# xiexh20/VisTracker

Hardware: AMD Instinct MI355X
Metric: frames/sec joint SMPL+object fit (higher is better)
Workload: dtype f32 (decoder GEMMs: 22-bit split-f16 operands x3 MFMA, fp32 accumulate)

## Files before the change

include/vistracker.h:

```cpp
#ifndef VISTRACKER_H
#define VISTRACKER_H

#ifdef __cplusplus
extern "C" {
#endif

#define VT_OK 0
#define VT_ERR_ARG -1
#define VT_ERR_HIP -2
#define VT_ERR_BUSY -3

#define VT_SMPL_V 6890
#define VT_SMPL_J 52
#define VT_SMPL_NB 10
#define VT_SMPL_NP 459
#define VT_FEAT 611
#define VT_HID 128

const char *vt_last_error(void);
int vt_version(void);

typedef struct vt_smplh vt_smplh;

int vt_smplh_create(vt_smplh **out, const float *v_template, const float *shapedirs, const float *posedirs,
                    const float *J_regressor, const float *weights, const int *parents, void *stream);
void vt_smplh_destroy(vt_smplh *h);

long vt_smplh_workspace_floats(int B);

int vt_smplh_forward(const vt_smplh *h, const float *pose, const float *betas, const float *trans, int B,
                     float *verts, float *jtr, float *v_posed, float *ws, void *stream);

long vt_smplh_bwd_scratch_floats(int B);
int vt_smplh_backward(const vt_smplh *h, const float *pose, const float *betas, int B, const float *dverts,
                      const float *djtr, const float *v_posed, const float *ws, float *scratch,
                      float *dpose, float *dbetas, float *dtrans, void *stream);

int vt_rodrigues_forward(const float *aa, int n, float *R, void *stream);
int vt_rodrigues_backward(const float *aa, int n, const float *dR, float *daa, void *stream);

typedef struct vt_landmarks vt_landmarks;
int vt_landmarks_create(vt_landmarks **out, const int *indptr, const int *indices, const float *data, int K, int V,
                        void *stream);
void vt_landmarks_destroy(vt_landmarks *h);
int vt_landmarks_forward(const vt_landmarks *h, const float *verts, int B, float *out, void *stream);
int vt_landmarks_backward(const vt_landmarks *h, const float *dout, int B, float *dverts, int accumulate, void *stream);

int vt_mahalanobis(const float *x, int B, int stride, int off, int n, const float *mean, const float *prec,
                   float *value, float *dx, float gscale, void *stream);

int vt_fill_f64(double *p, long n, double value, void *stream);
int vt_sum_to_term(const float *value, int n, float scale, double *term, void *stream);

typedef struct vt_sifnet vt_sifnet;
int vt_sifnet_create(vt_sifnet **out, const float *const *w, const float *const *b, const float *cam, void *stream);
void vt_sifnet_destroy(vt_sifnet *h);

int vt_nchw_to_nhwc(const float *src, int B, int C, int H, int W, float *dst, void *stream);

typedef struct {
    const float *maps[8];
    int res[8];
    const float *proj;
    int proj_cols;
    int act_level;
    int proj_level;
    int force_fp32;
} vt_maps;

int vt_query_forward(const vt_sifnet *h, const vt_maps *maps, const float *pts, const float *crop_center,
                     const float *body_center, int B, int N,
                     float *df, float *pca, float *parts, float *centers, float *vis, void *stream);
int vt_query_backward(const vt_sifnet *h, const vt_maps *maps, const float *pts, const float *crop_center,
                      const float *body_center, int B, int N,
                      const float *d_df, const float *d_pca, const float *d_parts, const float *d_centers,
                      const float *d_vis, float *dpts, void *stream);

long vt_query_projection_floats(const vt_maps *maps, int B);
int vt_query_build_projection(const vt_sifnet *h, const vt_maps *maps, int B, float *proj, void *stream);

int vt_query_human_loss(const vt_sifnet *h, const vt_maps *maps, const float *pts, const float *crop_center,
                        const float *body_center, int B, int N, const int *labels, const int *order, float w_dfh, float w_part,
                        float *dpts, double *terms, void *stream);
int vt_query_object_loss(const vt_sifnet *h, const vt_maps *maps, const float *pts, const float *crop_center,
                         const float *body_center, int B, int N, const float *occ, float w_obj,
                         float *dpts, double *terms, void *stream);

typedef struct vt_conv3x3 vt_conv3x3;
int vt_conv3x3_create(vt_conv3x3 **out, const float *weight, int cout, int cin, void *stream);
void vt_conv3x3_destroy(vt_conv3x3 *h);
int vt_conv3x3_forward(const vt_conv3x3 *h, const float *in, int B, int H, int W, float *out, int out_cstride, int out_coff, void *stream);
int vt_conv3x3_forward_gn(const vt_conv3x3 *h, const float *in, int in_cstride, int in_coff, const float *gn_stats, const float *gamma,
                          const float *beta, int groups, int B, int H, int W, float *out, int out_cstride, int out_coff, void *stream);
int vt_conv3x3_forward_gn_stats(const vt_conv3x3 *h, const float *in, int in_cstride, int in_coff, const float *gn_stats, const float *gamma,
                                const float *beta, int groups, int B, int H, int W, float *out, int out_cstride, int out_coff, double *stats_ws,
                                int stats_groups, void *stream);
int vt_conv3x3_forward_block(const vt_conv3x3 *h, const float *in, int in_cstride, int in_coff, const float *gn_stats, const float *gamma,
                             const float *beta, int groups, int B, int H, int W, float *out, int out_cstride, int out_coff,
                             const float *res, int res_cstride, int res_coff, float *fin, int fin_cstride, int fin_coff,
                             double *stats_ws, int stats_groups, void *stream);
int vt_conv3x3_tiles(int H, int W);
typedef struct vt_stem7x7 vt_stem7x7;
int vt_stem7x7_create(vt_stem7x7 **out, const float *weight, const float *bias, int cout, int cin, void *stream);
void vt_stem7x7_destroy(vt_stem7x7 *h);
int vt_stem7x7_forward(const vt_stem7x7 *h, const float *in, int in_cstride, int in_coff, int B, int H, int W, float *out, int out_cstride, int out_coff, void *stream);
typedef struct vt_conv1x1 vt_conv1x1;
int vt_conv1x1_create(vt_conv1x1 **out, const float *weight, const float *bias, int cout, int cin, void *stream);
void vt_conv1x1_destroy(vt_conv1x1 *h);
int vt_conv1x1_forward(const vt_conv1x1 *h, const float *in, int in_cstride, int in_coff, const float *gn_stats, const float *gamma, const float *beta, int groups,
                       int B, int H, int W, float *out, int out_cstride, int out_coff, const float *res, int res_cstride, int res_coff,
                       double *stats_ws, int stats_groups, void *stream);
int vt_groupnorm_finalize(double *ws, int nblk, int B, int HW, int C, int groups, float eps, void *stream);
int vt_conv3x3_forward_block_stats(const vt_conv3x3 *h, const float *in, int in_cstride, int in_coff, const float *gn_stats, const float *gamma,
                                   const float *beta, int groups, int B, int H, int W, float *out, int out_cstride, int out_coff,
                                   const float *res, int res_cstride, int res_coff, float *fin, int fin_cstride, int fin_coff,
                                   double *stats_ws, int stats_groups, double *fin_stats_ws, int fin_stats_groups, void *stream);
int vt_avgpool2x2_stats(const float *x, int B, int H, int W, int C, float *out, double *stats_ws, int stats_groups, void *stream);
int vt_sweep_blocks(int HW);
int vt_groupnorm_stats(const float *x, int cstride, int coff, int B, int HW, int C, int groups, float eps, double *ws, void *stream);

#define VT_PRECISION_SPLIT_F16 0
#define VT_PRECISION_FP32 1
int vt_sifnet_set_precision(vt_sifnet *h, int mode);
int vt_sifnet_get_precision(const vt_sifnet *h);

int vt_query_set_human_kernel(int threads);

int vt_query_project_step(const vt_sifnet *h, const vt_maps *maps, const float *pts, const float *crop_center,
                          const float *body_center, int B, int N, int df_idx, float threshold, float *pts_out,
                          float *df_target, void *stream);

int vt_kpts_step(const vt_landmarks *h, const float *verts, const float *kpts, const float *crop_center, int B, int mode, const float *cam, float net_size,
                 float gscale, double *term, float *J, float *dverts, int accumulate, void *stream);
int vt_query_human_step(const vt_sifnet *h, const vt_maps *maps, const float *pts, const float *crop_center, const float *body_center,
                        int B, int N, const int *labels, const int *order, float w_dfh, float w_part, int accumulate, float w_accel,
                        double *term_accel, float *dpts, double *terms, void *stream);
int vt_objstep_head(const float *M0, const float *noise, const float *t, const float *s, int B, const float *X0_points, int N, float *X_points,
                    const float *X0_verts, int NV, float *X_verts, float *R, double *terms, int nzero, float *svd_ws, void *stream);
int vt_temporal_loss2(const float *v, int B, int D, float gscale_accel, double *term_accel, float gscale_velocity, double *term_velocity, float *dv,
                      int init_zero, void *stream);
int vt_objstep_tail(const float *X0_verts, int NV, const float *dX_verts, const float *X0_points, int N, const float *dX_points, const float *s, int B,
                    const float *M0, const float *noise, const float *t, const float *t_init, float w_trans, double *term_trans,
                    float *dR, float *dt, float *dM,
                    float *pR, float *mR, float *vR, float lrR, float *pT, float *mT, float *vT, float lrT, int adam_step, float beta1, float beta2, float eps,
                    double *terms, const float *w, int nterms, float tol, int armed, float *state, int *stop_flag, float *history, int slot, int *ticket, int nzero,
                    float *svd_ws, void *stream);
int vt_objstep_tail_temporal(const float *X_points, float gscale_accel, double *term_accel, float gscale_velocity, double *term_velocity, int init_zero,
                             const float *X0_verts, int NV, const float *dX_verts, const float *X0_points, int N, const float *dX_points, const float *s, int B,
                             const float *M0, const float *noise, const float *t, const float *t_init, float w_trans, double *term_trans,
                             float *dR, float *dt, float *dM,
                             float *pR, float *mR, float *vR, float lrR, float *pT, float *mT, float *vT, float lrT, int adam_step, float beta1, float beta2, float eps,
                             double *terms, const float *w, int nterms, float tol, int armed, float *state, int *stop_flag, float *history, int slot, int *ticket, int nzero,
                             float *svd_ws, void *stream);
int vt_smplstep_tail(float *pose, const float *pose_init, float *dpose, int B, const float *prior_mean, const float *prior_prec, float gscale_prior,
                     double *term_prior, float w_pinit, double *term_pinit,
                     float *p0, int ps0, const float *g0, int gs0, float *m0, float *v0, int n0, float lr0,
                     float *p1, int ps1, const float *g1, int gs1, float *m1, float *v1, int n1, float lr1,
                     float *p2, int ps2, const float *g2, int gs2, float *m2, float *v2, int n2, float lr2,
                     int adam_step, float beta1, float beta2, float eps,
                     double *terms, const float *w, int nterms, float tol, int armed, float *state, int *stop_flag, float *history, int slot, int *ticket, int nzero,
                     void *stream);

int vt_so3_project_forward(const float *M0, const float *noise, int B, float *R, void *stream);
int vt_so3_project_backward(const float *M0, const float *noise, int B, const float *dR, float *dM, void *stream);

int vt_rigid_forward(const float *X0, int shared_x0, const float *R, const float *t, const float *s, int B, int N,
                     float *X, void *stream);
int vt_rigid_backward(const float *X0, int shared_x0, const float *s, int B, int N, const float *dX,
                      float *dR, float *dt, int accumulate, void *stream);

int vt_accel_loss(const float *v, int B, int D, const float *elem_w, float gscale, double *term, float *dv, void *stream);
int vt_accel_loss_strided(const float *v, int B, int D, int stride, const float *elem_w, float gscale, double *term,
                          float *dv, void *stream);
int vt_velocity_loss(const float *v, int B, int D, float gscale, double *term, float *dv, void *stream);

int vt_kpts_loss(const float *J, const float *kpts, const float *crop_center, int B, int K, int mode,
                 const float *cam, float net_size, float gscale, double *term, float *dJ, void *stream);

int vt_sqdiff_loss(const float *a, int a_stride, const float *b, int b_stride, int rows, int cols, float denom,
                   float gscale, double *term, float *da, void *stream);

long vt_collision_workspace_bytes(int B, int n_smpl_faces);
int vt_collision_loss(const float *smpl_verts, int n_smpl_verts, const int *smpl_faces, int n_smpl_faces, const float *obj_verts, int n_obj_verts,
                      const int *obj_faces, int n_obj_faces, int B, float sigma, int max_collisions, float gscale, double *term,
                      float *d_obj_t, int *pairs_per_frame, void *workspace, void *stream);

int vt_chamfer_ragged(const float *x, const int *offx, const float *y, const int *offy, int P, float gscale,
                      double *term, float *dx, float *dy, void *stream);
long vt_chamfer_ws_bytes(long total_x, long total_y, int P);
int vt_chamfer_ragged_ws(const float *x, const int *offx, long total_x, const float *y, const int *offy, long total_y, int P, float gscale,
                         double *term, float *dx, float *dy, void *ws, void *stream);

int vt_chamfer_ragged_idx(const float *x, const int *offx, long total_x, const float *y_base, const int *idx_y, const int *offy, long total_y, int P,
                          float gscale, double *term, float *dy_base, void *ws, int run_plan, void *stream);

int vt_nn_distance(const float *query, int nq, const float *search, int ns, int P, float *dist, void *stream);

long vt_sil_workspace_floats(int B, int NV, int NF, int size);
int vt_sil_forward(const float *verts, int B, int NV, const int *faces, int NF, const float *K, int size,
                   float *image, int *face_index, float *ws, void *stream);
int vt_sil_backward(const float *verts, int B, int NV, const int *faces, int NF, const float *K, int size,
                    const int *face_index, const float *d_image, float eps, float *ws, float *dverts, void *stream);
int vt_sil_setup(const float *mask_h, const float *mask_o, int B, int H, int W, const float *crop_centers, double expansion, int out, double crop_size,
                 double net_size, const double *cam_norm, double image_width, float *image_ref, float *keep_mask, float *K, double *boxes_ws, void *stream);

int vt_sil_mask_loss(const float *image, const float *keep, const float *ref, const float *occ, int B, int size,
                     float gscale, double *term, float *per_frame, float *d_image, void *stream);

int vt_sil_step(const float *verts, int B, int NV, const int *faces, int NF, const float *K, int size, const float *keep, const float *ref,
                const float *occ, float gscale, float eps, double *term, int *face_index, float *d_image, float *ws, float *dverts, void *stream);

int vt_triplane_render(const float *verts, const float *center, int B, int NV, const int *faces, int NF, int size,
                       float *masks, int *face_index, float *ws, void *stream);

int vt_upsample2x_bicubic_add(const float *low, const float *skip, int B, int h, int w, int C, float *out, void *stream);
int vt_upsample2x_bicubic_add_stats(const float *low, const float *skip, int B, int h, int w, int C, float *out, double *stats_ws, int stats_groups,
                                    void *stream);

long vt_groupnorm_workspace_doubles(int B, int HW, int C, int groups);
int vt_groupnorm_nhwc(const float *x, const float *gamma, const float *beta, int B, int HW, int C, int groups, float eps,
                      int relu, double *ws, float *y, void *stream);

int vt_adam_step(float *p, const float *g, float *m, float *v, long n, int step, float lr, float beta1, float beta2,
                 float eps, const int *stop_flag, void *stream);

int vt_adam_step_2d(float *p, long p_stride, const float *g, long g_stride, float *m, float *v, int rows, int cols,
                    int step, float lr, float beta1, float beta2, float eps, const int *stop_flag, void *stream);

int vt_loss_reduce_and_stop(const double *terms, const float *w, int nterms, float tol, int armed, float *state,
                            int *stop_flag, float *history, int slot, void *stream);

int vt_fill(float *p, long n, float value, void *stream);

int vt_stream_set_skip_flag(void *stream, const int *flag);

int vt_gen_round_compact(const float *surface, const float *df_target, const float *pre, const unsigned char *active, int B, int S, float filter_val,
                         float zmin, const long long *fill, int cap, int write, float *buf_points, int *order, float *kept_pre, long long *cnt,
                         long long *fill_out, void *stream);
int vt_gen_scatter_heads(const float *pred, int B, int C, int kmax, const long long *fill_old, const long long *cnt, int cap, float *buf, void *stream);
int vt_gen_resample(const float *samples, const int *order, const long long *cnt, const float *init, int B, int S, int S0, const float *u,
                    const float *pert, int M, float near_scale, float *out, void *stream);

long vt_render_workspace_bytes(int B, int NF, int size, int anti_aliasing, long list_entries);
int vt_render_static_create(void **layer, const float *verts, int NV, const int *faces, int NS, const float *face_colors, const float *K, float orig_size,
                            const float *light, int size, int anti_aliasing, void *stream);
void vt_render_static_destroy(void *layer);
int vt_render_rgb(const float *verts, int B, int NV, const int *faces, int NF, const float *face_colors, const float *K, int k_per_view, float orig_size,
                  const float *light, const float *background, const void *static_layer, int size, int anti_aliasing, float *rgb, float *alpha, float *depth,
                  int *face_index, void *ws, long ws_bytes, long *list_entries, void *stream);
int vt_render_panel_u8(const float *rgb, int B, int size, int row0, int nrows, int col0, int ncols, unsigned char *out, const long long *view_off,
                       long long out_row_stride, void *stream);
int vt_render_rgb_pv(const float *verts, int B, int NV, const int *faces, int NF, const float *face_colors, int colors_per_view, const float *K, int k_per_view,
                     float orig_size, const float *light, const float *background, const void *static_layer, int size, int anti_aliasing, float *rgb,
                     float *alpha, float *depth, int *face_index, void *ws, long ws_bytes, long *list_entries, void *stream);

int vt_contact_regions(const float *smpl_verts, const int *labels, const float *obj_verts, int B, int NVs, int NVo, int P, float thres, int *nn_idx,
                       float *nn_dist, int *part, int *count, float *centre, void *stream);
int vt_contact_spheres(const float *centre, const int *count, int B, int P, const float *unit_verts, int NSV, float radius, float *out, void *stream);
int vt_contact_face_colors(const int *part, int B, int NVo, const int *obj_faces, int NFo, int face_off, const float *base_colors, int NF, const float *palette,
                           int P, float *out, void *stream);

long vt_jpeg_workspace_bytes(int n, int H, int W, int subsampling, long long *max_out_bytes);
int vt_jpeg_encode(const unsigned char *rgb, int n, int H, int W, long long frame_stride, long long row_stride, int quality, int subsampling, void *ws,
                   long ws_bytes, unsigned char *out, long long out_cap, long long *offsets, void *stream);

int vt_mask_bbox(const unsigned char *pm, const unsigned char *om, int B, int H, int W, int thres, int *box, void *stream);
int vt_crop_resize_compose(const unsigned char *rgb, const unsigned char *pm, const unsigned char *om, int B, int H, int W, const int *corners, int crop_size,
                           int out_size, const float *table, float *out, long long frame_stride, void *stream);
int vt_resize_panel_u8(const unsigned char *src, long long src_bytes, const long long *frames, int n, int H, int size, int col0, int pw, unsigned char *out,
                       const long long *out_off, long long out_row_stride, void *stream);

int vt_overlay_panel_u8(const float *rgb, const float *alpha, int B, int size, int row0, int nrows, int col0, int ncols, unsigned char *out,
                        const long long *src_off, const long long *dst_off, long long out_row_stride, float opacity, void *stream);
int vt_mask_score(const int *fidx, int B, int is, int rows, int F, int nf_body, int nf_obj, const unsigned char *pm, long long pm_bytes, const unsigned char *om,
                  long long om_bytes, const long long *frames, int thres, int *count, void *stream);

long vt_point_mesh_workspace_bytes(int B, int n_faces);
int vt_point_mesh_distance(const float *points, int n_points, const float *verts, int n_verts, const int *faces, int n_faces, int B, float *dist, float *closest,
                           int *face_id, void *workspace, void *stream);
int vt_point_mesh_distance_ex(const float *points, int n_points, const float *verts, int n_verts, const int *faces, int n_faces, int B, float *dist,
                              float *closest, int *face_id, void *workspace, int flags, unsigned long long *n_tests, void *stream);
int vt_nearest_vertex(const float *points, int n_points, const float *verts, int n_verts, int B, int *vert_id, float *vert_dist, void *stream);

long vt_sifnet_loss_head_ws_bytes(int B, int n_points);
int vt_sifnet_loss_head(const float *df, const float *pca, const float *parts, const float *centers, const float *vis, int S, int B, int n_points,
                        const float *df_h, const float *df_o, const int *parts_gt, const float *pca_gt, const float *obj_center, const float *visibility,
                        int per_frame, float max_dist, const double *weights, int vis_loss, float gscale, double *terms, float *d_df, float *d_pca,
                        float *d_parts, float *d_centers, float *d_vis, void *workspace, void *stream);

long vt_decoder_param_floats(void);
long vt_decoder_param_offset(int head, int layer, int is_bias);
int vt_decoder_train_forward(const float *params, const float *cam, const vt_maps *maps, const float *pts, const float *crop_center, const float *body_center,
                             int B, int N, float *df, float *pca, float *parts, float *centers, float *vis, void *stream);
long vt_decoder_weight_grads_ws_bytes(int B, int N, int chunk_points);
int vt_decoder_weight_grads(const float *params, const float *cam, const vt_maps *maps, const float *pts, const float *crop_center, const float *body_center,
                            int B, int N, const float *d_df, const float *d_pca, const float *d_parts, const float *d_centers, const float *d_vis,
                            float *dparams, int accumulate, int chunk_points, void *workspace, void *stream);

long vt_decoder_grads_ws_bytes(int B, int N, int chunk_points, int want_maps);
int vt_decoder_grads(const float *params, const float *cam, const vt_maps *maps, const float *pts, const float *crop_center, const float *body_center,
                     int B, int N, const float *d_df, const float *d_pca, const float *d_parts, const float *d_centers, const float *d_vis,
                     float *dparams, int accumulate, const vt_maps *d_maps, int accumulate_maps, int chunk_points, void *workspace, void *stream);

long vt_conv_dgrad_workspace_bytes(int cout, int cin, int taps);
long vt_conv_wgrad_workspace_bytes(int B, int H, int W, int cout, int cin, int taps);
long vt_gn_relu_backward_workspace_bytes(int B, int HW, int C, int groups);
int vt_conv3x3_dgrad(const float *weight, int cout, int cin, const float *d_out, int do_cstride, int do_coff, int B, int H, int W,
                     float *d_in, int di_cstride, int di_coff, void *workspace, void *stream);
int vt_conv1x1_dgrad(const float *weight, int cout, int cin, const float *d_out, int do_cstride, int do_coff, int B, int H, int W,
                     float *d_in, int di_cstride, int di_coff, void *workspace, void *stream);
int vt_conv3x3_wgrad(const float *d_out, int do_cstride, int do_coff, const float *x_in, int xi_cstride, int xi_coff, const float *gn_stats, const float *gamma,
                     const float *beta, int groups, int B, int H, int W, int cin, int cout, float *dW, int accumulate, void *workspace, void *stream);
int vt_conv1x1_wgrad(const float *d_out, int do_cstride, int do_coff, const float *x_in, int xi_cstride, int xi_coff, const float *gn_stats, const float *gamma,
                     const float *beta, int groups, int B, int H, int W, int cin, int cout, float *dW, int accumulate, void *workspace, void *stream);
int vt_gn_relu_backward(const float *g, int g_cstride, int g_coff, const float *x_in, int x_cstride, int x_coff, const float *gn_stats, const float *gamma,
                        const float *beta, int groups, int B, int HW, int C, const float *base, int base_cstride, int base_coff,
                        float *d_x, int dx_cstride, int dx_coff, float *dgamma, float *dbeta, int accumulate, void *workspace, void *stream);
long vt_conv_block_backward_workspace(int B, int H, int W, int cin, int c1, int c2, int c3);
int vt_conv_block_backward(const float *dy, const float *x, const float *raw, const float *stats1, const float *stats2, const float *stats3,
                           const float *w1, const float *w2, const float *w3, const float *gamma1, const float *gamma2, const float *gamma3,
                           const float *beta1, const float *beta2, const float *beta3, const float *wproj, const float *gamma4, const float *beta4,
                           int B, int H, int W, int cin, int c1, int c2, int c3,
                           float *d_x, float *dW1, float *dW2, float *dW3, float *dgamma1, float *dbeta1, float *dgamma2, float *dbeta2, float *dgamma3, float *dbeta3,
                           float *dgamma4, float *dbeta4, float *dWproj, void *workspace, int accumulate, void *stream);

int vt_query_set_clock_probe(unsigned long long *counters);
long vt_calibrate_workspace_bytes(void);
int vt_calibrate(void *work, double *out, void *stream);

#ifdef __cplusplus
}
#endif
#endif
```

vistracker_amd/_lib.py:

```python
from __future__ import annotations

import ctypes as C
import os

_HERE = os.path.dirname(os.path.abspath(__file__))
LIB_PATH = os.environ.get("VT_LIB_PATH", os.path.join(_HERE, "libvistracker_hip.so"))

vp = C.c_void_p
fp = C.c_void_p
ci = C.c_int
cl = C.c_long
cf = C.c_float
cd = C.c_double


class VtMaps(C.Structure):
    _fields_ = [("maps", C.c_void_p * 8), ("res", C.c_int * 8), ("proj", C.c_void_p), ("proj_cols", C.c_int),
                ("act_level", C.c_int), ("proj_level", C.c_int), ("force_fp32", C.c_int)]


SIGNATURES = {
    "vt_last_error": (C.c_char_p, []),
    "vt_version": (ci, []),
    "vt_smplh_create": (ci, [C.POINTER(vp), vp, vp, vp, vp, vp, vp, vp]),
    "vt_smplh_destroy": (None, [vp]),
    "vt_smplh_workspace_floats": (cl, [ci]),
    "vt_smplh_bwd_scratch_floats": (cl, [ci]),
    "vt_smplh_forward": (ci, [vp, fp, fp, fp, ci, fp, fp, fp, fp, vp]),
    "vt_smplh_backward": (ci, [vp, fp, fp, ci, fp, fp, fp, fp, fp, fp, fp, fp, vp]),
    "vt_rodrigues_forward": (ci, [fp, ci, fp, vp]),
    "vt_rodrigues_backward": (ci, [fp, ci, fp, fp, vp]),
    "vt_landmarks_create": (ci, [C.POINTER(vp), vp, vp, vp, ci, ci, vp]),
    "vt_landmarks_destroy": (None, [vp]),
    "vt_landmarks_forward": (ci, [vp, fp, ci, fp, vp]),
    "vt_landmarks_backward": (ci, [vp, fp, ci, fp, ci, vp]),
    "vt_mahalanobis": (ci, [fp, ci, ci, ci, ci, fp, fp, fp, fp, cf, vp]),
    "vt_fill_f64": (ci, [fp, cl, cd, vp]),
    "vt_sum_to_term": (ci, [fp, ci, cf, fp, vp]),
    "vt_sifnet_create": (ci, [C.POINTER(vp), C.POINTER(vp), C.POINTER(vp), vp, vp]),
    "vt_sifnet_destroy": (None, [vp]),
    "vt_nchw_to_nhwc": (ci, [fp, ci, ci, ci, ci, fp, vp]),
    "vt_query_forward": (ci, [vp, C.POINTER(VtMaps), fp, fp, fp, ci, ci, fp, fp, fp, fp, fp, vp]),
    "vt_query_backward": (ci, [vp, C.POINTER(VtMaps), fp, fp, fp, ci, ci, fp, fp, fp, fp, fp, fp, vp]),
    "vt_query_human_loss": (ci, [vp, C.POINTER(VtMaps), fp, fp, fp, ci, ci, fp, fp, cf, cf, fp, fp, vp]),
    "vt_query_object_loss": (ci, [vp, C.POINTER(VtMaps), fp, fp, fp, ci, ci, fp, cf, fp, fp, vp]),
    "vt_query_set_human_kernel": (ci, [ci]),
    "vt_sifnet_set_precision": (ci, [vp, ci]),
    "vt_sifnet_get_precision": (ci, [vp]),
    "vt_groupnorm_nhwc": (ci, [fp, fp, fp, ci, ci, ci, ci, cf, ci, fp, fp, vp]),
    "vt_upsample2x_bicubic_add": (ci, [fp, fp, ci, ci, ci, ci, fp, vp]),
    "vt_conv3x3_create": (ci, [C.POINTER(vp), vp, ci, ci, vp]),
    "vt_conv3x3_destroy": (None, [vp]),
    "vt_conv3x3_forward": (ci, [vp, fp, ci, ci, ci, fp, ci, ci, vp]),
    "vt_conv3x3_forward_gn": (ci, [vp, fp, ci, ci, fp, fp, fp, ci, ci, ci, ci, fp, ci, ci, vp]),
    "vt_groupnorm_stats": (ci, [fp, ci, ci, ci, ci, ci, ci, cf, fp, vp]),
    "vt_groupnorm_workspace_doubles": (C.c_long, [ci, ci, ci, ci]),
    "vt_groupnorm_finalize": (ci, [fp, ci, ci, ci, ci, ci, cf, vp]),
    "vt_conv3x3_tiles": (ci, [ci, ci]),
    "vt_kpts_step": (ci, [vp, fp, fp, fp, ci, ci, vp, cf, cf, fp, fp, fp, ci, vp]),
    "vt_query_human_step": (ci, [vp, C.POINTER(VtMaps), fp, fp, fp, ci, ci, fp, fp, cf, cf, ci, cf, fp, fp, fp, vp]),
    "vt_objstep_head": (ci, [fp, fp, fp, fp, ci, fp, ci, fp, fp, ci, fp, fp, fp, ci, fp, vp]),
    "vt_temporal_loss2": (ci, [fp, ci, ci, cf, fp, cf, fp, fp, ci, vp]),
    "vt_objstep_tail": (ci, [fp, ci, fp, fp, ci, fp, fp, ci, fp, fp, fp, fp, cf, fp, fp, fp, fp,
                             fp, fp, fp, cf, fp, fp, fp, cf, ci, cf, cf, cf,
                             fp, vp, ci, cf, ci, fp, fp, fp, ci, fp, ci, fp, vp]),
    "vt_objstep_tail_temporal": (ci, [fp, cf, fp, cf, fp, ci,
                                      fp, ci, fp, fp, ci, fp, fp, ci, fp, fp, fp, fp, cf, fp, fp, fp, fp,
                                      fp, fp, fp, cf, fp, fp, fp, cf, ci, cf, cf, cf,
                                      fp, vp, ci, cf, ci, fp, fp, fp, ci, fp, ci, fp, vp]),
    "vt_smplstep_tail": (ci, [fp, fp, fp, ci, fp, fp, cf, fp, cf, fp,
                              fp, ci, fp, ci, fp, fp, ci, cf, fp, ci, fp, ci, fp, fp, ci, cf, fp, ci, fp, ci, fp, fp, ci, cf, ci, cf, cf, cf,
                              fp, vp, ci, cf, ci, fp, fp, fp, ci, fp, ci, vp]),
    "vt_stream_set_skip_flag": (ci, [vp, vp]),
    "vt_conv1x1_create": (ci, [C.POINTER(vp), vp, vp, ci, ci, vp]),
    "vt_stem7x7_create": (ci, [C.POINTER(vp), vp, vp, ci, ci, vp]),
    "vt_stem7x7_destroy": (None, [vp]),
    "vt_stem7x7_forward": (ci, [vp, fp, ci, ci, ci, ci, ci, fp, ci, ci, vp]),
    "vt_conv1x1_destroy": (None, [vp]),
    "vt_conv1x1_forward": (ci, [vp, fp, ci, ci, fp, fp, fp, ci, ci, ci, ci, fp, ci, ci, fp, ci, ci, fp, ci, vp]),
    "vt_conv3x3_forward_block": (ci, [vp, fp, ci, ci, fp, fp, fp, ci, ci, ci, ci, fp, ci, ci, fp, ci, ci, fp, ci, ci, fp, ci, vp]),
    "vt_conv3x3_forward_block_stats": (ci, [vp, fp, ci, ci, fp, fp, fp, ci, ci, ci, ci, fp, ci, ci, fp, ci, ci, fp, ci, ci, fp, ci, fp, ci, vp]),
    "vt_avgpool2x2_stats": (ci, [fp, ci, ci, ci, ci, fp, fp, ci, vp]),
    "vt_sweep_blocks": (ci, [ci]),
    "vt_upsample2x_bicubic_add_stats": (ci, [fp, fp, ci, ci, ci, ci, fp, fp, ci, vp]),
    "vt_conv3x3_forward_gn_stats": (ci, [vp, fp, ci, ci, fp, fp, fp, ci, ci, ci, ci, fp, ci, ci, fp, ci, vp]),
    "vt_triplane_render": (ci, [fp, fp, ci, ci, fp, ci, ci, fp, fp, fp, vp]),
    "vt_query_project_step": (ci, [vp, C.POINTER(VtMaps), fp, fp, fp, ci, ci, ci, cf, fp, fp, vp]),
    "vt_query_projection_floats": (C.c_long, [C.POINTER(VtMaps), ci]),
    "vt_query_build_projection": (ci, [vp, C.POINTER(VtMaps), ci, fp, vp]),
    "vt_so3_project_forward": (ci, [fp, fp, ci, fp, vp]),
    "vt_so3_project_backward": (ci, [fp, fp, ci, fp, fp, vp]),
    "vt_rigid_forward": (ci, [fp, ci, fp, fp, fp, ci, ci, fp, vp]),
    "vt_rigid_backward": (ci, [fp, ci, fp, ci, ci, fp, fp, fp, ci, vp]),
    "vt_accel_loss": (ci, [fp, ci, ci, fp, cf, fp, fp, vp]),
    "vt_accel_loss_strided": (ci, [fp, ci, ci, ci, fp, cf, fp, fp, vp]),
    "vt_velocity_loss": (ci, [fp, ci, ci, cf, fp, fp, vp]),
    "vt_kpts_loss": (ci, [fp, fp, fp, ci, ci, ci, vp, cf, cf, fp, fp, vp]),
    "vt_sqdiff_loss": (ci, [fp, ci, fp, ci, ci, ci, cf, cf, fp, fp, vp]),
    "vt_chamfer_ragged": (ci, [fp, fp, fp, fp, ci, cf, fp, fp, fp, vp]),
    "vt_chamfer_ws_bytes": (C.c_long, [C.c_long, C.c_long, ci]),
    "vt_chamfer_ragged_ws": (ci, [fp, fp, C.c_long, fp, fp, C.c_long, ci, cf, fp, fp, fp, fp, vp]),
    "vt_chamfer_ragged_idx": (ci, [fp, fp, C.c_long, fp, fp, fp, C.c_long, ci, cf, fp, fp, fp, ci, vp]),
    "vt_collision_workspace_bytes": (cl, [ci, ci]),
    "vt_collision_loss": (ci, [fp, ci, fp, ci, fp, ci, fp, ci, ci, cf, ci, cf, fp, fp, fp, fp, vp]),
    "vt_nn_distance": (ci, [fp, ci, fp, ci, ci, fp, vp]),
    "vt_sil_workspace_floats": (cl, [ci, ci, ci, ci]),
    "vt_sil_forward": (ci, [fp, ci, ci, fp, ci, fp, ci, fp, fp, fp, vp]),
    "vt_sil_backward": (ci, [fp, ci, ci, fp, ci, fp, ci, fp, fp, cf, fp, fp, vp]),
    "vt_sil_mask_loss": (ci, [fp, fp, fp, fp, ci, ci, cf, fp, fp, fp, vp]),
    "vt_sil_step": (ci, [fp, ci, ci, fp, ci, fp, ci, fp, fp, fp, cf, cf, fp, fp, fp, fp, fp, vp]),
    "vt_gen_round_compact": (ci, [fp, fp, fp, vp, ci, ci, cf, cf, vp, ci, ci, fp, vp, fp, vp, vp, vp]),
    "vt_gen_scatter_heads": (ci, [fp, ci, ci, ci, vp, vp, ci, fp, vp]),
    "vt_gen_resample": (ci, [fp, vp, vp, fp, ci, ci, ci, fp, fp, ci, cf, fp, vp]),
    "vt_sil_setup": (ci, [fp, fp, ci, ci, ci, fp, C.c_double, ci, C.c_double, C.c_double, C.POINTER(C.c_double), C.c_double, fp, fp, fp, fp, vp]),
    "vt_adam_step": (ci, [fp, fp, fp, fp, cl, ci, cf, cf, cf, cf, fp, vp]),
    "vt_adam_step_2d": (ci, [fp, cl, fp, cl, fp, fp, ci, ci, ci, cf, cf, cf, cf, fp, vp]),
    "vt_loss_reduce_and_stop": (ci, [fp, vp, ci, cf, ci, fp, fp, fp, ci, vp]),
    "vt_fill": (ci, [fp, cl, cf, vp]),
    "vt_selftest_mfma": (ci, [fp, fp, fp, vp]),
    "vt_query_set_clock_probe": (ci, [vp]),
    "vt_render_workspace_bytes": (cl, [ci, ci, ci, ci, cl]),
    "vt_render_static_create": (ci, [C.POINTER(vp), fp, ci, fp, ci, fp, fp, cf, C.POINTER(cf), ci, ci, vp]),
    "vt_render_static_destroy": (None, [vp]),
    "vt_render_rgb": (ci, [fp, ci, ci, fp, ci, fp, fp, ci, cf, C.POINTER(cf), C.POINTER(cf), vp, ci, ci, fp, fp, fp, fp, fp, cl,
                           C.POINTER(cl), vp]),
    "vt_render_panel_u8": (ci, [fp, ci, ci, ci, ci, ci, ci, fp, fp, C.c_longlong, vp]),
    "vt_render_rgb_pv": (ci, [fp, ci, ci, fp, ci, fp, ci, fp, ci, cf, C.POINTER(cf), C.POINTER(cf), vp, ci, ci, fp, fp, fp, fp, fp, cl,
                              C.POINTER(cl), vp]),
    "vt_contact_regions": (ci, [fp, fp, fp, ci, ci, ci, ci, cf, fp, fp, fp, fp, fp, vp]),
    "vt_contact_spheres": (ci, [fp, fp, ci, ci, fp, ci, cf, fp, vp]),
    "vt_contact_face_colors": (ci, [fp, ci, ci, fp, ci, ci, fp, ci, fp, ci, fp, vp]),
    "vt_jpeg_workspace_bytes": (cl, [ci, ci, ci, ci, C.POINTER(C.c_longlong)]),
    "vt_jpeg_encode": (ci, [fp, ci, ci, ci, C.c_longlong, C.c_longlong, ci, ci, vp, cl, vp, C.c_longlong,
                            C.POINTER(C.c_longlong), vp]),
    "vt_mask_bbox": (ci, [fp, fp, ci, ci, ci, ci, fp, vp]),
    "vt_crop_resize_compose": (ci, [fp, fp, fp, ci, ci, ci, fp, ci, ci, fp, fp, C.c_longlong, vp]),
    "vt_resize_panel_u8": (ci, [fp, C.c_longlong, vp, ci, ci, ci, ci, ci, fp, fp, C.c_longlong, vp]),
    "vt_overlay_panel_u8": (ci, [fp, fp, ci, ci, ci, ci, ci, ci, fp, fp, fp, C.c_longlong, cf, vp]),
    "vt_mask_score": (ci, [fp, ci, ci, ci, ci, ci, ci, fp, C.c_longlong, fp, C.c_longlong, vp, ci, fp, vp]),
    "vt_point_mesh_workspace_bytes": (cl, [ci, ci]),
    "vt_point_mesh_distance": (ci, [fp, ci, fp, ci, fp, ci, ci, fp, fp, fp, vp, vp]),
    "vt_point_mesh_distance_ex": (ci, [fp, ci, fp, ci, fp, ci, ci, fp, fp, fp, vp, ci, fp, vp]),
    "vt_nearest_vertex": (ci, [fp, ci, fp, ci, ci, fp, fp, vp]),
    "vt_sifnet_loss_head_ws_bytes": (cl, [ci, ci]),
    "vt_sifnet_loss_head": (ci, [fp, fp, fp, fp, fp, ci, ci, ci, fp, fp, fp, fp, fp, fp, ci, cf, C.POINTER(cd), ci, cf, fp, fp, fp, fp, fp, fp, vp, vp]),
    "vt_decoder_param_floats": (cl, []),
    "vt_decoder_param_offset": (cl, [ci, ci, ci]),
    "vt_decoder_train_forward": (ci, [fp, vp, C.POINTER(VtMaps), fp, fp, fp, ci, ci, fp, fp, fp, fp, fp, vp]),
    "vt_decoder_weight_grads_ws_bytes": (cl, [ci, ci, ci]),
    "vt_decoder_weight_grads": (ci, [fp, vp, C.POINTER(VtMaps), fp, fp, fp, ci, ci, fp, fp, fp, fp, fp, fp, ci, ci, vp, vp]),
    "vt_decoder_grads_ws_bytes": (cl, [ci, ci, ci, ci]),
    "vt_decoder_grads": (ci, [fp, vp, C.POINTER(VtMaps), fp, fp, fp, ci, ci, fp, fp, fp, fp, fp, fp, ci, C.POINTER(VtMaps), ci, ci, vp, vp]),
    "vt_conv_dgrad_workspace_bytes": (cl, [ci, ci, ci]),
    "vt_conv_wgrad_workspace_bytes": (cl, [ci, ci, ci, ci, ci, ci]),
    "vt_gn_relu_backward_workspace_bytes": (cl, [ci, ci, ci, ci]),
    "vt_conv3x3_dgrad": (ci, [fp, ci, ci, fp, ci, ci, ci, ci, ci, fp, ci, ci, vp, vp]),
    "vt_conv1x1_dgrad": (ci, [fp, ci, ci, fp, ci, ci, ci, ci, ci, fp, ci, ci, vp, vp]),
    "vt_conv3x3_wgrad": (ci, [fp, ci, ci, fp, ci, ci, fp, fp, fp, ci, ci, ci, ci, ci, ci, fp, ci, vp, vp]),
    "vt_conv1x1_wgrad": (ci, [fp, ci, ci, fp, ci, ci, fp, fp, fp, ci, ci, ci, ci, ci, ci, fp, ci, vp, vp]),
    "vt_gn_relu_backward": (ci, [fp, ci, ci, fp, ci, ci, fp, fp, fp, ci, ci, ci, ci, fp, ci, ci, fp, ci, ci, fp, fp, ci, vp, vp]),
    "vt_conv_block_backward_workspace": (cl, [ci, ci, ci, ci, ci, ci, ci]),
    "vt_conv_block_backward": (ci, [fp] * 6 + [fp] * 9 + [fp] * 3 + [ci] * 7 + [fp] * 13 + [vp, ci, vp]),
    "vt_calibrate_workspace_bytes": (cl, []),
    "vt_calibrate": (ci, [vp, C.POINTER(C.c_double), vp]),
}

_lib = None


class VtError(RuntimeError):
    pass


def lib():
    global _lib
    if _lib is None:
        if not os.path.exists(LIB_PATH):
            raise VtError(f"{LIB_PATH} is missing: build it with `make -C vistracker_amd/csrc` "
                          f"(or `python -c 'import __graft_entry__ as g; g.build()'`); there is no CPU fallback")
        import torch
        l = C.CDLL(LIB_PATH)
        for name, (res, args) in SIGNATURES.items():
            fn = getattr(l, name)
            fn.restype = res
            fn.argtypes = args
        _lib = l
        _host_tuning()
    return _lib


def _host_tuning():
    if os.environ.get("VT_HOST_THP", "keep") != "off":
        return
    try:
        C.CDLL(None, use_errno=True).prctl(41, 1, 0, 0, 0)
    except Exception:
        pass


VT_OK, VT_ERR_ARG, VT_ERR_HIP, VT_ERR_BUSY = 0, -1, -2, -3


def check(rc: int):
    if rc != 0:
        raise VtError(f"libvistracker_hip error {rc}: {lib().vt_last_error().decode()}")


def stream_ptr():
    import torch
    return torch.cuda.current_stream().cuda_stream


def dptr(t):
    if t is None:
        return None
    if not t.is_cuda:
        raise VtError("libvistracker_hip ops need CUDA (HIP) tensors; there is no CPU fallback in the product path")
    if not t.is_contiguous():
        raise VtError("libvistracker_hip ops need contiguous tensors")
    import torch
    if t.device.index != torch.cuda.current_device():
        raise VtError(f"tensor on cuda:{t.device.index} but the current device is cuda:{torch.cuda.current_device()}: "
                      "wrap the call in `with torch.cuda.device(tensor.device):`")
    return t.data_ptr()
```

vistracker_amd/csrc/smplh.hip:

```cpp
#include "common.h"
#include <cstring>

#define V_ VT_SMPL_V
#define J_ VT_SMPL_J
#define NB_ VT_SMPL_NB
#define NP_ VT_SMPL_NP
#define VP_ 6912
#define NVT_ 27
#define KQ_ 472
#define NQ_ 480
typedef float f32x4 __attribute__((ext_vector_type(4)));
#define MFMA16(a, b, c) __builtin_amdgcn_mfma_f32_16x16x4f32((a), (b), (c), 0, 0, 0)

#define WS_R 0
#define WS_J (52 * 9)
#define WS_G (WS_J + 52 * 3)
#define WS_A (WS_G + 52 * 12)
#define WS_FRAME (WS_A + 52 * 12)
#define PT_DA 0
#define PT_DTR 624
#define PT_N 627
#define KTOT_ (VP_ * 3)
#define KG_SLAB 24
#define NKS_ (KTOT_ / 16 / KG_SLAB)

#define SCHED_STEPS 32
#define SCHED_WIDTH 10
struct SmplParents { int p[J_]; int nsteps; short sched[SCHED_STEPS][SCHED_WIDTH]; };

#define SP_K 8
struct vt_smplh {
    float *Q_kcv, *Q_t, *W_jv, *W_v64, *J_t, *J_s;
    float *W_sp;
    int nnz;
    SmplParents par;
};

struct RodCtx { float n, ax, ay, az, c, s, qn, w, x, y, z; };

__device__ __forceinline__ void rodrigues_fwd(const float *t, float *R, RodCtx *k)
{
    const float xe = t[0] + 1e-8f, ye = t[1] + 1e-8f, ze = t[2] + 1e-8f;
    const float n = sqrtf(xe * xe + ye * ye + ze * ze);
    const float ax = t[0] / n, ay = t[1] / n, az = t[2] / n;
    const float h = n * 0.5f;
    const float c = cosf(h), s = sinf(h);
    const float q0 = c, q1 = s * ax, q2 = s * ay, q3 = s * az;
    const float qn = sqrtf(q0 * q0 + q1 * q1 + q2 * q2 + q3 * q3);
    const float w = q0 / qn, x = q1 / qn, y = q2 / qn, z = q3 / qn;
    const float w2 = w * w, x2 = x * x, y2 = y * y, z2 = z * z;
    const float wx = w * x, wy = w * y, wz = w * z, xy = x * y, xz = x * z, yz = y * z;
    R[0] = w2 + x2 - y2 - z2; R[1] = 2 * xy - 2 * wz;   R[2] = 2 * wy + 2 * xz;
    R[3] = 2 * wz + 2 * xy;   R[4] = w2 - x2 + y2 - z2; R[5] = 2 * yz - 2 * wx;
    R[6] = 2 * xz - 2 * wy;   R[7] = 2 * wx + 2 * yz;   R[8] = w2 - x2 - y2 + z2;
    if (k) { k->n = n; k->ax = ax; k->ay = ay; k->az = az; k->c = c; k->s = s; k->qn = qn; k->w = w; k->x = x; k->y = y; k->z = z; }
}

__device__ __forceinline__ void rodrigues_bwd(const float *t, const float *dR, float *dt)
{
    float R[9]; RodCtx k; rodrigues_fwd(t, R, &k);
    const float w = k.w, x = k.x, y = k.y, z = k.z;
    const float dw = 2 * w * (dR[0] + dR[4] + dR[8]) + 2 * (-z * dR[1] + y * dR[2] + z * dR[3] - x * dR[5] - y * dR[6] + x * dR[7]);
    const float dx = 2 * x * (dR[0] - dR[4] - dR[8]) + 2 * (y * dR[1] + z * dR[2] + y * dR[3] - w * dR[5] + z * dR[6] + w * dR[7]);
    const float dy = 2 * y * (-dR[0] + dR[4] - dR[8]) + 2 * (x * dR[1] + w * dR[2] + x * dR[3] + z * dR[5] - w * dR[6] + z * dR[7]);
    const float dz = 2 * z * (-dR[0] - dR[4] + dR[8]) + 2 * (-w * dR[1] + x * dR[2] + w * dR[3] + y * dR[5] + x * dR[6] + y * dR[7]);
    const float dot = w * dw + x * dx + y * dy + z * dz;
    const float dq0 = (dw - w * dot) / k.qn, dq1 = (dx - x * dot) / k.qn, dq2 = (dy - y * dot) / k.qn, dq3 = (dz - z * dot) / k.qn;
    const float dh = -k.s * dq0 + k.c * (k.ax * dq1 + k.ay * dq2 + k.az * dq3);
    const float dax = k.s * dq1, day = k.s * dq2, daz = k.s * dq3;
    const float dn = 0.5f * dh - (t[0] * dax + t[1] * day + t[2] * daz) / (k.n * k.n);
    dt[0] = dax / k.n + dn * (t[0] + 1e-8f) / k.n;
    dt[1] = day / k.n + dn * (t[1] + 1e-8f) / k.n;
    dt[2] = daz / k.n + dn * (t[2] + 1e-8f) / k.n;
}

__global__ void rodrigues_fwd_kernel(const float *aa, int n, float *R)
{
    const int i = blockIdx.x * blockDim.x + threadIdx.x;
    if (i >= n) return;
    float t[3] = {aa[3 * i], aa[3 * i + 1], aa[3 * i + 2]}, r[9];
    rodrigues_fwd(t, r, nullptr);
#pragma unroll
    for (int e = 0; e < 9; e++) R[9 * i + e] = r[e];
}

__global__ void rodrigues_bwd_kernel(const float *aa, int n, const float *dR, float *daa)
{
    const int i = blockIdx.x * blockDim.x + threadIdx.x;
    if (i >= n) return;
    float t[3] = {aa[3 * i], aa[3 * i + 1], aa[3 * i + 2]}, g[9], d[3];
#pragma unroll
    for (int e = 0; e < 9; e++) g[e] = dR[9 * i + e];
    rodrigues_bwd(t, g, d);
    daa[3 * i] = d[0]; daa[3 * i + 1] = d[1]; daa[3 * i + 2] = d[2];
}

__global__ __launch_bounds__(64) void smplh_pose_kernel(const float *__restrict__ pose, const float *__restrict__ betas,
                                                        const float *__restrict__ trans, const float *__restrict__ J_t,
                                                        const float *__restrict__ J_s, SmplParents par,
                                                        float *__restrict__ ws, float *__restrict__ jtr, const int *skip)
{
    VT_SKIP_RETURN(skip);
    __shared__ float sR[J_ * 9], sJ[J_ * 3], sG[J_ * 12];
    const int b = blockIdx.x, j = threadIdx.x;
    float *w = ws + (size_t)b * WS_FRAME;
    if (j < J_) {
        float t[3] = {pose[(b * J_ + j) * 3], pose[(b * J_ + j) * 3 + 1], pose[(b * J_ + j) * 3 + 2]}, R[9];
        rodrigues_fwd(t, R, nullptr);
#pragma unroll
        for (int e = 0; e < 9; e++) { sR[j * 9 + e] = R[e]; w[WS_R + j * 9 + e] = R[e]; }
#pragma unroll
        for (int c = 0; c < 3; c++) {
            float a = J_t[j * 3 + c];
#pragma unroll
            for (int l = 0; l < NB_; l++) a += J_s[(j * 3 + c) * NB_ + l] * betas[b * NB_ + l];
            sJ[j * 3 + c] = a; w[WS_J + j * 3 + c] = a;
        }
    }
    __shared__ int sPar[J_];
    if (j < J_) sPar[j] = par.p[j];
    __syncthreads();
    int lvl = 0, maxl = 0;
    if (j < J_) { for (int q = j; q != 0; q = sPar[q]) lvl++; }
    maxl = lvl;
    for (int o = 32; o > 0; o >>= 1) maxl = max(maxl, __shfl_xor(maxl, o, 64));
    maxl = __builtin_amdgcn_readfirstlane(maxl);
    if (j == 0) { for (int r = 0; r < 3; r++) { for (int c = 0; c < 3; c++) sG[r * 4 + c] = sR[r * 3 + c]; sG[r * 4 + 3] = sJ[r]; } }
    __syncthreads();
    for (int l = 1; l <= maxl; l++) {
        if (j < J_ && lvl == l) {
            const int i = j, p = sPar[i];
            const float *Gp = sG + 12 * p, *Ri = sR + 9 * i;
            const float d0 = sJ[3 * i] - sJ[3 * p], d1 = sJ[3 * i + 1] - sJ[3 * p + 1], d2 = sJ[3 * i + 2] - sJ[3 * p + 2];
            float *Gi = sG + 12 * i;
            for (int r = 0; r < 3; r++) {
                const float g0 = Gp[r * 4], g1 = Gp[r * 4 + 1], g2 = Gp[r * 4 + 2];
                Gi[r * 4 + 0] = g0 * Ri[0] + g1 * Ri[3] + g2 * Ri[6];
                Gi[r * 4 + 1] = g0 * Ri[1] + g1 * Ri[4] + g2 * Ri[7];
                Gi[r * 4 + 2] = g0 * Ri[2] + g1 * Ri[5] + g2 * Ri[8];
                Gi[r * 4 + 3] = g0 * d0 + g1 * d1 + g2 * d2 + Gp[r * 4 + 3];
            }
        }
        __syncthreads();
    }
    if (j < J_) {
        const float *G = sG + 12 * j;
#pragma unroll
        for (int r = 0; r < 3; r++) {
            const float gt = G[r * 4 + 3];
            w[WS_G + j * 12 + r * 4 + 0] = G[r * 4]; w[WS_G + j * 12 + r * 4 + 1] = G[r * 4 + 1];
            w[WS_G + j * 12 + r * 4 + 2] = G[r * 4 + 2]; w[WS_G + j * 12 + r * 4 + 3] = gt;
            w[WS_A + j * 12 + r * 4 + 0] = G[r * 4]; w[WS_A + j * 12 + r * 4 + 1] = G[r * 4 + 1]; w[WS_A + j * 12 + r * 4 + 2] = G[r * 4 + 2];
            w[WS_A + j * 12 + r * 4 + 3] = gt - (G[r * 4] * sJ[3 * j] + G[r * 4 + 1] * sJ[3 * j + 1] + G[r * 4 + 2] * sJ[3 * j + 2]);
            if (jtr) jtr[(b * J_ + j) * 3 + r] = gt + trans[3 * b + r];
        }
    }
}

#define FWD_FB 16
#ifndef FWD_PF
#define FWD_PF 6
#endif
#define AXS 516
#define SAS 628
#define FWD_R0 (FWD_FB * AXS > 8 * SAS ? FWD_FB * AXS : 8 * SAS)
__global__ __launch_bounds__(256) void smplh_verts_kernel(const float *__restrict__ Q_kcv, const float *__restrict__ W_jv,
                                                          const float *__restrict__ betas, const float *__restrict__ trans,
                                                          const float *__restrict__ ws, int B,
                                                          float *__restrict__ verts, float *__restrict__ v_posed, const float *__restrict__ W_sp, int nnz, const int *skip)
{
    VT_SKIP_RETURN(skip);
    extern __shared__ __attribute__((aligned(16))) float lds[];
    float *sAx = lds;
    float *sA = lds;
    float *sVp = lds + FWD_R0;
    float *sW = sVp + FWD_FB * 64 * 3;
    float *sTr = sW + (nnz > 0 ? 2 * SP_K * 64 : J_ * 64);
    const int tid = threadIdx.x, wave = tid >> 6, lane = tid & 63, q = lane >> 4, j = lane & 15;
    const int b0 = blockIdx.y * FWD_FB, v = blockIdx.x * 64 + wave * 16 + j;
    for (int k = tid; k < KQ_; k += 256) {
        const int e9 = k % 9;
        const float sub = (k < NP_ && (e9 == 0 || e9 == 4 || e9 == 8)) ? 1.f : 0.f;
        float val[FWD_FB];
#pragma unroll
        for (int f = 0; f < FWD_FB; f++) {
            const int b = min(b0 + f, B - 1);
            if (k < NP_) val[f] = ws[(size_t)b * WS_FRAME + WS_R + 9 + k];
            else if (k < NP_ + NB_) val[f] = betas[b * NB_ + (k - NP_)];
            else val[f] = (k == NP_ + NB_) ? 1.f : 0.f;
        }
#pragma unroll
        for (int f = 0; f < FWD_FB; f++) sAx[f * AXS + k] = val[f] - sub;
    }
    if (nnz > 0) {
        for (int i = tid; i < nnz * 64; i += 256) {
            sW[i] = W_sp[(size_t)(i >> 6) * VP_ + blockIdx.x * 64 + (i & 63)];
            sW[SP_K * 64 + i] = W_sp[(size_t)(SP_K + (i >> 6)) * VP_ + blockIdx.x * 64 + (i & 63)];
        }
    } else
        for (int i = tid; i < J_ * 64; i += 256) sW[i] = W_jv[(i >> 6) * VP_ + blockIdx.x * 64 + (i & 63)];
    if (tid < FWD_FB * 3) { const int f = tid / 3, b = min(b0 + f, B - 1); sTr[tid] = trans[b * 3 + tid % 3]; }
    __syncthreads();

    f32x4 acc[3];
#pragma unroll
    for (int c = 0; c < 3; c++) acc[c] = (f32x4){0.f, 0.f, 0.f, 0.f};
    constexpr int NS = KQ_ / 8;
    float bq[FWD_PF][2][3];
#define FWD_LOADQ(slot_, s_)                                                                     \
    {                                                                                            \
        const float *qk = Q_kcv + (size_t)(8 * (s_) + 2 * q) * 3 * VP_ + v;                      \
        _Pragma("unroll") for (int e = 0; e < 2; e++)                                            \
            _Pragma("unroll") for (int c = 0; c < 3; c++) bq[slot_][e][c] = qk[(size_t)(e * 3 + c) * VP_]; \
    }
#pragma unroll
    for (int s = 0; s < FWD_PF; s++) FWD_LOADQ(s, s)
#pragma unroll
    for (int s = 0; s < NS; s++) {
        const float2 av = *reinterpret_cast<const float2 *>(sAx + j * AXS + 8 * s + 2 * q);
#pragma unroll
        for (int c = 0; c < 3; c++) acc[c] = MFMA16(av.x, bq[s % FWD_PF][0][c], acc[c]);
#pragma unroll
        for (int c = 0; c < 3; c++) acc[c] = MFMA16(av.y, bq[s % FWD_PF][1][c], acc[c]);
        if (s + FWD_PF < NS) FWD_LOADQ(s % FWD_PF, s + FWD_PF)
        __builtin_amdgcn_sched_barrier(0);
    }
#undef FWD_LOADQ
    __syncthreads();
#pragma unroll
    for (int r = 0; r < 4; r++)
#pragma unroll
        for (int c = 0; c < 3; c++) sVp[((4 * q + r) * 64 + wave * 16 + j) * 3 + c] = acc[c][r];
    const int vv = tid & 63, vg = blockIdx.x * 64 + vv;
#pragma unroll 1
    for (int r = 0; r < 4; r++) {
        if ((r & 1) == 0) {
            if (r) __syncthreads();
            for (int i = tid; i < 8 * 624; i += 256) {
                const int sl = i / 624, f = 4 * (sl >> 1) + r + (sl & 1), b = min(b0 + f, B - 1);
                sA[sl * SAS + (i % 624)] = ws[(size_t)b * WS_FRAME + WS_A + (i % 624)];
            }
            __syncthreads();
        }
        const int f = 4 * wave + r, b = b0 + f;
        float T[12];
#pragma unroll
        for (int e = 0; e < 12; e++) T[e] = 0.f;
        const float4 *Af = reinterpret_cast<const float4 *>(sA + (2 * wave + (r & 1)) * SAS);
        if (nnz > 0) {
            for (int k = 0; k < nnz; k++) {
                const int jj = __float_as_int(sW[k * 64 + vv]);
                const float wj = sW[(SP_K + k) * 64 + vv];
                const float4 a0 = Af[jj * 3], a1 = Af[jj * 3 + 1], a2 = Af[jj * 3 + 2];
                T[0] += wj * a0.x; T[1] += wj * a0.y; T[2] += wj * a0.z; T[3] += wj * a0.w;
                T[4] += wj * a1.x; T[5] += wj * a1.y; T[6] += wj * a1.z; T[7] += wj * a1.w;
                T[8] += wj * a2.x; T[9] += wj * a2.y; T[10] += wj * a2.z; T[11] += wj * a2.w;
            }
        } else {
#pragma unroll 4
            for (int jj = 0; jj < J_; jj++) {
                const float wj = sW[jj * 64 + vv];
                const float4 a0 = Af[jj * 3], a1 = Af[jj * 3 + 1], a2 = Af[jj * 3 + 2];
                T[0] += wj * a0.x; T[1] += wj * a0.y; T[2] += wj * a0.z; T[3] += wj * a0.w;
                T[4] += wj * a1.x; T[5] += wj * a1.y; T[6] += wj * a1.z; T[7] += wj * a1.w;
                T[8] += wj * a2.x; T[9] += wj * a2.y; T[10] += wj * a2.z; T[11] += wj * a2.w;
            }
        }
        if (b < B && vg < V_) {
            const float p0 = sVp[(f * 64 + vv) * 3], p1 = sVp[(f * 64 + vv) * 3 + 1], p2 = sVp[(f * 64 + vv) * 3 + 2];
            const size_t o = ((size_t)b * V_ + vg) * 3;
#pragma unroll
            for (int rr = 0; rr < 3; rr++) verts[o + rr] = T[rr * 4] * p0 + T[rr * 4 + 1] * p1 + T[rr * 4 + 2] * p2 + T[rr * 4 + 3] + sTr[f * 3 + rr];
            v_posed[o] = p0; v_posed[o + 1] = p1; v_posed[o + 2] = p2;
        }
    }
}

template <int FB>
__global__ __launch_bounds__(256) void smplh_bwd_tile_kernel(const float *__restrict__ W_v64, const float *__restrict__ ws,
                                                             const float *__restrict__ v_posed, const float *__restrict__ dverts,
                                                             int B, float *__restrict__ part, float *__restrict__ dvp_g, const int *skip)
{
    VT_SKIP_RETURN(skip);
    extern __shared__ __attribute__((aligned(16))) float lds[];
    float *sdT = lds;
    float *sA = sdT + 256 * 13;
    const int tid = threadIdx.x, tile = blockIdx.x, b0 = blockIdx.y * FB, v0 = tile * 256, v = v0 + tid;
    const int wave = tid >> 6, lane = tid & 63, q = lane >> 4, j = lane & 15;
    for (int i = tid; i < FB * 624; i += 256) { const int f = i / 624, b = min(b0 + f, B - 1); sA[i] = ws[(size_t)b * WS_FRAME + WS_A + (i % 624)]; }
    float w1[4][13], w2[64];
#pragma unroll
    for (int mt = 0; mt < 4; mt++)
#pragma unroll
        for (int ks = 0; ks < 13; ks++) w1[mt][ks] = W_v64[(size_t)(v0 + 64 * wave + 16 * mt + j) * 64 + 4 * ks + q];
#pragma unroll
    for (int ks = 0; ks < 64; ks++) w2[ks] = W_v64[(size_t)(v0 + 4 * ks + q) * 64 + wave * 16 + j];
    __syncthreads();
    float dvn[3] = {0.f, 0.f, 0.f}, vpn[3] = {0.f, 0.f, 0.f};
    auto fetch = [&](int b) {
#pragma unroll
        for (int r = 0; r < 3; r++) { dvn[r] = 0.f; vpn[r] = 0.f; }
        if (b < B && v < V_) {
            const size_t o = ((size_t)b * V_ + v) * 3;
            dvn[0] = dverts[o]; dvn[1] = dverts[o + 1]; dvn[2] = dverts[o + 2];
            vpn[0] = v_posed[o]; vpn[1] = v_posed[o + 1]; vpn[2] = v_posed[o + 2];
        }
    };
    fetch(b0);
#pragma unroll 1
    for (int f = 0; f < FB; f++) {
        const int b = b0 + f;
        const float dv[3] = {dvn[0], dvn[1], dvn[2]}, vp[3] = {vpn[0], vpn[1], vpn[2]};
        if (f + 1 < FB) fetch(b + 1);
#pragma unroll
        for (int r = 0; r < 3; r++) {
            sdT[tid * 13 + r * 4 + 0] = dv[r] * vp[0]; sdT[tid * 13 + r * 4 + 1] = dv[r] * vp[1];
            sdT[tid * 13 + r * 4 + 2] = dv[r] * vp[2]; sdT[tid * 13 + r * 4 + 3] = dv[r];
        }
        __syncthreads();
        {
            f32x4 t[4];
#pragma unroll
            for (int mt = 0; mt < 4; mt++) t[mt] = (f32x4){0.f, 0.f, 0.f, 0.f};
#pragma unroll
            for (int ks = 0; ks < 13; ks++) {
                const float bv = j < 12 ? sA[f * 624 + (4 * ks + q) * 12 + j] : 0.f;
#pragma unroll
                for (int mt = 0; mt < 4; mt++) t[mt] = MFMA16(w1[mt][ks], bv, t[mt]);
            }
            const int r4 = (j < 12 ? (j >> 2) : 0) * 4 + 3;
#pragma unroll
            for (int mt = 0; mt < 4; mt++) {
#pragma unroll
                for (int r = 0; r < 4; r++) {
                    const int vl = 64 * wave + 16 * mt + 4 * q + r;
                    float x = t[mt][r] * sdT[vl * 13 + r4];
                    x += __shfl_down(x, 4, 16) + __shfl_down(x, 8, 16);
                    if (j < 3 && b < B) dvp_g[(size_t)b * KTOT_ + (size_t)(v0 + vl) * 3 + j] = x;
                }
            }
        }
        {
            f32x4 acc = (f32x4){0.f, 0.f, 0.f, 0.f}, acc2 = (f32x4){0.f, 0.f, 0.f, 0.f};
#pragma unroll
            for (int ks = 0; ks < 64; ks += 2) {
                const int va = 4 * ks + q, vb = va + 4;
                const float a0 = j < 12 ? sdT[va * 13 + j] : 0.f, a1 = j < 12 ? sdT[vb * 13 + j] : 0.f;
                acc = MFMA16(a0, w2[ks], acc);
                acc2 = MFMA16(a1, w2[ks + 1], acc2);
            }
            acc += acc2;
            if (b < B) {
                float *dst = part + ((size_t)tile * B + b) * PT_N;
                const int jn = wave * 16 + j;
#pragma unroll
                for (int r = 0; r < 4; r++) {
                    const int e = 4 * q + r;
                    if (e < 12) {
                        if (jn < J_) dst[PT_DA + jn * 12 + e] = acc[r];
                        else if (jn == J_ && (e & 3) == 3) dst[PT_DTR + (e >> 2)] = acc[r];
                    }
                }
            }
        }
        __syncthreads();
    }
}

#define BL_M 96
#ifndef BL_NW
#define BL_NW 1
#endif
#define BL_AS 132
__global__ __launch_bounds__(256) void smplh_bwd_blend_kernel(const float *__restrict__ Q_p, const float *__restrict__ dvp_g, int B,
                                                              float *__restrict__ part3, const int *skip)
{
    VT_SKIP_RETURN(skip);
    __shared__ __attribute__((aligned(16))) float sA[BL_M * BL_AS];
    const int tid = threadIdx.x, wave = tid >> 6, lane = tid & 63, q = lane >> 4, j = lane & 15;
    const int ks = blockIdx.x, m0 = blockIdx.z * BL_M, nt0 = blockIdx.y * (4 * BL_NW) + wave * BL_NW;
    f32x4 acc[6][BL_NW];
#pragma unroll
    for (int mt = 0; mt < 6; mt++)
#pragma unroll
        for (int n = 0; n < BL_NW; n++) acc[mt][n] = (f32x4){0.f, 0.f, 0.f, 0.f};
    const float4 *Q4 = reinterpret_cast<const float4 *>(Q_p);
#pragma unroll 1
    for (int c = 0; c < KG_SLAB / 8; c++) {
        __syncthreads();
        for (int i = tid; i < BL_M * 32; i += 256) {
            const int row = i >> 5, c4 = i & 31, b = m0 + row;
            float4 v = make_float4(0.f, 0.f, 0.f, 0.f);
            if (b < B) v = *reinterpret_cast<const float4 *>(dvp_g + (size_t)b * KTOT_ + (size_t)(ks * KG_SLAB + c * 8) * 16 + c4 * 4);
            *reinterpret_cast<float4 *>(sA + row * BL_AS + c4 * 4) = v;
        }
        __syncthreads();
#pragma unroll
        for (int g = 0; g < 8; g++) {
            const size_t kg = (size_t)ks * KG_SLAB + c * 8 + g;
            float bq[BL_NW][4];
#pragma unroll
            for (int n = 0; n < BL_NW; n++) {
                const float4 fq = Q4[(kg * (NQ_ / 16) + min(nt0 + n, NQ_ / 16 - 1)) * 64 + lane];
                bq[n][0] = fq.x; bq[n][1] = fq.y; bq[n][2] = fq.z; bq[n][3] = fq.w;
            }
#pragma unroll
            for (int mt = 0; mt < 6; mt++) {
                const float4 a4 = *reinterpret_cast<const float4 *>(sA + (mt * 16 + j) * BL_AS + g * 16 + q * 4);
                const float av[4] = {a4.x, a4.y, a4.z, a4.w};
#pragma unroll
                for (int s = 0; s < 4; s++)
#pragma unroll
                    for (int n = 0; n < BL_NW; n++) acc[mt][n] = MFMA16(av[s], bq[n][s], acc[mt][n]);
            }
        }
    }
#pragma unroll
    for (int mt = 0; mt < 6; mt++) {
#pragma unroll
        for (int r = 0; r < 4; r++) {
            const int b = m0 + mt * 16 + 4 * q + r;
            if (b < B) {
                float *dst = part3 + ((size_t)ks * B + b) * NQ_;
#pragma unroll
                for (int n = 0; n < BL_NW; n++)
                    if (nt0 + n < NQ_ / 16) dst[(nt0 + n) * 16 + j] = acc[mt][n][r];
            }
        }
    }
}

__global__ __launch_bounds__(256) void smplh_bwd_frame_kernel(const float *__restrict__ pose, const float *__restrict__ J_s,
                                                              SmplParents par, const float *__restrict__ ws,
                                                              const float *__restrict__ part, const float *__restrict__ part3,
                                                              const float *__restrict__ djtr, int B, float *__restrict__ dpose, float *__restrict__ dbetas,
                                                              float *__restrict__ dtrans, const int *skip)
{
    VT_SKIP_RETURN(skip);
    __shared__ float red[PT_N], red3[NQ_];
    __shared__ float sdG[J_ * 12], sdJ[J_ * 3], sdR[J_ * 9];
    __shared__ float sG[J_ * 12], sRm[J_ * 9], sJr[J_ * 3];
    const int b = blockIdx.x, tid = threadIdx.x;
    const float *w = ws + (size_t)b * WS_FRAME;
    for (int i = tid; i < J_ * 12; i += 256) sG[i] = w[WS_G + i];
    for (int i = tid; i < J_ * 9; i += 256) sRm[i] = w[WS_R + i];
    for (int i = tid; i < J_ * 3; i += 256) sJr[i] = w[WS_J + i];
    for (int i = tid; i < PT_N; i += 256) {
        float s = 0.f;
#pragma unroll 9
        for (int t = 0; t < NVT_; t++) s += part[((size_t)t * B + b) * PT_N + i];
        red[i] = s;
    }
    for (int i = tid; i < NQ_; i += 256) {
        float s = 0.f;
#pragma unroll 9
        for (int t = 0; t < NKS_; t++) s += part3[((size_t)t * B + b) * NQ_ + i];
        red3[i] = s;
    }
    __syncthreads();
    if (tid < J_) {
        const int j = tid;
        const float *G = sG + 12 * j; const float *Jr = sJr;
        float dj[3] = {0.f, 0.f, 0.f};
#pragma unroll
        for (int r = 0; r < 3; r++) {
            const float dat = red[PT_DA + 12 * j + r * 4 + 3];
#pragma unroll
            for (int c = 0; c < 3; c++) { sdG[12 * j + r * 4 + c] = red[PT_DA + 12 * j + r * 4 + c] - dat * Jr[3 * j + c]; dj[c] -= G[r * 4 + c] * dat; }
            sdG[12 * j + r * 4 + 3] = dat + (djtr ? djtr[(b * J_ + j) * 3 + r] : 0.f);
        }
        sdJ[3 * j] = dj[0]; sdJ[3 * j + 1] = dj[1]; sdJ[3 * j + 2] = dj[2];
#pragma unroll
        for (int e = 0; e < 9; e++) sdR[9 * j + e] = 0.f;
    }
    __syncthreads();
    const int jloc = tid / 24, el = tid - 24 * jloc;
    const int nsteps = par.nsteps > 0 ? par.nsteps : J_ - 1;
    for (int step = 0; step < nsteps; step++) {
        const int j = par.nsteps > 0 ? (jloc < SCHED_WIDTH ? (int)par.sched[step][jloc < SCHED_WIDTH ? jloc : 0] : -1) : (jloc == 0 ? J_ - 1 - step : -1);
        if (j >= 1) {
            const int p = par.p[j];
            const float *Gp = sG + 12 * p, *Rj = sRm + 9 * j, *dGj = sdG + 12 * j;
            float upd = 0.f; float *dst = nullptr; float upd2 = 0.f; float *dst2 = nullptr;
            if (el < 12) {
                const int r = el >> 2, c = el & 3;
                dst = sdG + 12 * p + el;
                if (c < 3) upd = dGj[r * 4] * Rj[3 * c] + dGj[r * 4 + 1] * Rj[3 * c + 1] + dGj[r * 4 + 2] * Rj[3 * c + 2] + dGj[r * 4 + 3] * (sJr[3 * j + c] - sJr[3 * p + c]);
                else upd = dGj[r * 4 + 3];
            } else if (el < 21) {
                const int e = el - 12, r = e / 3, c = e - 3 * r;
                dst = sdR + 9 * j + e;
                upd = Gp[r] * dGj[c] + Gp[4 + r] * dGj[4 + c] + Gp[8 + r] * dGj[8 + c];
            } else {
                const int c = el - 21;
                upd = Gp[c] * dGj[3] + Gp[4 + c] * dGj[7] + Gp[8 + c] * dGj[11];
                dst = sdJ + 3 * j + c; dst2 = sdJ + 3 * p + c; upd2 = -upd;
            }
            if (dst) *dst += upd;
            if (dst2) *dst2 += upd2;
        }
        __syncthreads();
    }
    if (tid < 3) { for (int c = 0; c < 3; c++) sdR[3 * tid + c] += sdG[tid * 4 + c]; sdJ[tid] += sdG[tid * 4 + 3]; }
    __syncthreads();
    if (tid < J_) {
        const int j = tid;
        float g[9], t[3] = {pose[(b * J_ + j) * 3], pose[(b * J_ + j) * 3 + 1], pose[(b * J_ + j) * 3 + 2]}, d[3];
#pragma unroll
        for (int e = 0; e < 9; e++) g[e] = sdR[9 * j + e] + (j >= 1 ? red3[(j - 1) * 9 + e] : 0.f);
        rodrigues_bwd(t, g, d);
        dpose[(b * J_ + j) * 3] = d[0]; dpose[(b * J_ + j) * 3 + 1] = d[1]; dpose[(b * J_ + j) * 3 + 2] = d[2];
    } else if (tid >= 64 && tid < 64 + NB_) {
        const int l = tid - 64;
        float s = red3[NP_ + l];
        for (int i = 0; i < J_ * 3; i++) s += J_s[i * NB_ + l] * sdJ[i];
        dbetas[b * NB_ + l] = s;
    } else if (tid >= 128 && tid < 131) {
        const int c = tid - 128;
        float s = red[PT_DTR + c];
        if (djtr) for (int j = 0; j < J_; j++) s += djtr[(b * J_ + j) * 3 + c];
        dtrans[b * 3 + c] = s;
    }
}

extern "C" int vt_smplh_create(vt_smplh **out, const float *v_template, const float *shapedirs, const float *posedirs,
                               const float *J_regressor, const float *weights, const int *parents, void *stream)
{
    VT_REQUIRE(out && v_template && shapedirs && posedirs && J_regressor && weights && parents, "vt_smplh_create: null argument");
    hipStream_t st = vt_stream(stream);
    vt_smplh *h = new vt_smplh();
    for (int j = 0; j < J_; j++) h->par.p[j] = (j == 0) ? 0 : parents[j];
    for (int j = 1; j < J_; j++) VT_REQUIRE(h->par.p[j] >= 0 && h->par.p[j] < j, "vt_smplh_create: parents[%d]=%d must be in [0,%d)", j, parents[j], j);
    {
        int lvl[J_], rank[J_], maxl = 0;
        lvl[0] = 0; rank[0] = 0;
        for (int j = 1; j < J_; j++) { lvl[j] = lvl[h->par.p[j]] + 1; maxl = std::max(maxl, lvl[j]); rank[j] = 0; for (int k = j + 1; k < J_; k++) rank[j] += (h->par.p[k] == h->par.p[j]); }
        int n = 0; bool ok = true;
        for (int t = 0; t < SCHED_STEPS; t++) for (int i = 0; i < SCHED_WIDTH; i++) h->par.sched[t][i] = -1;
        for (int l = maxl; l >= 1 && ok; l--)
            for (int r = 0; r < J_ && ok; r++) {
                int cnt = 0;
                for (int j = J_ - 1; j >= 1; j--) if (lvl[j] == l && rank[j] == r) { if (n >= SCHED_STEPS || cnt >= SCHED_WIDTH) { ok = false; break; } h->par.sched[n][cnt++] = (short)j; }
                if (cnt) n++;
            }
        h->par.nsteps = ok ? n : 0;
    }
    float *Q_kcv = new float[(size_t)KQ_ * 3 * VP_](), *Q_t = new float[(size_t)VP_ * 3 * NQ_](), *W_jv = new float[(size_t)J_ * VP_](),
          *J_t = new float[J_ * 3], *J_s = new float[J_ * 3 * NB_];
    for (int v = 0; v < V_; v++) for (int c = 0; c < 3; c++) {
        for (int k = 0; k < NP_ + NB_ + 1; k++) {
            const float val = k < NP_ ? posedirs[((size_t)v * 3 + c) * NP_ + k]
                            : (k < NP_ + NB_ ? shapedirs[((size_t)v * 3 + c) * NB_ + (k - NP_)] : v_template[v * 3 + c]);
            Q_kcv[(size_t)(k * 3 + c) * VP_ + v] = val;
            {
                const size_t kr = (size_t)v * 3 + c, g = kr >> 4, qq = (kr & 15) >> 2, ss = kr & 3;
                Q_t[((g * (NQ_ / 16) + (k >> 4)) * 64 + qq * 16 + (k & 15)) * 4 + ss] = val;
            }
        }
    }
    float *W_v64 = new float[(size_t)VP_ * 64]();
    for (int v = 0; v < V_; v++) { for (int j = 0; j < J_; j++) { W_jv[(size_t)j * VP_ + v] = weights[(size_t)v * J_ + j]; W_v64[(size_t)v * 64 + j] = weights[(size_t)v * J_ + j]; } W_v64[(size_t)v * 64 + J_] = 1.0f; }
    float *W_sp = new float[(size_t)2 * SP_K * VP_]();
    int nnz = 0;
    for (int v = 0; v < V_; v++) {
        int k = 0;
        for (int j = 0; j < J_; j++) {
            const float w = weights[(size_t)v * J_ + j];
            if (w == 0.0f) continue;
            if (k < SP_K) { const int jj = j; memcpy(&W_sp[(size_t)k * VP_ + v], &jj, 4); W_sp[(size_t)(SP_K + k) * VP_ + v] = w; }
            k++;
        }
        nnz = k > nnz ? k : nnz;
    }
    h->nnz = nnz <= SP_K ? (nnz > 0 ? nnz : 1) : 0;
    for (int j = 0; j < J_; j++) for (int c = 0; c < 3; c++) {
        double a = 0; double sb[NB_] = {0};
        for (int v = 0; v < V_; v++) {
            const double r = J_regressor[(size_t)j * V_ + v];
            if (r == 0.0) continue;
            a += r * v_template[v * 3 + c];
            for (int l = 0; l < NB_; l++) sb[l] += r * shapedirs[((size_t)v * 3 + c) * NB_ + l];
        }
        J_t[j * 3 + c] = (float)a;
        for (int l = 0; l < NB_; l++) J_s[(j * 3 + c) * NB_ + l] = (float)sb[l];
    }
    int rc = VT_OK;
    if ((rc = vt_upload(&h->Q_kcv, Q_kcv, (size_t)KQ_ * 3 * VP_, st)) || (rc = vt_upload(&h->Q_t, Q_t, (size_t)VP_ * 3 * NQ_, st)) ||
        (rc = vt_upload(&h->W_jv, W_jv, (size_t)J_ * VP_, st)) || (rc = vt_upload(&h->W_v64, W_v64, (size_t)VP_ * 64, st)) ||
        (rc = vt_upload(&h->J_t, J_t, (size_t)J_ * 3, st)) || (rc = vt_upload(&h->J_s, J_s, (size_t)J_ * 3 * NB_, st)) ||
        (rc = vt_upload(&h->W_sp, W_sp, (size_t)2 * SP_K * VP_, st))) {
        return rc;
    }
    VT_HIP(hipStreamSynchronize(st));
    delete[] Q_kcv; delete[] Q_t; delete[] W_jv; delete[] W_v64; delete[] J_t; delete[] J_s; delete[] W_sp;
    *out = h;
    return VT_OK;
}

extern "C" void vt_smplh_destroy(vt_smplh *h)
{
    if (!h) return;
    hipFree(h->Q_kcv); hipFree(h->Q_t); hipFree(h->W_jv); hipFree(h->W_v64); hipFree(h->J_t); hipFree(h->J_s); hipFree(h->W_sp);
    delete h;
}

extern "C" long vt_smplh_workspace_floats(int B) { return (long)B * WS_FRAME; }
extern "C" long vt_smplh_bwd_scratch_floats(int B) { return (long)NVT_ * B * PT_N + (long)B * KTOT_ + (long)NKS_ * B * NQ_; }

#define BWD_FB 6

extern "C" int vt_smplh_forward(const vt_smplh *h, const float *pose, const float *betas, const float *trans, int B,
                                float *verts, float *jtr, float *v_posed, float *ws, void *stream)
{
    VT_REQUIRE(h && pose && betas && trans && verts && v_posed && ws && B > 0, "vt_smplh_forward: null argument or B <= 0");
    hipStream_t st = vt_stream(stream); const int *skip = vt_skip_flag_of(st);
    hipLaunchKernelGGL(smplh_pose_kernel, dim3(B), dim3(64), 0, st, pose, betas, trans, h->J_t, h->J_s, h->par, ws, jtr, skip);
    VT_LAUNCH_CHECK();
    const size_t lds_f = sizeof(float) * (FWD_R0 + FWD_FB * 64 * 3 + (h->nnz > 0 ? 2 * SP_K * 64 : J_ * 64) + FWD_FB * 3);
    VT_LDS_LIMIT(smplh_verts_kernel, sizeof(float) * (FWD_R0 + FWD_FB * 64 * 3 + J_ * 64 + FWD_FB * 3));
    hipLaunchKernelGGL(smplh_verts_kernel, dim3(VP_ / 64, (B + FWD_FB - 1) / FWD_FB), dim3(256), lds_f, st, h->Q_kcv, h->W_jv, betas, trans, ws, B,
                       verts, v_posed, h->W_sp, h->nnz, skip);
    VT_LAUNCH_CHECK();
    return VT_OK;
}

extern "C" int vt_smplh_backward(const vt_smplh *h, const float *pose, const float *betas, int B, const float *dverts,
                                 const float *djtr, const float *v_posed, const float *ws, float *scratch,
                                 float *dpose, float *dbetas, float *dtrans, void *stream)
{
    (void)betas;
    VT_REQUIRE(h && pose && dverts && v_posed && ws && scratch && dpose && dbetas && dtrans && B > 0, "vt_smplh_backward: null argument or B <= 0");
    hipStream_t st = vt_stream(stream); const int *skip = vt_skip_flag_of(st);
    const size_t lds = sizeof(float) * (256 * 13 + BWD_FB * 624);
    float *dvp_g = scratch + (size_t)NVT_ * B * PT_N, *part3 = dvp_g + (size_t)B * KTOT_;
    VT_LDS_LIMIT(smplh_bwd_tile_kernel<BWD_FB>, lds);
    hipLaunchKernelGGL(smplh_bwd_tile_kernel<BWD_FB>, dim3(NVT_, (B + BWD_FB - 1) / BWD_FB), dim3(256), lds, st, h->W_v64, ws, v_posed, dverts, B, scratch, dvp_g, skip);
    VT_LAUNCH_CHECK();
    hipLaunchKernelGGL(smplh_bwd_blend_kernel, dim3(NKS_, (NQ_ / 16 + 4 * BL_NW - 1) / (4 * BL_NW), (B + BL_M - 1) / BL_M), dim3(256), 0, st, h->Q_t, dvp_g, B, part3, skip);
    VT_LAUNCH_CHECK();
    hipLaunchKernelGGL(smplh_bwd_frame_kernel, dim3(B), dim3(256), 0, st, pose, h->J_s, h->par, ws, scratch, part3, djtr, B, dpose, dbetas, dtrans, skip);
    VT_LAUNCH_CHECK();
    return VT_OK;
}

extern "C" int vt_rodrigues_forward(const float *aa, int n, float *R, void *stream)
{
    VT_REQUIRE(aa && R && n > 0, "vt_rodrigues_forward: bad argument");
    hipLaunchKernelGGL(rodrigues_fwd_kernel, dim3((n + 255) / 256), dim3(256), 0, vt_stream(stream), aa, n, R);
    VT_LAUNCH_CHECK();
    return VT_OK;
}

extern "C" int vt_rodrigues_backward(const float *aa, int n, const float *dR, float *daa, void *stream)
{
    VT_REQUIRE(aa && dR && daa && n > 0, "vt_rodrigues_backward: bad argument");
    hipLaunchKernelGGL(rodrigues_bwd_kernel, dim3((n + 255) / 256), dim3(256), 0, vt_stream(stream), aa, n, dR, daa);
    VT_LAUNCH_CHECK();
    return VT_OK;
}
```

vistracker_amd/fitting.py:

```python
from __future__ import annotations

import contextlib
import ctypes as C
import functools
import os
import threading
import time
from dataclasses import dataclass, field

import numpy as np
import torch

from . import _lib as L
from . import ops

FIT_WEIGHTS = {"pose": 1e-5, "hand": 1e-5, "j2d": 0.09, "object": 900.0, "part": 0.0025, "contact": 900.0, "scale": 100.0,
               "df_h": 100.0, "mask": 0.0009, "ocent": 0.0, "pinit": 25.0, "rot": 100.0, "trans": 100.0,
               "stemp": 10000.0, "otemp": 225.0, "ovtemp": 2500.0, "collide": 9.0}
SMPLT_WEIGHTS = {"pose": 1e-5, "hand": 1e-5, "kpts": 0.09, "temp": 900.0, "ptemp": 25.0, "pinit": 900.0}
JOINT_WEIGHTS_66 = np.repeat(np.array([1, 10, 10, 10, 5, 5, 10, 1, 1, 10, 1, 1, 5, 5, 5, 5, 5, 5, 1, 1, 1, 1], np.float32), 3)
JOINT_WEIGHTS_66[37:39] = 10.0


def _lib():
    return L.lib()


def _chk(rc):
    L.check(rc)


def _ev_begin(prof):
    if prof is None:
        return None
    e = torch.cuda.Event(enable_timing=True); e.record()
    return e


def _flush_events(prof, local, executed):
    if prof is None:
        return
    for k, v in local.items():
        prof[k].extend((a, b, n) for a, b, n, step in v if executed is None or step < executed)


def _ev_end(prof, key, e0, frames, step):
    if prof is None:
        return
    e1 = torch.cuda.Event(enable_timing=True); e1.record()
    prof[key].append((e0, e1, frames, step))


class Terms:

    def __init__(self, names, device):
        self.names = list(names)
        self.buf = torch.zeros(len(self.names), dtype=torch.float64, device=device)
        self.idx = {n: i for i, n in enumerate(self.names)}

    def ptr(self, name):
        return self.buf.data_ptr() + 8 * self.idx[name]

    def zero(self, first=0, count=None):
        count = len(self.names) - first if count is None else count
        _chk(_lib().vt_fill_f64(self.buf.data_ptr() + 8 * first, count, 0.0, L.stream_ptr()))

    def weights(self, table, decay, extra=None):
        w = np.zeros(16, np.float32)
        for n, i in self.idx.items():
            w[i] = table[n] / (1.0 + decay) * (1.0 if extra is None else extra.get(n, 1.0))
        return w


class AdamState:

    def __init__(self, slices, stop_flag):
        self.slices = slices
        self.m = [torch.zeros(p.shape[0], n, device=p.device) for p, n, g, lr in slices]
        self.v = [torch.zeros(p.shape[0], n, device=p.device) for p, n, g, lr in slices]
        self.t = 0
        self.stop_flag = stop_flag

    def tick(self):
        self.t += 1
        return self.t

    def step(self):
        t = self.tick()
        for (p, n, g, lr), m, v in zip(self.slices, self.m, self.v):
            _chk(_lib().vt_adam_step_2d(p.data_ptr(), p.shape[1], g.data_ptr(), g.shape[1], m.data_ptr(), v.data_ptr(), p.shape[0], n,
                                        t, lr, 0.9, 0.999, 1e-8, self.stop_flag.data_ptr(), L.stream_ptr()))

    @functools.cached_property
    def smpl_tail_groups(self):
        out = ()
        for (p, n, g, lr), m, v in zip(self.slices, self.m, self.v):
            out += (p.data_ptr(), p.shape[1], g.data_ptr(), g.shape[1], m.data_ptr(), v.data_ptr(), n, lr)
        return out + (None, 0, None, 0, None, None, 0, 0.0) * (3 - len(self.slices))

    @functools.cached_property
    def object_tail_groups(self):
        rot = trans = (None, None, None, 0.0)
        for (p, n, g, lr), m, v in zip(self.slices, self.m, self.v):
            if n == 9:
                rot = (p.data_ptr(), m.data_ptr(), v.data_ptr(), lr)
            else:
                trans = (p.data_ptr(), m.data_ptr(), v.data_ptr(), lr)
        return rot + trans


def _check_finite(res, what):
    executed = res.losses[:res.steps]
    if executed.size and not np.isfinite(executed).all():
        bad = int(np.flatnonzero(~np.isfinite(executed))[0])
        raise FloatingPointError(f"{what}: non-finite loss at Adam step {bad} (non-finite input or decoder activation out of range)")


def _as_input(t, dev):
    if t is None:
        return None
    return torch.as_tensor(t).to(device=dev, dtype=torch.float32).contiguous()


def _require_params(*ts):
    for t in ts:
        if not (torch.is_tensor(t) and t.is_cuda and t.dtype == torch.float32 and t.is_contiguous()):
            raise L.VtError("fit loops update their parameters in place: pass contiguous float32 CUDA tensors "
                            f"(got {type(t).__name__} {getattr(t, 'dtype', None)} on {getattr(t, 'device', None)})")
        if t.device != ts[0].device:
            raise L.VtError("fit loops: all parameters must live on the same device")


@dataclass
class FitResult:
    steps: int = 0
    outer_iters: int = 0
    stopped_early: bool = False
    losses: np.ndarray = field(default_factory=lambda: np.zeros(0, np.float32))


def morton_order(points) -> np.ndarray:
    p = np.asarray(points, np.float64)
    q = ((p - p.min(0)) / (p.max(0) - p.min(0) + 1e-12) * 1023).astype(np.int64)

    def part(x):
        x = (x | (x << 16)) & 0x030000FF; x = (x | (x << 8)) & 0x0300F00F; x = (x | (x << 4)) & 0x030C30C3
        return (x | (x << 2)) & 0x09249249
    return np.argsort(part(q[:, 0]) | (part(q[:, 1]) << 1) | (part(q[:, 2]) << 2), kind="stable")


def morton_order_device(p: torch.Tensor) -> torch.Tensor:
    p = p.double()
    lo = p.min(0).values; hi = p.max(0).values
    q = ((p - lo) / (hi - lo + 1e-12) * 1023).long()

    def part(x):
        x = (x | (x << 16)) & 0x030000FF; x = (x | (x << 8)) & 0x0300F00F; x = (x | (x << 4)) & 0x030C30C3
        return (x | (x << 2)) & 0x09249249
    key = part(q[:, 0]) | (part(q[:, 1]) << 1)
    if p.shape[1] > 2:
        key = key | (part(q[:, 2]) << 2)
    return torch.argsort(key, stable=True).to(torch.int32)


class _StopWatch:
    _tls = threading.local()

    def __init__(self, ctx, stop, lookahead):
        self.ctx, self.stop, self.look = ctx, stop, lookahead
        self.pending = None; self.n = 0
        if lookahead:
            pool = getattr(self._tls, "pool", None)
            if pool is None or pool[0] != stop.device:
                pool = (stop.device, torch.zeros(2, dtype=torch.int32).pin_memory(), [torch.cuda.Event(), torch.cuda.Event()])
                self._tls.pool = pool
            _, self.host, self.ev = pool

    def _wait(self, k):
        t0 = time.perf_counter()
        self.ev[k].synchronize()
        with self.ctx._counter_lock:
            self.ctx.host_wait_s += time.perf_counter() - t0
        return bool(int(self.host[k]))

    def check(self):
        if not self.look:
            return bool(self.ctx._read_stop(self.stop))
        k = self.n & 1; self.n += 1
        self.host[k:k + 1].copy_(self.stop, non_blocking=True); self.ev[k].record()
        prev, self.pending = self.pending, k
        return prev is not None and self._wait(prev)

    def final(self):
        if not self.look or self.pending is None:
            return False
        k, self.pending = self.pending, None
        return self._wait(k)


class _Fit:

    def __init__(self, dev, names, nsteps, prev_loss, prof):
        self.terms = Terms(names, dev)
        self.stop = torch.zeros(1, dtype=torch.int32, device=dev)
        self.loss_state = torch.full((2,), prev_loss, device=dev)
        self.ticket = torch.zeros(1, dtype=torch.int32, device=dev)
        self.hist = torch.full((nsteps,), float("nan"), device=dev)
        self.lp = {"human": [], "object": []} if prof is not None else None
        self.adam = None


class _SmplFit(_Fit):

    def __init__(self, pose, betas, trans, names, nsteps, prev_loss, prof=None):
        dev = pose.device; B = self.B = pose.shape[0]
        super().__init__(dev, names, nsteps, prev_loss, prof)
        self.pose, self.betas, self.trans = pose, betas, trans
        self.verts = torch.empty(B, 6890, 3, device=dev); self.jtr = torch.empty(B, 52, 3, device=dev); self.vposed = torch.empty_like(self.verts)
        self.ws = torch.empty(_lib().vt_smplh_workspace_floats(B), device=dev); self.scratch = torch.empty(_lib().vt_smplh_bwd_scratch_floats(B), device=dev)
        self.dverts = torch.empty_like(self.verts); self.J = torch.empty(B, 25, 3, device=dev); self.dJ = torch.empty_like(self.J)
        self.dpose = torch.empty(B, 156, device=dev); self.dbetas = torch.empty(B, 10, device=dev); self.dtrans = torch.empty(B, 3, device=dev)
        self.vb = torch.empty(B, device=dev)
        self.pose_init = pose.clone()

    @property
    def vert_order_ptr(self):
        return self.vert_order.data_ptr() if self.vert_order is not None else None


class _ObjectFit(_Fit):

    def __init__(self, ctx, obj_R, obj_t, sil, nsteps, prof):
        dev = obj_R.device; B = self.B = obj_R.shape[0]; N = self.N = ctx.obj_points.shape[0]; NV = self.NV = ctx.obj_verts.shape[0]
        super().__init__(dev, ["object", "otemp", "ovtemp", "mask", "trans", "contact", "collide", "scale"], nsteps, 300.0, prof)
        self.obj_R, self.obj_t, self.sil = obj_R, obj_t, sil
        self.R = torch.empty(B, 3, 3, device=dev); self.X = torch.empty(B, N, 3, device=dev); self.dX = torch.empty_like(self.X)
        self.svd_ws = torch.empty(B, 22, device=dev)
        self.dR = torch.empty(B, 3, 3, device=dev); self.dM = torch.empty(B, 3, 3, device=dev); self.dt = torch.empty(B, 3, device=dev)
        if sil is not None:
            self.Vt = torch.empty(B, NV, 3, device=dev); self.dVt = torch.empty_like(self.Vt)
            self.fidx = torch.empty(B, sil.size, sil.size, dtype=torch.int32, device=dev); self.dimg = torch.empty(B, sil.size, sil.size, device=dev)
            self.sws = torch.empty(_lib().vt_sil_workspace_floats(B, NV, ctx.obj_faces.shape[0], sil.size), device=dev)
            if not ctx.fused_steps:
                self.img = torch.empty_like(self.dimg); self.per = torch.empty(B, device=dev)
        self.trans_init = None
        self.Vc = self.cws = None
        self.contact = None


class FitContext:
    use_projection = True
    sort_object_points = True
    sort_query_points = True
    collision_loss = False
    fused_steps = os.environ.get("VT_FUSED_STEPS", "1") != "0"
    fused_smpl_query = os.environ.get("VT_FUSED_SMPL_QUERY", "0") != "0"
    device_skip = os.environ.get("VT_DEVICE_SKIP", "1") != "0"

    def __init__(self, smpl_model, regressors, priors, decoders=None, part_labels=None, obj_verts=None, obj_faces=None, obj_points=None,
                 cam=ops.DEFAULT_CAM, device="cuda:0"):
        self.device = torch.device(device)
        dev = self.device
        self.smpl = ops.SmplhHandle(smpl_model, dev)
        self.b25 = ops.LandmarkHandle(regressors["body25"], dev)
        self.net = ops.SifNetHandle(decoders, cam, dev) if decoders is not None else None
        self.cam = np.ascontiguousarray(cam, np.float32)
        t = lambda a, dt=torch.float32: None if a is None else torch.as_tensor(np.ascontiguousarray(a), dtype=dt, device=dev)
        self.pri = {k: t(v) for k, v in priors.items()}
        self.labels = t(part_labels, torch.int32)
        self.vert_order = t(morton_order(np.asarray(smpl_model["v_template"])), torch.int32) if self.sort_query_points else None
        if obj_points is not None and self.sort_object_points:
            obj_points = np.asarray(obj_points, np.float32)[morton_order(obj_points)]
        self.obj_verts = t(obj_verts); self.obj_faces = t(obj_faces, torch.int32); self.obj_points = t(obj_points)
        self.smpl_faces = t(np.asarray(smpl_model["f"]).astype(np.int32), torch.int32) if "f" in smpl_model else None
        self.jw66 = t(JOINT_WEIGHTS_66)

    range_retries = 0
    fp32_fallbacks = 0
    _counter_lock = threading.Lock()
    host_wait_s = 0.0

    def _with_range_fallback(self, maps, params, run):
        if self.net is None or maps is None or maps.force_fp32 or self.net.precision == "fp32":
            return run()
        saved = [p.clone() for p in params]
        while True:
            try:
                return run()
            except FloatingPointError as e:
                import warnings
                for p, s0 in zip(params, saved):
                    p.copy_(s0)
                if maps.act_level + 1 < maps.ACT_LEVELS:
                    maps.set_act_level(maps.act_level + 1)
                    warnings.warn(f"{e}; repeating the fit at operand-range level {maps.act_level} of the split-f16 decoders", RuntimeWarning)
                    with self._counter_lock:
                        self.range_retries += 1
                    continue
                if maps.force_fp32:
                    raise
                warnings.warn(f"{e}; repeating the fit on the strict-fp32 decoder kernels (5x slower)", RuntimeWarning)
                maps.set_force_fp32(True)
                with self._counter_lock:
                    self.fp32_fallbacks += 1
                return run()

    def smpl_forward(self, pose, betas, trans, verts, jtr, vposed, ws):
        _chk(_lib().vt_smplh_forward(self.smpl.h, pose.data_ptr(), betas.data_ptr(), trans.data_ptr(), pose.shape[0], verts.data_ptr(),
                                     jtr.data_ptr(), vposed.data_ptr(), ws.data_ptr(), L.stream_ptr()))

    def smpl_backward(self, pose, betas, dverts, vposed, ws, scratch, dpose, dbetas, dtrans):
        _chk(_lib().vt_smplh_backward(self.smpl.h, pose.data_ptr(), betas.data_ptr(), pose.shape[0], dverts.data_ptr(), None, vposed.data_ptr(),
                                      ws.data_ptr(), scratch.data_ptr(), dpose.data_ptr(), dbetas.data_ptr(), dtrans.data_ptr(), L.stream_ptr()))

    def hand_prior_value(self, pose, terms, name, scratch_b):
        B = pose.shape[0]
        for off, m, p in ((66, "lhand_mean", "lhand_prec"), (111, "rhand_mean", "rhand_prec")):
            _chk(_lib().vt_mahalanobis(pose.data_ptr(), B, 156, off, 45, self.pri[m].data_ptr(), self.pri[p].data_ptr(), scratch_b.data_ptr(), None, 0.0, L.stream_ptr()))
            _chk(_lib().vt_sum_to_term(scratch_b.data_ptr(), B, 1.0 / 45.0, terms.ptr(name), L.stream_ptr()))

    def body_prior(self, pose, dpose, w, terms, name, scratch_b):
        B = pose.shape[0]
        _chk(_lib().vt_mahalanobis(pose.data_ptr(), B, 156, 3, 63, self.pri["body_mean"].data_ptr(), self.pri["body_prec"].data_ptr(),
                                   scratch_b.data_ptr(), dpose.data_ptr(), w / B, L.stream_ptr()))
        _chk(_lib().vt_sum_to_term(scratch_b.data_ptr(), B, 1.0 / B, terms.ptr(name), L.stream_ptr()))

    def _run_fit(self, f, start, end, check_every, outer, prof=None):
        res = FitResult()
        with self._skip_after_stop(f.stop) as skipping:
            watch = _StopWatch(self, f.stop, skipping)
            for it in range(start, end):
                step, phase, w, armed = outer(it)
                for i in range(10):
                    step(f, phase, (it - start) * 10 + i, w, armed)
                res.steps += 10
                res.outer_iters += 1
                if (it - start) % check_every == check_every - 1 and watch.check():
                    res.stopped_early = True
                    break
            res.stopped_early = res.stopped_early or watch.final()
        res.losses = f.hist.cpu().numpy()
        if res.stopped_early:
            res.steps = int(np.isfinite(res.losses).sum())
            res.outer_iters = -(-res.steps // 10)
        _flush_events(prof, f.lp, res.steps if (res.stopped_early and self.device_skip) else None)
        _check_finite(res, "fit")
        return res

    def fit_smplt(self, pose, betas, trans, kpts, max_iter=100, iter_for_global=8, temporal=True, pinit_w=900.0,
                  lr_global=0.01, lr_all=0.001, it_range=None, check_every=1, weights=None, early_stop=True):
        with torch.cuda.device(pose.device):
            return self._fit_smplt(pose, betas, trans, kpts, max_iter, iter_for_global, temporal, pinit_w, lr_global, lr_all, it_range, check_every, weights, early_stop)

    def _fit_smplt(self, pose, betas, trans, kpts, max_iter, iter_for_global, temporal, pinit_w, lr_global, lr_all, it_range, check_every, weights, early_stop=True):
        _require_params(pose, betas, trans)
        table = dict(SMPLT_WEIGHTS); table["pinit"] = pinit_w
        if weights is not None:
            table.update({k: float(v) for k, v in weights.items() if k in table})
        start, end = it_range if it_range is not None else (0, max_iter)
        f = _SmplFit(pose, betas, trans, ["kpts", "temp", "ptemp", "pose", "pinit", "hand"], (end - start) * 10, 0.0)
        f.kpts = _as_input(kpts, pose.device)
        f.temporal = temporal and f.B >= 3
        self.hand_prior_value(pose, f.terms, "hand", f.vb)

        def outer(it):
            if f.adam is None or it == iter_for_global:
                if it < iter_for_global:
                    f.adam = AdamState([(trans, 3, f.dtrans, lr_global), (pose, 3, f.dpose, lr_global), (betas, 2, f.dbetas, lr_global)], f.stop)
                else:
                    f.adam = AdamState([(trans, 3, f.dtrans, lr_all), (pose, 66, f.dpose, lr_all), (betas, 10, f.dbetas, lr_all)], f.stop)
            return self._smplt_step, None, f.terms.weights(table, it // 3), int(early_stop and it > 0.3 * max_iter)
        return self._run_fit(f, start, end, check_every, outer)

    def optimize_smpl(self, maps, pose, betas, trans, crop_center, body_center, body_kpts, max_iter=100, iter_for_betas=1,
                      iter_for_pose=1, iter_for_kpts=1, it_range=None, net_size=512.0, check_every=1, prof=None, early_stop=True):
        with torch.cuda.device(pose.device):
            return self._with_range_fallback(maps, (pose, betas, trans), lambda: self._optimize_smpl(
                maps, pose, betas, trans, crop_center, body_center, body_kpts, max_iter, iter_for_betas, iter_for_pose, iter_for_kpts, it_range, net_size,
                check_every, prof, early_stop))

    def _optimize_smpl(self, maps, pose, betas, trans, crop_center, body_center, body_kpts, max_iter, iter_for_betas, iter_for_pose, iter_for_kpts,
                       it_range, net_size, check_every, prof, early_stop=True):
        dev = pose.device
        _require_params(pose, betas, trans)
        split_route = self.net.precision != "fp32" and not maps.force_fp32
        if self.use_projection and split_route:
            maps.build_projection(self.net)
        total = iter_for_betas + iter_for_kpts + iter_for_pose + max_iter
        start, end = it_range if it_range is not None else (0, total)
        f = _SmplFit(pose, betas, trans, ["df_h", "part", "pose", "pinit", "j2d", "stemp", "hand"], (end - start) * 10, 300.0, prof)
        f.maps, f.net_size = maps, net_size
        f.crop_center, f.body_center, f.body_kpts = _as_input(crop_center, dev), _as_input(body_center, dev), _as_input(body_kpts, dev)
        f.vert_order = self.vert_order
        if self.sort_query_points:
            self.smpl_forward(pose, betas, trans, f.verts, f.jtr, f.vposed, f.ws)
            v0 = f.verts[f.B // 2]
            f.vert_order = morton_order_device(torch.stack([v0[:, 0] / v0[:, 2], v0[:, 1] / v0[:, 2]], 1))
        self.hand_prior_value(pose, f.terms, "hand", f.vb)
        if not self.fused_steps:
            step = self._smpl_step
        elif split_route and self.fused_smpl_query:
            step = self._smpl_step_fused_query
        else:
            step = self._smpl_step_fused
        arm_after = 0.25 * max_iter + iter_for_betas + iter_for_pose

        def outer(it):
            if it < iter_for_betas:
                phase = "global"
                if f.adam is None:
                    f.adam = AdamState([(betas, 2, f.dbetas, 0.02), (trans, 3, f.dtrans, 0.02)], f.stop)
            else:
                phase = "kpts" if it >= iter_for_betas + iter_for_pose else "smpl all pose"
                if f.adam is None or it == iter_for_betas:
                    f.adam = AdamState([(trans, 3, f.dtrans, 0.006), (pose, 66, f.dpose, 0.006), (betas, 10, f.dbetas, 0.006)], f.stop)
            return step, phase, f.terms.weights(FIT_WEIGHTS, 1 if phase != "kpts" else it / 3), int(early_stop and it > arm_after)
        return self._run_fit(f, start, end, check_every, outer, prof)

    def optimize_smpl_object(self, maps, smpl_verts, obj_R, obj_t, obj_s, crop_center, body_center, occ, sil=None, noise=None,
                             iter_for_obj=15, iter_for_sil=30, joint_iter=10, max_iter=100, it_range=None, seed=0, check_every=1, prof=None, early_stop=True):
        with torch.cuda.device(obj_R.device):
            return self._with_range_fallback(maps, (obj_R, obj_t), lambda: self._optimize_smpl_object(
                maps, smpl_verts, obj_R, obj_t, obj_s, crop_center, body_center, occ, sil, noise, iter_for_obj, iter_for_sil, joint_iter, max_iter, it_range,
                seed, check_every, prof, early_stop))

    def _optimize_smpl_object(self, maps, smpl_verts, obj_R, obj_t, obj_s, crop_center, body_center, occ, sil, noise, iter_for_obj, iter_for_sil,
                              joint_iter, max_iter, it_range, seed, check_every, prof, early_stop=True):
        dev = obj_R.device; B = obj_R.shape[0]
        _require_params(obj_R, obj_t)
        if self.use_projection and self.net.precision != "fp32" and not maps.force_fp32:
            maps.build_projection(self.net)
        total = joint_iter + iter_for_obj + max_iter + iter_for_sil
        start, end = it_range if it_range is not None else (0, total)
        f = _ObjectFit(self, obj_R, obj_t, sil, (end - start) * 10, prof)
        f.maps = maps
        f.smpl_verts, f.obj_s, f.crop_center, f.body_center, f.occ = (_as_input(x, dev) for x in (smpl_verts, obj_s, crop_center, body_center, occ))
        f.obj_s = f.obj_s.reshape(-1)
        if noise is not None:
            f.noise = _as_input(noise, dev)
        else:
            gen = torch.Generator(device=dev); gen.manual_seed(seed)
            f.noise = torch.rand((end - start) * 10, B, 3, 3, device=dev, generator=gen)
        ones = torch.ones_like(f.obj_s)
        _chk(_lib().vt_sqdiff_loss(f.obj_s.data_ptr(), 1, ones.data_ptr(), 1, B, 1, float(B), 0.0, f.terms.ptr("scale"), None, L.stream_ptr()))
        Rv, dMv = obj_R.view(B, 9), f.dM.view(B, 9)

        def outer(it):
            if it < iter_for_obj:
                phase = "object only"
                if f.adam is None:
                    f.adam = AdamState([(Rv, 9, dMv, 0.002), (obj_t, 3, f.dt, 0.006)], f.stop)
            elif it < iter_for_obj + iter_for_sil:
                phase = "sil"
                if sil is None:
                    raise L.VtError("phase 'sil' needs a SilSetup")
                if f.adam is None or it == iter_for_obj:
                    f.adam = AdamState([(Rv, 9, dMv, 0.006), (obj_t, 3, f.dt, 0.006)], f.stop)
                    f.trans_init = obj_t.clone()
            else:
                phase = "joint"
                if f.adam is None or it == iter_for_obj + iter_for_sil:
                    f.adam = AdamState([(obj_t, 3, f.dt, 0.002)], f.stop)
            decay = 1 if phase == "object only" else (it - iter_for_obj + 1 if phase == "sil" else (it - iter_for_obj + 1) / 3)
            tw = 10.0 if phase == "joint" else 1.0
            w = f.terms.weights(FIT_WEIGHTS, decay, {"otemp": tw, "ovtemp": tw})
            fused = self.fused_steps and not (phase == "joint" and self.collision_loss)
            return (self._object_step_fused if fused else self._object_step), phase, w, int(early_stop and phase == "joint" and it > 0.25 * max_iter)
        return self._run_fit(f, start, end, check_every, outer, prof)

    def _read_stop(self, stop):
        t0 = time.perf_counter()
        v = int(stop.item())
        with self._counter_lock:
            self.host_wait_s += time.perf_counter() - t0
        return v

    @contextlib.contextmanager
    def _skip_after_stop(self, stop):
        if not self.device_skip:
            yield False
            return
        sp = L.stream_ptr()
        rc = _lib().vt_stream_set_skip_flag(sp, stop.data_ptr())
        if rc == L.VT_ERR_BUSY:
            yield False
            return
        L.check(rc)
        try:
            yield True
        finally:
            _lib().vt_stream_set_skip_flag(sp, None)

    def _smplt_step(self, f, phase, k, w, armed):
        lib = _lib(); st = L.stream_ptr(); B = f.B; pose = f.pose
        f.terms.zero(0, 5)
        self.smpl_forward(pose, f.betas, f.trans, f.verts, f.jtr, f.vposed, f.ws)
        _chk(lib.vt_landmarks_forward(self.b25.h, f.verts.data_ptr(), B, f.J.data_ptr(), st))
        _chk(lib.vt_kpts_loss(f.J.data_ptr(), f.kpts.data_ptr(), None, B, 25, 0, self.cam.ctypes.data, 0.0, float(w[0]), f.terms.ptr("kpts"), f.dJ.data_ptr(), st))
        _chk(lib.vt_landmarks_backward(self.b25.h, f.dJ.data_ptr(), B, f.dverts.data_ptr(), 0, st))
        if f.temporal:
            _chk(lib.vt_accel_loss(f.verts.data_ptr(), B, 6890 * 3, None, float(w[1]), f.terms.ptr("temp"), f.dverts.data_ptr(), st))
        self.smpl_backward(pose, f.betas, f.dverts, f.vposed, f.ws, f.scratch, f.dpose, f.dbetas, f.dtrans)
        if f.temporal:
            _chk(lib.vt_accel_loss_strided(pose.data_ptr(), B, 66, 156, self.jw66.data_ptr(), float(w[2]), f.terms.ptr("ptemp"), f.dpose.data_ptr(), st))
        self.body_prior(pose, f.dpose, float(w[3]), f.terms, "pose", f.vb)
        _chk(lib.vt_sqdiff_loss(pose.data_ptr() + 12, 156, f.pose_init.data_ptr() + 12, 156, B, 63, float(B * 63), float(w[4]),
                                f.terms.ptr("pinit"), f.dpose.data_ptr() + 12, st))
        f.adam.step()
        _chk(lib.vt_loss_reduce_and_stop(f.terms.buf.data_ptr(), w.ctypes.data, len(f.terms.names), 1e-3, armed, f.loss_state.data_ptr(),
                                         f.stop.data_ptr(), f.hist.data_ptr(), k, st))

    def _human_query(self, f, k, w):
        ev = _ev_begin(f.lp)
        _chk(_lib().vt_query_human_loss(self.net.h, C.byref(f.maps.c), f.verts.data_ptr(), f.crop_center.data_ptr(), f.body_center.data_ptr(), f.B, 6890,
                                        self.labels.data_ptr(), f.vert_order_ptr, float(w[0]), float(w[1]), f.dverts.data_ptr(), f.terms.ptr("df_h"),
                                        L.stream_ptr()))
        _ev_end(f.lp, "human", ev, f.B, k)

    def _smpl_step(self, f, phase, k, w, armed):
        lib = _lib(); st = L.stream_ptr(); B = f.B; pose = f.pose
        f.terms.zero(0, 6)
        self.smpl_forward(pose, f.betas, f.trans, f.verts, f.jtr, f.vposed, f.ws)
        self._human_query(f, k, w)
        if phase == "kpts":
            _chk(lib.vt_landmarks_forward(self.b25.h, f.verts.data_ptr(), B, f.J.data_ptr(), st))
            _chk(lib.vt_kpts_loss(f.J.data_ptr(), f.body_kpts.data_ptr(), f.crop_center.data_ptr(), B, 25, 1, self.cam.ctypes.data, f.net_size,
                                  float(w[4]), f.terms.ptr("j2d"), f.dJ.data_ptr(), st))
            _chk(lib.vt_landmarks_backward(self.b25.h, f.dJ.data_ptr(), B, f.dverts.data_ptr(), 1, st))
        if B >= 4:
            _chk(lib.vt_accel_loss(f.verts.data_ptr(), B, 6890 * 3, None, float(w[5]), f.terms.ptr("stemp"), f.dverts.data_ptr(), st))
        self.smpl_backward(pose, f.betas, f.dverts, f.vposed, f.ws, f.scratch, f.dpose, f.dbetas, f.dtrans)
        self.body_prior(pose, f.dpose, float(w[2]), f.terms, "pose", f.vb)
        _chk(lib.vt_sqdiff_loss(pose.data_ptr() + 12, 156, f.pose_init.data_ptr() + 12, 156, B, 69, float(B), float(w[3]),
                                f.terms.ptr("pinit"), f.dpose.data_ptr() + 12, st))
        f.adam.step()
        _chk(lib.vt_loss_reduce_and_stop(f.terms.buf.data_ptr(), w.ctypes.data, len(f.terms.names), 1e-3, armed, f.loss_state.data_ptr(),
                                         f.stop.data_ptr(), f.hist.data_ptr(), k, st))

    def _smpl_step_fused(self, f, phase, k, w, armed):
        lib = _lib(); st = L.stream_ptr(); B = f.B
        self.smpl_forward(f.pose, f.betas, f.trans, f.verts, f.jtr, f.vposed, f.ws)
        self._human_query(f, k, w)
        if phase == "kpts":
            _chk(lib.vt_kpts_step(self.b25.h, f.verts.data_ptr(), f.body_kpts.data_ptr(), f.crop_center.data_ptr(), B, 1, self.cam.ctypes.data, f.net_size,
                                  float(w[4]), f.terms.ptr("j2d"), f.J.data_ptr(), f.dverts.data_ptr(), 1, st))
        if B >= 4:
            _chk(lib.vt_accel_loss(f.verts.data_ptr(), B, 6890 * 3, None, float(w[5]), f.terms.ptr("stemp"), f.dverts.data_ptr(), st))
        self.smpl_backward(f.pose, f.betas, f.dverts, f.vposed, f.ws, f.scratch, f.dpose, f.dbetas, f.dtrans)
        self._smpl_tail(f, k, w, armed)

    def _smpl_step_fused_query(self, f, phase, k, w, armed):
        lib = _lib(); st = L.stream_ptr(); B = f.B
        self.smpl_forward(f.pose, f.betas, f.trans, f.verts, f.jtr, f.vposed, f.ws)
        if phase == "kpts":
            _chk(lib.vt_kpts_step(self.b25.h, f.verts.data_ptr(), f.body_kpts.data_ptr(), f.crop_center.data_ptr(), B, 1, self.cam.ctypes.data, f.net_size,
                                  float(w[4]), f.terms.ptr("j2d"), f.J.data_ptr(), f.dverts.data_ptr(), 0, st))
        ev = _ev_begin(f.lp)
        _chk(lib.vt_query_human_step(self.net.h, C.byref(f.maps.c), f.verts.data_ptr(), f.crop_center.data_ptr(), f.body_center.data_ptr(), B, 6890,
                                     self.labels.data_ptr(), f.vert_order_ptr, float(w[0]), float(w[1]), int(phase == "kpts"), float(w[5]),
                                     f.terms.ptr("stemp") if B >= 4 else None, f.dverts.data_ptr(), f.terms.ptr("df_h"), st))
        _ev_end(f.lp, "human", ev, B, k)
        self.smpl_backward(f.pose, f.betas, f.dverts, f.vposed, f.ws, f.scratch, f.dpose, f.dbetas, f.dtrans)
        self._smpl_tail(f, k, w, armed)

    def _smpl_tail(self, f, k, w, armed):
        _chk(_lib().vt_smplstep_tail(f.pose.data_ptr(), f.pose_init.data_ptr(), f.dpose.data_ptr(), f.B, self.pri["body_mean"].data_ptr(),
                                     self.pri["body_prec"].data_ptr(), float(w[2]) / f.B, f.terms.ptr("pose"), float(w[3]), f.terms.ptr("pinit"),
                                     *f.adam.smpl_tail_groups, f.adam.tick(), 0.9, 0.999, 1e-8,
                                     f.terms.buf.data_ptr(), w.ctypes.data, len(f.terms.names), 1e-3, armed, f.loss_state.data_ptr(), f.stop.data_ptr(),
                                     f.hist.data_ptr(), k, f.ticket.data_ptr(), 6, L.stream_ptr()))

    def _object_query(self, f, k, w):
        ev = _ev_begin(f.lp)
        _chk(_lib().vt_query_object_loss(self.net.h, C.byref(f.maps.c), f.X.data_ptr(), f.crop_center.data_ptr(), f.body_center.data_ptr(), f.B, f.N,
                                         f.occ.data_ptr(), float(w[0]), f.dX.data_ptr(), f.terms.ptr("object"), L.stream_ptr()))
        _ev_end(f.lp, "object", ev, f.B, k)

    def _contacts(self, f, w):
        if f.contact is None:
            f.contact = self._contacts_once(f.maps, f.smpl_verts, f.X, f.crop_center, f.body_center)
        if f.contact["P"] > 0:
            self._contact_term(f.contact, f.X, f.dX, float(w[5]), f.terms)

    def _object_step(self, f, phase, k, w, armed):
        lib = _lib(); st = L.stream_ptr(); B, N, NV, nz = f.B, f.N, f.NV, f.noise[k]
        obj_R, obj_t, obj_s, X, dX, R, dR, dt = f.obj_R, f.obj_t, f.obj_s, f.X, f.dX, f.R, f.dR, f.dt
        nf = self.obj_faces.shape[0]
        f.terms.zero(0, 7)
        _chk(lib.vt_so3_project_forward(obj_R.data_ptr(), nz.data_ptr(), B, R.data_ptr(), st))
        _chk(lib.vt_rigid_forward(self.obj_points.data_ptr(), 1, R.data_ptr(), obj_t.data_ptr(), obj_s.data_ptr(), B, N, X.data_ptr(), st))
        if phase == "sil":
            _chk(lib.vt_fill(dX.data_ptr(), dX.numel(), 0.0, st))
        else:
            self._object_query(f, k, w)
        if B >= 4:
            _chk(lib.vt_accel_loss(X.data_ptr(), B, N * 3, None, float(w[1]), f.terms.ptr("otemp"), dX.data_ptr(), st))
            _chk(lib.vt_velocity_loss(X.data_ptr(), B, N * 3, float(w[2]), f.terms.ptr("ovtemp"), dX.data_ptr(), st))
        acc = 0
        if phase == "sil":
            sil = f.sil
            _chk(lib.vt_rigid_forward(self.obj_verts.data_ptr(), 1, R.data_ptr(), obj_t.data_ptr(), obj_s.data_ptr(), B, NV, f.Vt.data_ptr(), st))
            _chk(lib.vt_sil_forward(f.Vt.data_ptr(), B, NV, self.obj_faces.data_ptr(), nf, sil.K.data_ptr(), sil.size, f.img.data_ptr(), f.fidx.data_ptr(),
                                    f.sws.data_ptr(), st))
            _chk(lib.vt_sil_mask_loss(f.img.data_ptr(), sil.keep.data_ptr(), sil.ref.data_ptr(), f.occ.data_ptr(), B, sil.size, float(w[3]),
                                      f.terms.ptr("mask"), f.per.data_ptr(), f.dimg.data_ptr(), st))
            _chk(lib.vt_sil_backward(f.Vt.data_ptr(), B, NV, self.obj_faces.data_ptr(), nf, sil.K.data_ptr(), sil.size, f.fidx.data_ptr(), f.dimg.data_ptr(),
                                     1e-4, f.sws.data_ptr(), f.dVt.data_ptr(), st))
            _chk(lib.vt_rigid_backward(self.obj_verts.data_ptr(), 1, obj_s.data_ptr(), B, NV, f.dVt.data_ptr(), dR.data_ptr(), dt.data_ptr(), 0, st))
            _chk(lib.vt_sqdiff_loss(obj_t.data_ptr(), 3, f.trans_init.data_ptr(), 3, B, 3, float(B * 3), float(w[4]), f.terms.ptr("trans"), dt.data_ptr(), st))
            acc = 1
        if phase == "joint":
            self._contacts(f, w)
        _chk(lib.vt_rigid_backward(self.obj_points.data_ptr(), 1, obj_s.data_ptr(), B, N, dX.data_ptr(), dR.data_ptr(), dt.data_ptr(), acc, st))
        if phase == "joint" and self.collision_loss:
            if f.cws is None:
                f.Vc = torch.empty(B, NV, 3, device=X.device)
                f.cws = torch.empty((lib.vt_collision_workspace_bytes(B, self.smpl_faces.shape[0]) + 7) // 8, dtype=torch.int64, device=X.device)
            _chk(lib.vt_rigid_forward(self.obj_verts.data_ptr(), 1, R.data_ptr(), obj_t.data_ptr(), obj_s.data_ptr(), B, NV, f.Vc.data_ptr(), st))
            _chk(lib.vt_collision_loss(f.smpl_verts.data_ptr(), f.smpl_verts.shape[1], self.smpl_faces.data_ptr(), self.smpl_faces.shape[0], f.Vc.data_ptr(), NV,
                                       self.obj_faces.data_ptr(), nf, B, 0.5, 8, float(w[6]), f.terms.ptr("collide"), dt.data_ptr(), None, f.cws.data_ptr(), st))
        _chk(lib.vt_so3_project_backward(obj_R.data_ptr(), nz.data_ptr(), B, dR.data_ptr(), f.dM.data_ptr(), st))
        f.adam.step()
        _chk(lib.vt_loss_reduce_and_stop(f.terms.buf.data_ptr(), w.ctypes.data, len(f.terms.names), 1e-4, armed, f.loss_state.data_ptr(), f.stop.data_ptr(),
                                         f.hist.data_ptr(), k, st))

    def _object_step_fused(self, f, phase, k, w, armed):
        lib = _lib(); st = L.stream_ptr(); B, N, NV, nz = f.B, f.N, f.NV, f.noise[k]
        is_sil = phase == "sil"
        X, dX = f.X.data_ptr(), f.dX.data_ptr()
        obj_verts, Vt, dVt = (self.obj_verts.data_ptr(), f.Vt.data_ptr(), f.dVt.data_ptr()) if is_sil else (None, None, None)
        _chk(lib.vt_objstep_head(f.obj_R.data_ptr(), nz.data_ptr(), f.obj_t.data_ptr(), f.obj_s.data_ptr(), B, self.obj_points.data_ptr(), N, X,
                                 obj_verts, NV, Vt, f.R.data_ptr(), f.terms.buf.data_ptr(), 7, f.svd_ws.data_ptr(), st))
        if not is_sil:
            self._object_query(f, k, w)
        tail_temporal = B >= 4 and phase != "joint"
        if B >= 4 and phase == "joint":
            _chk(lib.vt_temporal_loss2(X, B, N * 3, float(w[1]), f.terms.ptr("otemp"), float(w[2]), f.terms.ptr("ovtemp"), dX, 0, st))
        elif is_sil and B < 4:
            _chk(lib.vt_fill(dX, f.dX.numel(), 0.0, st))
        if is_sil:
            sil = f.sil
            _chk(lib.vt_sil_step(Vt, B, NV, self.obj_faces.data_ptr(), self.obj_faces.shape[0], sil.K.data_ptr(), sil.size, sil.keep.data_ptr(),
                                 sil.ref.data_ptr(), f.occ.data_ptr(), float(w[3]), 1e-4, f.terms.ptr("mask"), f.fidx.data_ptr(), f.dimg.data_ptr(),
                                 f.sws.data_ptr(), dVt, st))
        if phase == "joint":
            self._contacts(f, w)
        tail, pre = lib.vt_objstep_tail, ()
        if tail_temporal:
            tail, pre = lib.vt_objstep_tail_temporal, (X, float(w[1]), f.terms.ptr("otemp"), float(w[2]), f.terms.ptr("ovtemp"), int(is_sil))
        _chk(tail(*pre, obj_verts, NV, dVt, self.obj_points.data_ptr(), N, dX, f.obj_s.data_ptr(), B, f.obj_R.data_ptr(), nz.data_ptr(), f.obj_t.data_ptr(),
                  f.trans_init.data_ptr() if is_sil else None, float(w[4]), f.terms.ptr("trans"), f.dR.data_ptr(), f.dt.data_ptr(), f.dM.data_ptr(),
                  *f.adam.object_tail_groups, f.adam.tick(), 0.9, 0.999, 1e-8, f.terms.buf.data_ptr(), w.ctypes.data, len(f.terms.names), 1e-4, armed,
                  f.loss_state.data_ptr(), f.stop.data_ptr(), f.hist.data_ptr(), k, f.ticket.data_ptr(), 0, f.svd_ws.data_ptr(), st))

    def _contact_term(self, contact, X, dX, w, terms):
        _chk(_lib().vt_chamfer_ragged_idx(contact["x"].data_ptr(), contact["offx"].data_ptr(), contact["x"].shape[0], X.data_ptr(), contact["idx_o32"].data_ptr(),
                                          contact["offy"].data_ptr(), contact["idx_o32"].shape[0], contact["P"], w, terms.ptr("contact"), dX.data_ptr(),
                                          contact["ws"].data_ptr(), int(not contact["planned"]), L.stream_ptr()))
        contact["planned"] = True

    def _contacts_once(self, maps, smpl_verts, X, crop_center, body_center, thres=0.08):
        B, N = X.shape[:2]; V = smpl_verts.shape[1]; dev = X.device
        df_o, _, parts_o, _, _ = ops.sifnet_query(self.net, maps, X, crop_center, body_center, head_mask=0b00101)
        df_h, _, _, _, _ = ops.sifnet_query(self.net, maps, smpl_verts, crop_center, body_center, head_mask=0b00001)
        mask_o = df_o[:, 0] < thres
        mask_h = df_h[:, 1] < thres
        lab_o = parts_o.argmax(1)
        lab_h = self.labels.long().unsqueeze(0).expand(B, V)
        oh = torch.zeros(B, 14, device=dev, dtype=torch.long); oo = torch.zeros_like(oh)
        oh.scatter_add_(1, lab_h, mask_h.long()); oo.scatter_add_(1, lab_o, mask_o.long())
        pair = (oh > 0) & (oo > 0)
        P = int(pair.sum().item())
        if P == 0:
            return {"P": 0}
        sel_h = mask_h & pair.gather(1, lab_h); sel_o = mask_o & pair.gather(1, lab_o)
        bh, vh = sel_h.nonzero(as_tuple=True); bo, no = sel_o.nonzero(as_tuple=True)
        cnt_h = (oh * pair).reshape(-1); cnt_o = (oo * pair).reshape(-1)
        keep = pair.reshape(-1)
        ch, co = cnt_h[keep], cnt_o[keep]
        perm = torch.argsort(ch * co, descending=True, stable=True)
        rank_of_key = torch.zeros(B * 14, dtype=torch.long, device=dev)
        rank_of_key[keep.nonzero(as_tuple=True)[0][perm]] = torch.arange(P, device=dev)
        kh = rank_of_key[bh * 14 + lab_h[bh, vh]]; ko = rank_of_key[bo * 14 + lab_o[bo, no]]
        oh_s = torch.sort(kh, stable=True); oo_s = torch.sort(ko, stable=True)
        idx_h = (bh * V + vh)[oh_s.indices]; idx_o = (bo * N + no)[oo_s.indices]
        offx = torch.zeros(P + 1, dtype=torch.int32, device=dev); offy = torch.zeros(P + 1, dtype=torch.int32, device=dev)
        offx[1:] = torch.cumsum(ch[perm], 0).int(); offy[1:] = torch.cumsum(co[perm], 0).int()
        x = smpl_verts.reshape(-1, 3).index_select(0, idx_h).contiguous()
        ws = torch.empty(int(_lib().vt_chamfer_ws_bytes(x.shape[0], idx_o.shape[0], P)), dtype=torch.uint8, device=dev)
        return {"P": P, "x": x, "offx": offx, "offy": offy, "idx_o": idx_o, "idx_o32": idx_o.int().contiguous(), "ws": ws, "planned": False}


class SilSetup:

    def __init__(self, K, keep, ref, size=256):
        self.K, self.keep, self.ref, self.size = K.contiguous(), keep.contiguous(), ref.contiguous(), size
```

vistracker_amd/ops.py:

```python
from __future__ import annotations

import ctypes as C

import numpy as np
import torch

from . import _lib as L


def _f32(t):
    return t.detach().contiguous().float()


def _np32(a):
    return np.ascontiguousarray(np.asarray(a), dtype=np.float32)


class SmplhHandle:

    def __init__(self, model: dict, device="cuda:0"):
        self.device = torch.device(device)
        par = np.asarray(model["parents"]).astype(np.int64).copy()
        par[0] = 0
        par = np.ascontiguousarray(par, dtype=np.int32)
        arrs = [_np32(model[k]) for k in ("v_template", "shapedirs", "posedirs", "J_regressor", "weights")]
        assert arrs[0].shape == (6890, 3) and arrs[1].shape == (6890, 3, 10) and arrs[2].shape == (6890, 3, 459)
        assert arrs[3].shape == (52, 6890) and arrs[4].shape == (6890, 52)
        h = C.c_void_p()
        with torch.cuda.device(self.device):
            L.check(L.lib().vt_smplh_create(C.byref(h), *[a.ctypes.data for a in arrs], par.ctypes.data, L.stream_ptr()))
        self.h = h
        self.faces = np.asarray(model["f"]).astype(np.int64) if "f" in model else None

    def __del__(self):
        try:
            if getattr(self, "h", None):
                L.lib().vt_smplh_destroy(self.h)
        except Exception:
            pass


class _SmplhFn(torch.autograd.Function):
    @staticmethod
    def forward(ctx, handle: SmplhHandle, pose, betas, trans):
        pose, betas, trans = _f32(pose), _f32(betas), _f32(trans)
        B = pose.shape[0]
        dev = pose.device
        verts = torch.empty(B, 6890, 3, device=dev); jtr = torch.empty(B, 52, 3, device=dev)
        vposed = torch.empty(B, 6890, 3, device=dev)
        ws = torch.empty(L.lib().vt_smplh_workspace_floats(B), device=dev)
        L.check(L.lib().vt_smplh_forward(handle.h, L.dptr(pose), L.dptr(betas), L.dptr(trans), B, L.dptr(verts), L.dptr(jtr),
                                         L.dptr(vposed), L.dptr(ws), L.stream_ptr()))
        ctx.handle = handle
        ctx.save_for_backward(pose, betas, vposed, ws)
        ctx.mark_non_differentiable(vposed)
        return verts, jtr, vposed

    @staticmethod
    def backward(ctx, dverts, djtr, _dvp):
        pose, betas, vposed, ws = ctx.saved_tensors
        B = pose.shape[0]
        dev = pose.device
        dverts = torch.zeros(B, 6890, 3, device=dev) if dverts is None else _f32(dverts)
        djtr = None if djtr is None else _f32(djtr)
        scratch = torch.empty(L.lib().vt_smplh_bwd_scratch_floats(B), device=dev)
        dpose = torch.empty(B, 156, device=dev); dbetas = torch.empty(B, 10, device=dev); dtrans = torch.empty(B, 3, device=dev)
        L.check(L.lib().vt_smplh_backward(ctx.handle.h, L.dptr(pose), L.dptr(betas), B, L.dptr(dverts), L.dptr(djtr), L.dptr(vposed),
                                          L.dptr(ws), L.dptr(scratch), L.dptr(dpose), L.dptr(dbetas), L.dptr(dtrans), L.stream_ptr()))
        return None, dpose, dbetas, dtrans


def smplh_forward(handle: SmplhHandle, pose, betas, trans):
    return _SmplhFn.apply(handle, pose, betas, trans)


def rodrigues(aa):
    aa = _f32(aa).reshape(-1, 3)
    R = torch.empty(aa.shape[0], 9, device=aa.device)
    L.check(L.lib().vt_rodrigues_forward(L.dptr(aa), aa.shape[0], L.dptr(R), L.stream_ptr()))
    return R


def rodrigues_bwd(aa, dR):
    aa = _f32(aa).reshape(-1, 3); dR = _f32(dR).reshape(-1, 9)
    d = torch.empty_like(aa)
    L.check(L.lib().vt_rodrigues_backward(L.dptr(aa), aa.shape[0], L.dptr(dR), L.dptr(d), L.stream_ptr()))
    return d


class LandmarkHandle:
    def __init__(self, csr: dict, device="cuda:0"):
        self.K, self.V = csr["shape"]
        ip = np.ascontiguousarray(csr["indptr"], np.int32); ix = np.ascontiguousarray(csr["indices"], np.int32)
        da = _np32(csr["data"])
        h = C.c_void_p()
        with torch.cuda.device(torch.device(device)):
            L.check(L.lib().vt_landmarks_create(C.byref(h), ip.ctypes.data, ix.ctypes.data, da.ctypes.data, self.K, self.V, L.stream_ptr()))
        self.h = h

    def __del__(self):
        try:
            if getattr(self, "h", None):
                L.lib().vt_landmarks_destroy(self.h)
        except Exception:
            pass


class _LandmarkFn(torch.autograd.Function):
    @staticmethod
    def forward(ctx, handle, verts):
        verts = _f32(verts); B = verts.shape[0]
        out = torch.empty(B, handle.K, 3, device=verts.device)
        L.check(L.lib().vt_landmarks_forward(handle.h, L.dptr(verts), B, L.dptr(out), L.stream_ptr()))
        ctx.handle = handle; ctx.B = B
        return out

    @staticmethod
    def backward(ctx, dout):
        dout = _f32(dout)
        dverts = torch.empty(ctx.B, ctx.handle.V, 3, device=dout.device)
        L.check(L.lib().vt_landmarks_backward(ctx.handle.h, L.dptr(dout), ctx.B, L.dptr(dverts), 0, L.stream_ptr()))
        return None, dverts


def landmarks(handle: LandmarkHandle, verts):
    return _LandmarkFn.apply(handle, verts)


class _MahalanobisFn(torch.autograd.Function):
    @staticmethod
    def forward(ctx, x, off, mean, prec):
        x = _f32(x); B, stride = x.shape; n = mean.shape[0]
        val = torch.empty(B, device=x.device)
        L.check(L.lib().vt_mahalanobis(L.dptr(x), B, stride, off, n, L.dptr(mean), L.dptr(prec), L.dptr(val), None, 0.0, L.stream_ptr()))
        ctx.save_for_backward(x, mean, prec); ctx.off = off
        return val

    @staticmethod
    def backward(ctx, dval):
        x, mean, prec = ctx.saved_tensors
        B, stride = x.shape; n = mean.shape[0]
        dx = torch.zeros_like(x); val = torch.empty(B, device=x.device)
        L.check(L.lib().vt_mahalanobis(L.dptr(x), B, stride, ctx.off, n, L.dptr(mean), L.dptr(prec), L.dptr(val), L.dptr(dx), 1.0, L.stream_ptr()))
        return dx * dval.reshape(B, 1), None, None, None


def mahalanobis(x, off, mean, prec):
    return _MahalanobisFn.apply(x, off, mean, prec)


HEADS = ("df", "pca", "parts", "centers", "vis")
HEAD_DIMS = (2, 9, 14, 3, 1)
MAP_ORDER = ("im_feat", "tmpx", "tri_tmpx0", "tri_tmpx1", "tri_tmpx2", "tri_feat0", "tri_feat1", "tri_feat2")
MAP_CHANNELS = (256, 64, 32, 32, 32, 64, 64, 64)
DEFAULT_CAM = (979.7844, 979.840, 1018.952, 779.486, 1200.0)


class SifNetHandle:

    def __init__(self, decoders: dict, cam=DEFAULT_CAM, device="cuda:0"):
        ws, bs = [], []
        for name, k in zip(HEADS, HEAD_DIMS):
            layers = decoders[name]
            assert len(layers) == 4 and tuple(layers[0][0].shape) == (128, 611) and tuple(layers[3][0].shape) == (k, 128)
            for (w, b) in layers:
                ws.append(_np32(w)); bs.append(_np32(b))
        wp = (C.c_void_p * 20)(*[w.ctypes.data for w in ws]); bp = (C.c_void_p * 20)(*[b.ctypes.data for b in bs])
        cam = _np32(cam)
        h = C.c_void_p()
        with torch.cuda.device(torch.device(device)):
            L.check(L.lib().vt_sifnet_create(C.byref(h), wp, bp, cam.ctypes.data, L.stream_ptr()))
        self.h = h; self.cam = cam

    PRECISIONS = {"split-f16": 0, "fp32": 1}

    def set_precision(self, mode: str):
        L.check(L.lib().vt_sifnet_set_precision(self.h, self.PRECISIONS[mode]))
        return self

    @property
    def precision(self) -> str:
        return {v: k for k, v in self.PRECISIONS.items()}[L.lib().vt_sifnet_get_precision(self.h)]

    def __del__(self):
        try:
            if getattr(self, "h", None):
                L.lib().vt_sifnet_destroy(self.h)
        except Exception:
            pass


class FeatureMaps:

    def __init__(self, nhwc: dict):
        self.t = [nhwc[k] for k in MAP_ORDER]
        for t, c in zip(self.t, MAP_CHANNELS):
            assert t.is_cuda and t.is_contiguous() and t.dtype == torch.float32 and t.shape[-1] == c and t.shape[1] == t.shape[2]
        self.B = self.t[0].shape[0]
        self.proj = None
        self.c = L.VtMaps()
        for i, t in enumerate(self.t):
            self.c.maps[i] = t.data_ptr(); self.c.res[i] = t.shape[1]

    ACT_LEVELS = 3

    @property
    def act_level(self) -> int:
        return int(self.c.act_level)

    def set_act_level(self, level: int):
        assert 0 <= level < self.ACT_LEVELS
        self.c.act_level = level
        return self

    @property
    def force_fp32(self) -> bool:
        return bool(self.c.force_fp32)

    def set_force_fp32(self, on: bool = True):
        self.c.force_fp32 = 1 if on else 0
        return self

    def slice(self, start, end):
        fm = FeatureMaps({k: t[start:end] for k, t in zip(MAP_ORDER, self.t)})
        fm.c.act_level = self.c.act_level; fm.c.force_fp32 = self.c.force_fp32
        return fm

    def select(self, idx):
        fm = FeatureMaps({k: t.index_select(0, idx).contiguous() for k, t in zip(MAP_ORDER, self.t)})
        fm.c.act_level = self.c.act_level; fm.c.force_fp32 = self.c.force_fp32
        if self.proj is not None:
            fm.proj = self.proj.view(self.B, -1).index_select(0, idx).reshape(-1).contiguous()
            fm.c.proj = fm.proj.data_ptr(); fm.c.proj_cols = self.c.proj_cols; fm.c.proj_level = self.c.proj_level
        return fm

    def build_projection(self, net):
        h = net.h if hasattr(net, "h") else net.handle.h
        n = L.lib().vt_query_projection_floats(C.byref(self.c), self.B)
        self.proj = torch.empty(n, device=self.t[0].device)
        self.c.proj = None; self.c.proj_cols = 0
        L.check(L.lib().vt_query_build_projection(h, C.byref(self.c), self.B, self.proj.data_ptr(), L.stream_ptr()))
        self.c.proj = self.proj.data_ptr(); self.c.proj_cols = n // (self.B * self.t[0].shape[1] * self.t[0].shape[2])
        self.c.proj_level = self.c.act_level
        return self

    def drop_projection(self):
        self.proj = None; self.c.proj = None; self.c.proj_cols = 0
        return self

    @staticmethod
    def from_nchw(maps: dict, device="cuda:0"):
        out = {}
        for k in MAP_ORDER:
            src = maps[k]
            src = torch.as_tensor(src, dtype=torch.float32).to(device).contiguous()
            B, Cc, H, W = src.shape
            dst = torch.empty(B, H, W, Cc, device=src.device)
            L.check(L.lib().vt_nchw_to_nhwc(L.dptr(src), B, Cc, H, W, L.dptr(dst), L.stream_ptr()))
            out[k] = dst
        return FeatureMaps(out)


class _QueryFn(torch.autograd.Function):
    @staticmethod
    def forward(ctx, net: SifNetHandle, maps: FeatureMaps, pts, cc, bc, head_mask):
        pts, cc, bc = _f32(pts), _f32(cc), _f32(bc)
        B, N = pts.shape[:2]
        outs = [torch.empty(B, k, N, device=pts.device) if (head_mask >> i) & 1 else None for i, k in enumerate(HEAD_DIMS)]
        L.check(L.lib().vt_query_forward(net.h, C.byref(maps.c), L.dptr(pts), L.dptr(cc), L.dptr(bc), B, N,
                                         *[L.dptr(o) for o in outs], L.stream_ptr()))
        ctx.net, ctx.maps, ctx.mask = net, maps, head_mask
        ctx.save_for_backward(pts, cc, bc)
        return tuple(o if o is not None else pts.new_zeros(0) for o in outs)

    @staticmethod
    def backward(ctx, *gs):
        pts, cc, bc = ctx.saved_tensors
        B, N = pts.shape[:2]
        live = [(i, _f32(g)) for i, g in enumerate(gs) if g is not None and (ctx.mask >> i) & 1 and g.numel() > 0]
        total = None
        for s in range(0, len(live), 2):
            args = [None] * 5
            for i, g in live[s:s + 2]:
                args[i] = g
            dpts = torch.empty(B, N, 3, device=pts.device)
            L.check(L.lib().vt_query_backward(ctx.net.h, C.byref(ctx.maps.c), L.dptr(pts), L.dptr(cc), L.dptr(bc), B, N,
                                              *[L.dptr(a) for a in args], L.dptr(dpts), L.stream_ptr()))
            total = dpts if total is None else total + dpts
        if total is None:
            total = torch.zeros(B, N, 3, device=pts.device)
        return None, None, total, None, None, None


def sifnet_query(net, maps, pts, crop_center, body_center, head_mask=31):
    return _QueryFn.apply(net, maps, pts, crop_center, body_center, head_mask)


def sifnet_project_step(net, maps, pts, crop_center, body_center, df_idx, threshold=1.0, out=None, want_target=True):
    pts = _f32(pts.detach()); B, N = pts.shape[:2]
    cc = _f32(crop_center); bc = _f32(body_center)
    out = torch.empty_like(pts) if out is None else out
    dft = torch.empty(B, N, device=pts.device) if want_target else None
    L.check(L.lib().vt_query_project_step(net.h, C.byref(maps.c), L.dptr(pts), L.dptr(cc), L.dptr(bc), B, N, int(df_idx), float(threshold),
                                          L.dptr(out), L.dptr(dft), L.stream_ptr()))
    return out, dft


class _So3Fn(torch.autograd.Function):
    @staticmethod
    def forward(ctx, M, noise):
        M = _f32(M); B = M.shape[0]
        noise = None if noise is None else _f32(noise)
        R = torch.empty(B, 3, 3, device=M.device)
        L.check(L.lib().vt_so3_project_forward(L.dptr(M), L.dptr(noise), B, L.dptr(R), L.stream_ptr()))
        ctx.save_for_backward(M, noise if noise is not None else M.new_zeros(0)); ctx.has_noise = noise is not None
        return R

    @staticmethod
    def backward(ctx, dR):
        M, noise = ctx.saved_tensors
        dR = _f32(dR); dM = torch.empty_like(M)
        L.check(L.lib().vt_so3_project_backward(L.dptr(M), L.dptr(noise) if ctx.has_noise else None, M.shape[0], L.dptr(dR), L.dptr(dM), L.stream_ptr()))
        return dM, None


def so3_project(M, noise=None):
    return _So3Fn.apply(M, noise)


class _RigidFn(torch.autograd.Function):
    @staticmethod
    def forward(ctx, X0, R, t, s):
        X0, R, t, s = _f32(X0), _f32(R), _f32(t), _f32(s)
        B = R.shape[0]; shared = int(X0.dim() == 2); N = X0.shape[-2]
        X = torch.empty(B, N, 3, device=R.device)
        L.check(L.lib().vt_rigid_forward(L.dptr(X0), shared, L.dptr(R), L.dptr(t), L.dptr(s), B, N, L.dptr(X), L.stream_ptr()))
        ctx.save_for_backward(X0, s); ctx.shared = shared
        return X

    @staticmethod
    def backward(ctx, dX):
        X0, s = ctx.saved_tensors
        dX = _f32(dX); B, N = dX.shape[:2]
        dR = torch.empty(B, 3, 3, device=dX.device); dt = torch.empty(B, 3, device=dX.device)
        L.check(L.lib().vt_rigid_backward(L.dptr(X0), ctx.shared, L.dptr(s), B, N, L.dptr(dX), L.dptr(dR), L.dptr(dt), 0, L.stream_ptr()))
        return None, dR, dt, None


def rigid_transform(X0, R, t, s):
    return _RigidFn.apply(X0, R, t, s)


class _StencilFn(torch.autograd.Function):
    @staticmethod
    def forward(ctx, v, kind, elem_w):
        v2 = _f32(v).reshape(v.shape[0], -1)
        B, D = v2.shape
        term = torch.zeros(1, dtype=torch.float64, device=v.device)
        if kind == "accel":
            L.check(L.lib().vt_accel_loss(L.dptr(v2), B, D, L.dptr(elem_w), 0.0, L.dptr(term), None, L.stream_ptr()))
        else:
            L.check(L.lib().vt_velocity_loss(L.dptr(v2), B, D, 0.0, L.dptr(term), None, L.stream_ptr()))
        ctx.save_for_backward(v2, elem_w if elem_w is not None else v2.new_zeros(0))
        ctx.kind, ctx.shape, ctx.has_w = kind, v.shape, elem_w is not None
        return term.float().reshape(())

    @staticmethod
    def backward(ctx, g):
        v2, w = ctx.saved_tensors
        B, D = v2.shape
        dv = torch.zeros_like(v2)
        if ctx.kind == "accel":
            L.check(L.lib().vt_accel_loss(L.dptr(v2), B, D, L.dptr(w) if ctx.has_w else None, 1.0, None, L.dptr(dv), L.stream_ptr()))
        else:
            L.check(L.lib().vt_velocity_loss(L.dptr(v2), B, D, 1.0, None, L.dptr(dv), L.stream_ptr()))
        return (dv * g).reshape(ctx.shape), None, None


def accel_loss(v, elem_w=None):
    return _StencilFn.apply(v, "accel", elem_w)


def velocity_loss(v):
    return _StencilFn.apply(v, "velocity", None)


class _ChamferFn(torch.autograd.Function):
    @staticmethod
    def forward(ctx, x, y, offx, offy):
        x, y = _f32(x), _f32(y); P = offx.numel() - 1
        term = torch.zeros(1, dtype=torch.float64, device=x.device)
        L.check(L.lib().vt_chamfer_ragged(L.dptr(x), L.dptr(offx), L.dptr(y), L.dptr(offy), P, 0.0, L.dptr(term), None, None, L.stream_ptr()))
        ctx.save_for_backward(x, y, offx, offy)
        return term.float().reshape(())

    @staticmethod
    def backward(ctx, g):
        x, y, offx, offy = ctx.saved_tensors
        dx = torch.zeros_like(x); dy = torch.zeros_like(y)
        L.check(L.lib().vt_chamfer_ragged(L.dptr(x), L.dptr(offx), L.dptr(y), L.dptr(offy), offx.numel() - 1, 1.0, None, L.dptr(dx), L.dptr(dy), L.stream_ptr()))
        return dx * g, dy * g, None, None


def chamfer_ragged(x, y, offx, offy):
    return _ChamferFn.apply(x, y, offx, offy)


def collision_loss(smpl_verts, smpl_faces, obj_verts, obj_faces, sigma=0.5, max_collisions=8, gscale=0.0, want_pairs=False):
    sv, ov = _f32(smpl_verts), _f32(obj_verts)
    sf = smpl_faces.to(torch.int32).contiguous(); of = obj_faces.to(torch.int32).contiguous()
    B = sv.shape[0]; dev = sv.device
    ws = torch.empty((L.lib().vt_collision_workspace_bytes(B, sf.shape[0]) + 7) // 8, dtype=torch.int64, device=dev)
    term = torch.zeros(1, dtype=torch.float64, device=dev); dt = torch.zeros(B, 3, device=dev)
    npairs = torch.zeros(B, dtype=torch.int32, device=dev) if want_pairs else None
    L.check(L.lib().vt_collision_loss(L.dptr(sv), sv.shape[1], L.dptr(sf), sf.shape[0], L.dptr(ov), ov.shape[1], L.dptr(of), of.shape[0], B, float(sigma),
                                      int(max_collisions), float(gscale), L.dptr(term), L.dptr(dt), L.dptr(npairs), L.dptr(ws), L.stream_ptr()))
    return (term.float().reshape(()), dt, npairs) if want_pairs else (term.float().reshape(()), dt)


def _frames(t, name):
    if not torch.is_tensor(t) or not t.is_cuda:
        raise L.VtError(f"{name}: a device tensor expected; there is no CPU path")
    t = _f32(t)
    single = t.dim() == 2
    if single:
        t = t[None]
    if t.dim() != 3 or t.shape[-1] != 3 or t.shape[1] == 0:
        raise L.VtError(f"{name}: (B,K,3) or (K,3) with K > 0 expected, got {tuple(t.shape)}")
    return t.contiguous(), single


def check_faces(faces, n_verts):
    f = torch.as_tensor(faces)
    if f.dim() != 2 or f.shape[1] != 3 or f.shape[0] == 0 or f.dtype.is_floating_point:
        raise L.VtError(f"faces: (NF,3) integers with NF > 0 expected, got {tuple(f.shape)} {f.dtype}")
    lo, hi = int(f.min()), int(f.max())
    if lo < 0 or hi >= n_verts:
        raise L.VtError(f"faces: vertex indices span [{lo}, {hi}] but the mesh has {n_verts} vertices")
    return f.to(torch.int32).contiguous()


def point_mesh_distance(points, verts, faces, want_closest=True, want_face=True, validate=True, culling=True, n_tests=None):
    p, single = _frames(points, "points")
    v, vsingle = _frames(verts, "verts")
    if single != vsingle or p.shape[0] != v.shape[0] or p.device != v.device:
        raise L.VtError(f"point_mesh_distance: points {tuple(p.shape)} and verts {tuple(v.shape)} must share the frame axis and the device")
    B, N = p.shape[:2]; NV = v.shape[1]
    f = check_faces(faces, NV) if validate else faces
    if f.dtype != torch.int32 or f.device != p.device:
        f = f.to(device=p.device, dtype=torch.int32)
    f = f.contiguous(); NF = f.shape[0]
    dev = p.device
    with torch.cuda.device(dev):
        ws = torch.empty((L.lib().vt_point_mesh_workspace_bytes(B, NF) + 15) // 16, 2, dtype=torch.int64, device=dev)
        dist = torch.empty(B, N, device=dev)
        closest = torch.empty(B, N, 3, device=dev) if want_closest else None
        face_id = torch.empty(B, N, dtype=torch.int32, device=dev) if want_face else None
        if culling and n_tests is None:
            L.check(L.lib().vt_point_mesh_distance(L.dptr(p), N, L.dptr(v), NV, L.dptr(f), NF, B, L.dptr(dist), L.dptr(closest), L.dptr(face_id), L.dptr(ws),
                                                   L.stream_ptr()))
        else:
            if n_tests is not None and (n_tests.dtype != torch.int64 or n_tests.numel() != 1):
                raise L.VtError("point_mesh_distance: n_tests is a (1,) int64 device tensor")
            L.check(L.lib().vt_point_mesh_distance_ex(L.dptr(p), N, L.dptr(v), NV, L.dptr(f), NF, B, L.dptr(dist), L.dptr(closest), L.dptr(face_id), L.dptr(ws),
                                                      0 if culling else 1, L.dptr(n_tests), L.stream_ptr()))
    if single:
        dist, closest, face_id = dist[0], (closest[0] if want_closest else None), (face_id[0] if want_face else None)
    return dist, closest, face_id


def nearest_vertex(points, verts, want_dist=True):
    p, single = _frames(points, "points")
    v, vsingle = _frames(verts, "verts")
    if single != vsingle or p.shape[0] != v.shape[0] or p.device != v.device:
        raise L.VtError(f"nearest_vertex: points {tuple(p.shape)} and verts {tuple(v.shape)} must share the frame axis and the device")
    B, N = p.shape[:2]; dev = p.device
    with torch.cuda.device(dev):
        vid = torch.empty(B, N, dtype=torch.int32, device=dev)
        vd = torch.empty(B, N, device=dev) if want_dist else None
        L.check(L.lib().vt_nearest_vertex(L.dptr(p), N, L.dptr(v), v.shape[1], B, L.dptr(vid), L.dptr(vd), L.stream_ptr()))
    return (vid[0], vd[0] if want_dist else None) if single else (vid, vd)


LOSS_WEIGHTS = (1.0, 1.0, 0.006, 500.0, 1000.0, 1000.0)
LOSS_SLOTS = ("df_h", "df_o", "parts", "pca", "vis", "obj_center")
LOSS_SLOT_WEIGHT = (0, 1, 2, 3, 5, 4)
VIS_LOSSES = {"l1": 0, "l2": 1}
_LOSS_WK = {}


def _loss_dev(t, name):
    if not torch.is_tensor(t) or not t.is_cuda:
        raise L.VtError(f"sifnet_loss_head: {name} must be a device tensor; there is no CPU path")
    return t


def _loss_preds(preds):
    if len(preds) == 0:
        raise L.VtError("sifnet_loss_head: no predictions")
    if not torch.is_tensor(preds[0]):
        stacks = [tuple(p) for p in preds]
        if any(len(p) != 5 for p in stacks):
            raise L.VtError("sifnet_loss_head: every stack is a (df, pca, parts, centers, vis) tuple")
        for p in stacks:
            for t, name in zip(p, HEADS):
                _loss_dev(t, name)
        B, N = stacks[0][0].shape[0], stacks[0][0].shape[-1]
        heads = [torch.stack([p[i].reshape(B, k, N) for p in stacks]) if len(stacks) > 1 else stacks[0][i].reshape(1, B, k, N) for i, k in enumerate(HEAD_DIMS)]
    else:
        if len(preds) != 5:
            raise L.VtError("sifnet_loss_head: five prediction tensors (df, pca, parts, centers, vis) expected")
        for t, name in zip(preds, HEADS):
            _loss_dev(t, name)
        N = preds[0].shape[-1]
        if preds[0].dim() not in (3, 4):
            raise L.VtError(f"sifnet_loss_head: df is (S,B,2,N) or (B,2,N), got {tuple(preds[0].shape)}")
        S, B = (1, preds[0].shape[0]) if preds[0].dim() == 3 else tuple(preds[0].shape[:2])
        heads = [t.reshape(S, B, k, N) for t, k in zip(preds, HEAD_DIMS)]
    S, B, _, N = heads[0].shape
    if B == 0 or N == 0:
        raise L.VtError(f"sifnet_loss_head: B = {B}, N = {N}")
    for t, k, name in zip(heads, HEAD_DIMS, HEADS):
        if tuple(t.shape) != (S, B, k, N) or t.dtype != torch.float32:
            raise L.VtError(f"sifnet_loss_head: {name} is float32 ({S},{B},{k},{N}), got {t.dtype} {tuple(t.shape)}")
    return [t.contiguous() for t in heads]


class _LossHeadFn(torch.autograd.Function):
    @staticmethod
    def forward(ctx, df, pca, parts, centers, vis, labels, per_frame, max_dist, weights, vis_loss):
        heads = (df, pca, parts, centers, vis)
        S, B, _, N = df.shape
        dev = df.device
        want = any(ctx.needs_input_grad[:5])
        with torch.cuda.device(dev):
            grads = [torch.empty_like(t) if want and ctx.needs_input_grad[i] else None for i, t in enumerate(heads)]
            terms = torch.empty(6, dtype=torch.float64, device=dev)
            ws = torch.empty(L.lib().vt_sifnet_loss_head_ws_bytes(B, N) // 8, dtype=torch.float64, device=dev)
            w = (C.c_double * 6)(*weights)
            L.check(L.lib().vt_sifnet_loss_head(*[L.dptr(t) for t in heads], S, B, N, *[L.dptr(t) for t in labels], int(per_frame), float(max_dist), w,
                                                int(vis_loss), 1.0, L.dptr(terms), *[L.dptr(g) for g in grads], L.dptr(ws), L.stream_ptr()))
        ctx.grads = grads
        key = (dev.index, weights)
        if key not in _LOSS_WK:
            if len(_LOSS_WK) > 16:
                _LOSS_WK.clear()
            _LOSS_WK[key] = torch.tensor([float(weights[i]) for i in LOSS_SLOT_WEIGHT], dtype=torch.float64, device=dev)
        wk = _LOSS_WK[key]
        losses_all = terms * wk
        ctx.mark_non_differentiable(terms, losses_all)
        return losses_all.sum(), losses_all, terms

    @staticmethod
    def backward(ctx, g, _gl, _gt):
        g = g.to(torch.float32)
        return tuple(None if d is None else d * g for d in ctx.grads) + (None,) * 5


def sifnet_loss_head(preds, df_h, df_o, parts_gt, pca_gt, obj_center, visibility, max_dist=5.0, weights=LOSS_WEIGHTS, vis_loss="l2", validate=False,
                     want_terms=False):
    heads = _loss_preds(preds)
    S, B, _, N = heads[0].shape
    dev = heads[0].device
    if vis_loss not in VIS_LOSSES:
        raise L.VtError(f"sifnet_loss_head: unknown vis_loss {vis_loss!r} (l1 or l2)")
    if len(weights) != 6:
        raise L.VtError("sifnet_loss_head: six loss weights expected")
    for t, name in ((df_h, "df_h"), (df_o, "df_o"), (parts_gt, "parts_gt"), (pca_gt, "pca_gt"), (obj_center, "obj_center"), (visibility, "visibility")):
        if _loss_dev(t, name).device != dev:
            raise L.VtError(f"sifnet_loss_head: {name} on {t.device}, the predictions on {dev}")
    if tuple(df_h.shape) != (B, N) or tuple(df_o.shape) != (B, N) or tuple(parts_gt.shape) != (B, N):
        raise L.VtError(f"sifnet_loss_head: df_h, df_o, parts_gt are ({B},{N}), got {tuple(df_h.shape)}, {tuple(df_o.shape)}, {tuple(parts_gt.shape)}")
    if validate:
        lo, hi = float(parts_gt.min()), float(parts_gt.max())
        if lo < 0 or hi > HEAD_DIMS[2] - 1:
            raise L.VtError(f"sifnet_loss_head: part labels span [{lo:g}, {hi:g}], outside [0, {HEAD_DIMS[2]})")
    frame = {"pca_gt": (pca_gt, 9), "obj_center": (obj_center, 3), "visibility": (visibility, 1)}
    kinds = {}
    for name, (t, k) in frame.items():
        if t.numel() == B * k * N and (N > 1 or t.dim() > (1 if k == 1 else 2)):
            kinds[name] = False
        elif t.numel() == B * k:
            kinds[name] = True
        else:
            raise L.VtError(f"sifnet_loss_head: {name} holds {B} x {k} x {N} values per point or {B} x {k} per frame, got {tuple(t.shape)}")
    per_frame = all(kinds.values())
    lab = []
    for name, (t, k) in frame.items():
        t = _f32(t)
        if kinds[name] and not per_frame:
            t = t.reshape(B, k, 1).expand(B, k, N)
        lab.append(t.reshape(B, k) if per_frame else t.reshape(B, k, N).contiguous())
    labels = (_f32(df_h), _f32(df_o), parts_gt.detach().to(torch.int32).contiguous(), *lab)
    error, losses_all, terms = _LossHeadFn.apply(*heads, labels, per_frame, max_dist, tuple(float(w) for w in weights), VIS_LOSSES[vis_loss])
    return (error, losses_all, terms) if want_terms else (error, losses_all)


STATE_DICT_MODULES = {"df": "df", "pca": "pca_predictor", "parts": "part_predictor", "centers": "center_predictor", "vis": "visib_predictor"}
STATE_DICT_LAYERS = (0, 2, 4, 6)


class DecoderParams:

    def __init__(self, flat, cam=DEFAULT_CAM):
        lib = L.lib()
        n = int(lib.vt_decoder_param_floats())
        if not torch.is_tensor(flat) or flat.dtype != torch.float32 or tuple(flat.shape) != (n,):
            raise L.VtError(f"DecoderParams: a float32 tensor of {n} values expected")
        self.flat = flat.detach().contiguous().requires_grad_(True)
        self.cam = _np32(cam)
        self.views, data = {}, self.flat.detach()
        for h, (name, k) in enumerate(zip(HEADS, HEAD_DIMS)):
            for l in range(4):
                shape = (k if l == 3 else 128, MAP_CHANNELS_TOTAL if l == 0 else 128)
                ow, ob = int(lib.vt_decoder_param_offset(h, l, 0)), int(lib.vt_decoder_param_offset(h, l, 1))
                self.views[(name, l, "weight")] = data[ow:ow + shape[0] * shape[1]].view(shape)
                self.views[(name, l, "bias")] = data[ob:ob + shape[0]]
        if sum(v.numel() for v in self.views.values()) != n:
            raise L.VtError("DecoderParams: the library's offsets do not tile the parameter buffer")

    @classmethod
    def from_decoders(cls, decoders: dict, cam=DEFAULT_CAM, device="cuda:0"):
        p = cls(torch.zeros(int(L.lib().vt_decoder_param_floats())), cam)
        for name in HEADS:
            if len(decoders[name]) != 4:
                raise L.VtError(f"DecoderParams: {name} has {len(decoders[name])} layers, 4 expected")
            for l, (w, b) in enumerate(decoders[name]):
                for kind, a in (("weight", w), ("bias", b)):
                    v = p.views[(name, l, kind)]
                    a = torch.as_tensor(_np32(a))
                    if tuple(a.shape) != tuple(v.shape):
                        raise L.VtError(f"DecoderParams: {name} layer {l} {kind} is {tuple(v.shape)}, got {tuple(a.shape)}")
                    v.copy_(a)
        return cls(p.flat.detach().to(device), cam)

    def to_decoders(self) -> dict:
        host = DecoderParams(self.flat.detach().cpu(), self.cam)
        return {name: [(host.views[(name, l, "weight")].numpy().copy(), host.views[(name, l, "bias")].numpy().copy()) for l in range(4)] for name in HEADS}

    def state_dict(self, prefix: str = "") -> dict:
        out = {}
        for name in HEADS:
            for l, i in enumerate(STATE_DICT_LAYERS):
                out[f"{prefix}{STATE_DICT_MODULES[name]}.{i}.weight"] = self.views[(name, l, "weight")].clone().unsqueeze(-1)
                out[f"{prefix}{STATE_DICT_MODULES[name]}.{i}.bias"] = self.views[(name, l, "bias")].clone()
        return out

    def load_state_dict(self, sd: dict):
        with torch.no_grad():
            for name in HEADS:
                for l, i in enumerate(STATE_DICT_LAYERS):
                    for kind in ("weight", "bias"):
                        key = f"{STATE_DICT_MODULES[name]}.{i}.{kind}"
                        t = sd.get(key, sd.get("module." + key))
                        if t is None:
                            raise KeyError(key)
                        v = self.views[(name, l, kind)]
                        t = torch.as_tensor(t, dtype=torch.float32)
                        if t.numel() != v.numel():
                            raise L.VtError(f"DecoderParams.load_state_dict: {key} holds {v.numel()} values, got {tuple(t.shape)}")
                        v.copy_(t.reshape(v.shape))
        return self


MAP_CHANNELS_TOTAL = sum(MAP_CHANNELS) + 3


def _train_maps(maps):
    maps = [maps] if isinstance(maps, FeatureMaps) else list(maps)
    if not maps or not all(isinstance(m, FeatureMaps) for m in maps):
        raise L.VtError("sifnet_query_train: maps is a FeatureMaps or a list of them, one per stack")
    return maps


class _QueryTrainFn(torch.autograd.Function):
    @staticmethod
    def forward(ctx, flat, cam, maps, pts, cc, bc, chunk_points, *map_tensors):
        B, N = pts.shape[:2]
        outs = []
        with torch.cuda.device(flat.device):
            for m in maps:
                o = [torch.empty(B, k, N, device=flat.device) for k in HEAD_DIMS]
                L.check(L.lib().vt_decoder_train_forward(L.dptr(flat), cam.ctypes.data, C.byref(m.c), L.dptr(pts), L.dptr(cc), L.dptr(bc), B, N,
                                                         *[L.dptr(t) for t in o], L.stream_ptr()))
                outs += o
        ctx.cam, ctx.maps, ctx.chunk = cam, maps, chunk_points
        ctx.set_materialize_grads(False)
        ctx.save_for_backward(flat, pts, cc, bc)
        return tuple(outs)

    @staticmethod
    def backward(ctx, *gs):
        flat, pts, cc, bc = ctx.saved_tensors
        B, N = pts.shape[:2]
        want_w, want_m = ctx.needs_input_grad[0], ctx.needs_input_grad[7:]
        lib = L.lib()
        with torch.cuda.device(flat.device):
            dflat = torch.empty_like(flat) if want_w else None
            dmaps = [None] * len(want_m)
            if not any(want_m):
                ws = torch.empty(int(lib.vt_decoder_weight_grads_ws_bytes(B, N, ctx.chunk)) // 4 + 4, device=flat.device)
            else:
                ws = torch.empty(int(lib.vt_decoder_grads_ws_bytes(B, N, ctx.chunk, 1)) // 4 + 4, device=flat.device)
            for s, m in enumerate(ctx.maps):
                g = [None if t is None else _f32(t) for t in gs[5 * s:5 * s + 5]]
                if not any(want_m):
                    if want_w:
                        L.check(lib.vt_decoder_weight_grads(L.dptr(flat), ctx.cam.ctypes.data, C.byref(m.c), L.dptr(pts), L.dptr(cc), L.dptr(bc), B, N,
                                                            *[L.dptr(t) for t in g], L.dptr(dflat), 1 if s else 0, int(ctx.chunk), L.dptr(ws), L.stream_ptr()))
                    continue
                dm = L.VtMaps()
                for i, t in enumerate(m.t):
                    dm.res[i] = t.shape[1]
                    if want_m[8 * s + i]:
                        dmaps[8 * s + i] = torch.empty_like(t)
                        dm.maps[i] = dmaps[8 * s + i].data_ptr()
                if not want_w and not any(want_m[8 * s:8 * s + 8]):
                    continue
                L.check(lib.vt_decoder_grads(L.dptr(flat), ctx.cam.ctypes.data, C.byref(m.c), L.dptr(pts), L.dptr(cc), L.dptr(bc), B, N,
                                             *[L.dptr(t) for t in g], L.dptr(dflat), 1 if s else 0, C.byref(dm), 0, int(ctx.chunk), L.dptr(ws), L.stream_ptr()))
        return (dflat, None, None, None, None, None, None, *dmaps)


def sifnet_query_train(params: DecoderParams, maps, pts, crop_center, body_center, chunk_points=0, train_decoders=True):
    maps = _train_maps(maps)
    if not isinstance(params, DecoderParams):
        raise L.VtError("sifnet_query_train: params is an ops.DecoderParams")
    for t, name in ((pts, "points"), (crop_center, "crop_center"), (body_center, "body_center")):
        if not torch.is_tensor(t) or not t.is_cuda:
            raise L.VtError(f"sifnet_query_train: {name} must be a device tensor; there is no CPU path")
    if pts.requires_grad:
        raise L.VtError("sifnet_query_train: the points are data here (no gradient flows to them); detach them, or use sifnet_query for the gradient to the points")
    pts, cc, bc = _f32(pts), _f32(crop_center), _f32(body_center)
    B, N = pts.shape[:2]
    if pts.dim() != 3 or pts.shape[2] != 3 or tuple(cc.shape) != (B, 2) or tuple(bc.shape) != (B, 3) or any(m.B != B for m in maps):
        raise L.VtError(f"sifnet_query_train: points (B,N,3), crop_center (B,2), body_center (B,3), maps of B frames; got {tuple(pts.shape)}, {tuple(cc.shape)}, "
                        f"{tuple(bc.shape)}, {[m.B for m in maps]}")
    flat = params.flat if train_decoders else params.flat.detach()
    outs = _QueryTrainFn.apply(flat, params.cam, maps, pts, cc, bc, int(chunk_points), *[t for m in maps for t in m.t])
    return [(outs[5 * s], outs[5 * s + 1].view(B, 3, 3, N), outs[5 * s + 2], outs[5 * s + 3], outs[5 * s + 4]) for s in range(len(maps))]


CONV_BLOCK_PARAMS = ("w1", "w2", "w3", "gamma1", "gamma2", "gamma3", "beta1", "beta2", "beta3", "wproj", "gamma4", "beta4")
CONV_BLOCK_BACKWARD_ARGS = (("dy", "x", "raw", "stats1", "stats2", "stats3") + CONV_BLOCK_PARAMS + ("B", "H", "W", "cin", "c1", "c2", "c3")
                            + ("d_x", "dW1", "dW2", "dW3", "dgamma1", "dbeta1", "dgamma2", "dbeta2", "dgamma3", "dbeta3", "dgamma4", "dbeta4", "dWproj")
                            + ("workspace", "accumulate", "stream"))


def conv_block_backward_raw(dy, x, raw, stats, params, want=None, out=None, accumulate=0, ws=None):
    lib = L.lib()
    B, cin, H, W = x.shape
    c1, c2, c3 = (int(params[k].shape[0]) for k in ("w1", "w2", "w3"))
    proj = params.get("wproj") is not None
    names = ["d_x", "dW1", "dW2", "dW3", "dgamma1", "dbeta1", "dgamma2", "dbeta2", "dgamma3", "dbeta3"] + (["dgamma4", "dbeta4", "dWproj"] if proj else [])
    like = {"d_x": x, "dW1": params["w1"], "dW2": params["w2"], "dW3": params["w3"], "dWproj": params.get("wproj")}
    for i in "1234":
        like["dgamma" + i] = like["dbeta" + i] = params.get("gamma" + i)
    want = names if want is None else [n for n in names if n in want]
    res = dict(out or {})
    for n in want:
        if n not in res:
            res[n] = torch.empty_like(like[n], memory_format=torch.channels_last if n == "d_x" else torch.contiguous_format)
    if ws is None:
        nbytes = int(lib.vt_conv_block_backward_workspace(B, H, W, cin, c1, c2, c3))
        if nbytes < 0:
            raise L.VtError(f"conv_block_backward: unsupported block shape B={B} H={H} W={W} {cin}->({c1},{c2},{c3})")
        ws = torch.empty(nbytes // 4 + 4, device=x.device)
    ptr = lambda t: None if t is None else t.data_ptr()
    order = ("d_x", "dW1", "dW2", "dW3", "dgamma1", "dbeta1", "dgamma2", "dbeta2", "dgamma3", "dbeta3", "dgamma4", "dbeta4", "dWproj")
    with torch.cuda.device(x.device):
        L.check(lib.vt_conv_block_backward(dy.data_ptr(), x.data_ptr(), raw.data_ptr(), *[s.data_ptr() for s in stats], *[ptr(params.get(k)) for k in CONV_BLOCK_PARAMS],
                                           B, H, W, cin, c1, c2, c3, *[ptr(res.get(n)) if n in want else None for n in order],
                                           ws.data_ptr(), int(accumulate), L.stream_ptr()))
    return res


class _ConvBlockTrainFn(torch.autograd.Function):
    @staticmethod
    def forward(ctx, blk, x, *tensors):
        lib = L.lib()
        p = dict(zip(CONV_BLOCK_PARAMS, tensors))
        B, Cin, H, W = x.shape
        couts = [int(p[k].shape[0]) for k in ("w1", "w2", "w3")]
        Ct, Cr = sum(couts), couts[0] + couts[1]
        with torch.cuda.device(x.device):
            h3, h1 = blk.conv_handles(x.device)
            tiles = lib.vt_conv3x3_tiles(H, W)
            st = getattr(x, "_vt_stats", None)
            if st is not None:
                if not st[2]:
                    L.check(lib.vt_groupnorm_finalize(st[0].data_ptr(), st[1], B, H * W, Cin, 32, 1e-5, L.stream_ptr()))
                    st[2] = True
                ws = st[0]
            else:
                ws = torch.empty(lib.vt_groupnorm_workspace_doubles(B, H * W, Cin, 32), dtype=torch.float64, device=x.device)
                L.check(lib.vt_groupnorm_stats(x.data_ptr(), Cin, 0, B, H * W, Cin, 32, 1e-5, ws.data_ptr(), L.stream_ptr()))
            res = x
            if h1 is not None:
                res = torch.empty(B, Ct, H, W, device=x.device, memory_format=torch.channels_last)
                L.check(lib.vt_conv1x1_forward(h1, x.data_ptr(), Cin, 0, ws.data_ptr(), p["gamma4"].data_ptr(), p["beta4"].data_ptr(), 32, B, H, W,
                                               res.data_ptr(), Ct, 0, None, Ct, 0, None, 32, L.stream_ptr()))
            raw = torch.empty(B, Cr, H, W, device=x.device, memory_format=torch.channels_last)
            fin = torch.empty(B, Ct, H, W, device=x.device, memory_format=torch.channels_last)
            ws_fin = torch.empty(B * 32 + tiles * B * Ct * 2, dtype=torch.float64, device=x.device)
            src, cstride, coff, off = x, Cin, 0, 0
            stats = [ws]
            for i, co in enumerate(couts):
                last = i == 2
                ws_out = None if last else torch.empty(B * 32 + tiles * B * co * 2, dtype=torch.float64, device=x.device)
                L.check(lib.vt_conv3x3_forward_block_stats(h3[i], src.data_ptr(), cstride, coff, stats[-1].data_ptr(), p[f"gamma{i + 1}"].data_ptr(),
                                                           p[f"beta{i + 1}"].data_ptr(), 32, B, H, W, None if last else raw.data_ptr(), Cr, 0 if last else off,
                                                           res.data_ptr(), Ct, off, fin.data_ptr(), Ct, off, None if last else ws_out.data_ptr(), 32,
                                                           ws_fin.data_ptr(), 32, L.stream_ptr()))
                if not last:
                    L.check(lib.vt_groupnorm_finalize(ws_out.data_ptr(), tiles, B, H * W, co, 32, 1e-5, L.stream_ptr()))
                    stats.append(ws_out)
                src, cstride, coff = raw, Cr, off
                off += co
        ctx.save_for_backward(x, raw, *stats, *[t for t in tensors if t is not None])
        ctx.present = [t is not None for t in tensors]
        ctx.mark_non_differentiable(ws_fin)
        return fin, ws_fin

    @staticmethod
    def backward(ctx, dy, _):
        sv = ctx.saved_tensors
        x, raw, stats = sv[0], sv[1], sv[2:5]
        it = iter(sv[5:])
        p = {k: (next(it) if have else None) for k, have in zip(CONV_BLOCK_PARAMS, ctx.present)}
        need = dict(zip(("d_x",) + CONV_BLOCK_PARAMS, ctx.needs_input_grad[1:]))
        gname = {"d_x": "d_x", "w1": "dW1", "w2": "dW2", "w3": "dW3", "wproj": "dWproj"}
        for i in "1234":
            gname["gamma" + i], gname["beta" + i] = "dgamma" + i, "dbeta" + i
        want = [gname[k] for k, n in need.items() if n and (k == "d_x" or p[k] is not None)]
        dy = dy.float().contiguous(memory_format=torch.channels_last)
        g = conv_block_backward_raw(dy, x, raw, stats, p, want=want)
        return (None, g.get("d_x"), *[g.get(gname[k]) if need[k] and p[k] is not None else None for k in CONV_BLOCK_PARAMS])


def conv_block_train(x, params):
    if not (torch.is_tensor(x) and x.is_cuda and x.dim() == 4):
        raise L.VtError("conv_block_train: x must be a (B,C,H,W) device tensor; there is no CPU path")
    B, Cin, H, W = x.shape
    tensors = params.tensors()
    couts = [int(tensors[i].shape[0]) for i in range(3)]
    if int(L.lib().vt_conv_block_backward_workspace(B, H, W, Cin, *couts)) < 0 or int(tensors[0].shape[1]) != Cin or (tensors[9] is None) != (Cin == sum(couts)):
        raise L.VtError(f"conv_block_train: block {Cin}->{couts} at {H}x{W} is not served (H % 8 == 0, W % 16 == 0, widths in {{32, 64, 128}}, Cin % 32 == 0 up to 256)")
    xc = x if x.dtype == torch.float32 and x.is_contiguous(memory_format=torch.channels_last) else x.float().contiguous(memory_format=torch.channels_last)
    if xc is not x and hasattr(x, "_vt_stats"):
        xc._vt_stats = x._vt_stats
    fin, ws_fin = _ConvBlockTrainFn.apply(params, xc, *tensors)
    fin._vt_stats = [ws_fin, int(L.lib().vt_conv3x3_tiles(H, W)), False]
    return fin


class _SilFn(torch.autograd.Function):
    @staticmethod
    def forward(ctx, verts, faces, K, size, eps):
        verts, K = _f32(verts), _f32(K); B, NV = verts.shape[:2]; NF = faces.shape[0]
        img = torch.empty(B, size, size, device=verts.device)
        fidx = torch.empty(B, size, size, dtype=torch.int32, device=verts.device)
        ws = torch.empty(L.lib().vt_sil_workspace_floats(B, NV, NF, size), device=verts.device)
        L.check(L.lib().vt_sil_forward(L.dptr(verts), B, NV, L.dptr(faces), NF, L.dptr(K), size, L.dptr(img), L.dptr(fidx), L.dptr(ws), L.stream_ptr()))
        ctx.save_for_backward(verts, faces, K, fidx, ws); ctx.size, ctx.eps = size, eps
        return img

    @staticmethod
    def backward(ctx, dimg):
        verts, faces, K, fidx, ws = ctx.saved_tensors
        B, NV = verts.shape[:2]
        dimg = _f32(dimg)
        dverts = torch.empty_like(verts)
        L.check(L.lib().vt_sil_backward(L.dptr(verts), B, NV, L.dptr(faces), faces.shape[0], L.dptr(K), ctx.size, L.dptr(fidx),
                                        L.dptr(dimg), ctx.eps, L.dptr(ws), L.dptr(dverts), L.stream_ptr()))
        return dverts, None, None, None, None


def silhouette(verts, faces, K, size=256, eps=1e-4):
    return _SilFn.apply(verts, faces, K, size, eps)


def div255_table():
    return (np.arange(256, dtype=np.float64) / 255.0).astype(np.float32)


_DIV255 = {}


def _u8(t, name):
    if t.dtype != torch.uint8:
        raise L.VtError(f"{name}: uint8 expected, got {t.dtype}")
    return t


def mask_bbox(pm, om, thres=127):
    B, H, W = pm.shape
    if tuple(om.shape) != (B, H, W):
        raise L.VtError(f"mask_bbox: masks of {tuple(pm.shape)} and {tuple(om.shape)}")
    p, o = L.dptr(_u8(pm, "pm")), L.dptr(_u8(om, "om"))
    box = torch.empty(B, 4, dtype=torch.int32, device=pm.device)
    L.check(L.lib().vt_mask_bbox(p, o, B, H, W, int(thres), L.dptr(box), L.stream_ptr()))
    return box


def crop_resize_compose(rgb, pm, om, corners, crop_size, out_size, out=None):
    B, H, W = pm.shape
    S, cs = int(out_size), int(crop_size)
    if tuple(rgb.shape) != (B, H, W, 3) or tuple(om.shape) != (B, H, W):
        raise L.VtError(f"crop_resize_compose: rgb {tuple(rgb.shape)}, masks {tuple(pm.shape)} and {tuple(om.shape)}")
    ptrs = [L.dptr(_u8(t, n)) for t, n in ((rgb, "rgb"), (pm, "pm"), (om, "om"))]
    c = np.ascontiguousarray(corners, dtype=np.int64).reshape(-1, 4)
    ext = np.stack([c[:, 2] - c[:, 0], c[:, 3] - c[:, 1]], 1)
    if c.shape[0] != B or (ext <= 0).any() or (np.abs(ext - cs) > 1).any() or np.abs(c).max(initial=0) >= 2 ** 29:
        raise ValueError(f"crop_resize_compose: corners {c.tolist()} are not {B} crops of size {cs}")
    if out is None:
        out = torch.empty(B, 5, S, S, device=rgb.device)
    elif out.dtype != torch.float32 or out.dim() != 4 or out.shape[0] != B or out.shape[1] < 5 or tuple(out.shape[2:]) != (S, S):
        raise L.VtError(f"crop_resize_compose: out {tuple(out.shape)} {out.dtype} for {B} crops of {S} x {S}")
    dev = rgb.device.index
    if dev not in _DIV255:
        _DIV255[dev] = torch.as_tensor(div255_table(), device=rgb.device)
    cd = torch.as_tensor(c.astype(np.int32), device=rgb.device)
    L.check(L.lib().vt_crop_resize_compose(*ptrs, B, H, W, L.dptr(cd), cs, S, L.dptr(_DIV255[dev]), L.dptr(out), out.stride(0), L.stream_ptr()))
    return out


def resize_panel_u8(src, frames, H, size, col0, pw, out, out_off, out_row_stride):
    d = np.ascontiguousarray(frames, dtype=np.int64).reshape(-1, 6)
    if src.dim() == 0 or src.stride(-1) != 1 or out.device != src.device:
        raise L.VtError("resize_panel_u8: src must have packed bytes and live on out's device")
    off = torch.as_tensor(np.ascontiguousarray(out_off, dtype=np.int64).reshape(-1), device=out.device) if not torch.is_tensor(out_off) else out_off
    if off.dtype != torch.int64 or off.numel() != d.shape[0]:
        raise L.VtError(f"resize_panel_u8: {off.numel()} {off.dtype} offsets for {d.shape[0]} frames")
    L.dptr(_u8(out, "out")); L.dptr(off)
    if not src.is_cuda or src.device.index != torch.cuda.current_device():
        raise L.VtError("resize_panel_u8: src must be a tensor of the current device; there is no CPU route")
    span = 1 + sum((n - 1) * st for n, st in zip(src.shape, src.stride()))
    L.check(L.lib().vt_resize_panel_u8(_u8(src, "src").data_ptr(), span, d.ctypes.data, d.shape[0], int(H), int(size), int(col0), int(pw), out.data_ptr(),
                                       off.data_ptr(), int(out_row_stride), L.stream_ptr()))
    return out


def _offsets(off, n, device, name):
    off = torch.as_tensor(np.ascontiguousarray(off, dtype=np.int64).reshape(-1), device=device) if not torch.is_tensor(off) else off
    if off.dtype != torch.int64 or off.numel() != n:
        raise L.VtError(f"{name}: {off.numel()} {off.dtype} offsets for {n} views")
    return off


def overlay_panel_u8(rgb, alpha, out, src_off, dst_off, row0, nrows, col0, ncols, out_row_stride, opacity):
    B, S = rgb.shape[0], rgb.shape[1]
    if tuple(rgb.shape) != (B, S, S, 3) or tuple(alpha.shape) != (B, S, S) or rgb.dtype != torch.float32 or alpha.dtype != torch.float32:
        raise L.VtError(f"overlay_panel_u8: rgb {tuple(rgb.shape)} {rgb.dtype}, alpha {tuple(alpha.shape)} {alpha.dtype}")
    so, do = _offsets(src_off, B, rgb.device, "overlay_panel_u8"), _offsets(dst_off, B, rgb.device, "overlay_panel_u8")
    L.check(L.lib().vt_overlay_panel_u8(L.dptr(rgb), L.dptr(alpha), B, S, int(row0), int(nrows), int(col0), int(ncols), L.dptr(_u8(out, "out")), L.dptr(so),
                                        L.dptr(do), int(out_row_stride), float(opacity), L.stream_ptr()))
    return out


def _span(t):
    return 1 + sum((n - 1) * st for n, st in zip(t.shape, t.stride()))


def mask_score(fidx, rows, F, nf_body, nf_obj, pm, om, frames, thres=127, count=None):
    B, s = fidx.shape[0], fidx.shape[1]
    d = np.ascontiguousarray(frames, dtype=np.int64).reshape(-1, 8)
    if fidx.dim() != 3 or fidx.shape[2] != s or fidx.dtype != torch.int32 or d.shape[0] != B:
        raise L.VtError(f"mask_score: fidx {tuple(fidx.shape)} {fidx.dtype} with {d.shape[0]} mask descriptors")
    for m, name in ((pm, "pm"), (om, "om")):
        if not m.is_cuda or m.device != fidx.device or m.device.index != torch.cuda.current_device() or m.numel() == 0:
            raise L.VtError(f"mask_score: {name} must be a non-empty tensor of fidx's (the current) device; there is no CPU route")
        _u8(m, name)
    if count is None:
        count = torch.empty(B, 2, 4, dtype=torch.int32, device=fidx.device)
    elif count.dtype != torch.int32 or tuple(count.shape) != (B, 2, 4):
        raise L.VtError(f"mask_score: count {tuple(count.shape)} {count.dtype} for {B} views")
    L.check(L.lib().vt_mask_score(L.dptr(fidx), B, s, int(rows), int(F), int(nf_body), int(nf_obj), pm.data_ptr(), _span(pm), om.data_ptr(), _span(om),
                                  d.ctypes.data, int(thres), L.dptr(count), L.stream_ptr()))
    return count


class FusedAdam:

    def __init__(self, params, lr=1e-3, betas=(0.9, 0.999), eps=1e-8, stop_flag=None):
        if isinstance(params[0], dict):
            self.params = [p["params"] for p in params]; self.lrs = [p.get("lr", lr) for p in params]
        else:
            self.params = list(params); self.lrs = [lr] * len(self.params)
        self.betas, self.eps, self.t = betas, eps, 0
        self.m = [torch.zeros_like(p) for p in self.params]; self.v = [torch.zeros_like(p) for p in self.params]
        self.stop_flag = stop_flag

    def zero_grad(self):
        for p in self.params:
            p.grad = None

    def step(self, grads=None):
        self.t += 1
        for i, p in enumerate(self.params):
            g = p.grad if grads is None else grads[i]
            if g is None:
                continue
            g = g.contiguous()
            L.check(L.lib().vt_adam_step(L.dptr(p.data), L.dptr(g), L.dptr(self.m[i]), L.dptr(self.v[i]), p.numel(), self.t, self.lrs[i],
                                         self.betas[0], self.betas[1], self.eps, L.dptr(self.stop_flag), L.stream_ptr()))
```

Baseline: 151.4.

## Precompute frozen hand-pose blend prefix and skip frozen columns in SMPL-H backward

```diff
diff --git a/include/vistracker.h b/include/vistracker.h
--- a/include/vistracker.h
+++ b/include/vistracker.h
@@ -35,6 +35,13 @@
 int vt_smplh_backward(const vt_smplh *h, const float *pose, const float *betas, int B, const float *dverts,
                       const float *djtr, const float *v_posed, const float *ws, float *scratch,
                       float *dpose, float *dbetas, float *dtrans, void *stream);
+
+long vt_smplh_prefix_floats(int B);
+int vt_smplh_prefix(const vt_smplh *h, const float *pose, int B, float *ws, float *prefix, void *stream);
+int vt_smplh_forward_prefixed(const vt_smplh *h, const float *pose, const float *betas, const float *trans, int B, const float *prefix,
+                              float *verts, float *jtr, float *v_posed, float *ws, void *stream);
+int vt_smplh_backward_free(const vt_smplh *h, const float *pose, int B, const float *dverts, const float *djtr, const float *v_posed,
+                           const float *ws, float *scratch, int n_free_pose_cols, float *dpose, float *dbetas, float *dtrans, void *stream);
 
 int vt_rodrigues_forward(const float *aa, int n, float *R, void *stream);
 int vt_rodrigues_backward(const float *aa, int n, const float *dR, float *daa, void *stream);
diff --git a/vistracker_amd/_lib.py b/vistracker_amd/_lib.py
--- a/vistracker_amd/_lib.py
+++ b/vistracker_amd/_lib.py
@@ -28,6 +28,10 @@
     "vt_smplh_bwd_scratch_floats": (cl, [ci]),
     "vt_smplh_forward": (ci, [vp, fp, fp, fp, ci, fp, fp, fp, fp, vp]),
     "vt_smplh_backward": (ci, [vp, fp, fp, ci, fp, fp, fp, fp, fp, fp, fp, fp, vp]),
+    "vt_smplh_prefix_floats": (cl, [ci]),
+    "vt_smplh_prefix": (ci, [vp, fp, ci, fp, fp, vp]),
+    "vt_smplh_forward_prefixed": (ci, [vp, fp, fp, fp, ci, fp, fp, fp, fp, fp, vp]),
+    "vt_smplh_backward_free": (ci, [vp, fp, ci, fp, fp, fp, fp, fp, ci, fp, fp, fp, vp]),
     "vt_rodrigues_forward": (ci, [fp, ci, fp, vp]),
     "vt_rodrigues_backward": (ci, [fp, ci, fp, fp, vp]),
     "vt_landmarks_create": (ci, [C.POINTER(vp), vp, vp, vp, ci, ci, vp]),
diff --git a/vistracker_amd/csrc/smplh.hip b/vistracker_amd/csrc/smplh.hip
--- a/vistracker_amd/csrc/smplh.hip
+++ b/vistracker_amd/csrc/smplh.hip
@@ -9,6 +9,19 @@
 #define NVT_ 27
 #define KQ_ 472
 #define NQ_ 480
+#define J_LIVE_ 22
+#define NP_LIVE_ ((J_LIVE_ - 1) * 9)
+#define KF_ 272
+#define NT_LIVE_ 13
+#define NQ_HAND_ (NT_LIVE_ * 16)
+#define NP_NUM_ (J_ * 3)
+__host__ __device__ constexpr int kq_of_posemap(int p) { return p < NP_LIVE_ ? KF_ + p : p - NP_LIVE_; }
+__host__ __device__ constexpr int nq_of_posemap(int p) { return p < NP_LIVE_ ? p : NQ_HAND_ + (p - NP_LIVE_); }
+#define KQ_BETA0 (KF_ + NP_LIVE_)
+#define KQ_TEMPLATE (KQ_ - 1)
+#define NQ_BETA0 NP_LIVE_
+static_assert(KF_ % 8 == 0 && KF_ >= NP_ - NP_LIVE_ && KQ_BETA0 + NB_ <= KQ_TEMPLATE && (KQ_ - KF_) % 8 == 0, "K order of Q_kcv");
+static_assert(NQ_BETA0 + NB_ <= NQ_HAND_ && NQ_HAND_ + (NP_ - NP_LIVE_) <= NQ_, "N order of Q_t");
 typedef float f32x4 __attribute__((ext_vector_type(4)));
 #define MFMA16(a, b, c) __builtin_amdgcn_mfma_f32_16x16x4f32((a), (b), (c), 0, 0, 0)
 
@@ -98,17 +111,31 @@
 __global__ __launch_bounds__(64) void smplh_pose_kernel(const float *__restrict__ pose, const float *__restrict__ betas,
                                                         const float *__restrict__ trans, const float *__restrict__ J_t,
                                                         const float *__restrict__ J_s, SmplParents par,
-                                                        float *__restrict__ ws, float *__restrict__ jtr, const int *skip)
+                                                        float *__restrict__ ws, float *__restrict__ jtr, int rod_lo, int rod_hi, int chain,
+                                                        const int *skip)
 {
     VT_SKIP_RETURN(skip);
     __shared__ float sR[J_ * 9], sJ[J_ * 3], sG[J_ * 12];
     const int b = blockIdx.x, j = threadIdx.x;
     float *w = ws + (size_t)b * WS_FRAME;
     if (j < J_) {
-        float t[3] = {pose[(b * J_ + j) * 3], pose[(b * J_ + j) * 3 + 1], pose[(b * J_ + j) * 3 + 2]}, R[9];
-        rodrigues_fwd(t, R, nullptr);
-#pragma unroll
-        for (int e = 0; e < 9; e++) { sR[j * 9 + e] = R[e]; w[WS_R + j * 9 + e] = R[e]; }
+        float R[9];
+        if (j >= rod_lo && j < rod_hi) {
+            float t[3] = {pose[(b * J_ + j) * 3], pose[(b * J_ + j) * 3 + 1], pose[(b * J_ + j) * 3 + 2]};
+            rodrigues_fwd(t, R, nullptr);
+#pragma unroll
+            for (int e = 0; e < 9; e++) w[WS_R + j * 9 + e] = R[e];
+        } else if (chain) {
+#pragma unroll
+            for (int e = 0; e < 9; e++) R[e] = w[WS_R + j * 9 + e];
+        }
+        if (chain) {
+#pragma unroll
+            for (int e = 0; e < 9; e++) sR[j * 9 + e] = R[e];
+        }
+    }
+    if (!chain) return;
+    if (j < J_) {
 #pragma unroll
         for (int c = 0; c < 3; c++) {
             float a = J_t[j * 3 + c];
@@ -164,12 +191,15 @@
 #define AXS 516
 #define SAS 628
 #define FWD_R0 (FWD_FB * AXS > 8 * SAS ? FWD_FB * AXS : 8 * SAS)
+template <int MODE>
 __global__ __launch_bounds__(256) void smplh_verts_kernel(const float *__restrict__ Q_kcv, const float *__restrict__ W_jv,
                                                           const float *__restrict__ betas, const float *__restrict__ trans,
                                                           const float *__restrict__ ws, int B,
-                                                          float *__restrict__ verts, float *__restrict__ v_posed, const float *__restrict__ W_sp, int nnz, const int *skip)
+                                                          float *__restrict__ verts, float *__restrict__ v_posed, const float *__restrict__ W_sp, int nnz,
+                                                          float *prefix, const int *skip)
 {
     VT_SKIP_RETURN(skip);
+    constexpr int K0 = MODE == 2 ? KF_ : 0, K1 = MODE == 1 ? KF_ : KQ_;
     extern __shared__ __attribute__((aligned(16))) float lds[];
     float *sAx = lds;
     float *sA = lds;
@@ -178,34 +208,40 @@
     float *sTr = sW + (nnz > 0 ? 2 * SP_K * 64 : J_ * 64);
     const int tid = threadIdx.x, wave = tid >> 6, lane = tid & 63, q = lane >> 4, j = lane & 15;
     const int b0 = blockIdx.y * FWD_FB, v = blockIdx.x * 64 + wave * 16 + j;
-    for (int k = tid; k < KQ_; k += 256) {
-        const int e9 = k % 9;
-        const float sub = (k < NP_ && (e9 == 0 || e9 == 4 || e9 == 8)) ? 1.f : 0.f;
+    for (int k = K0 + tid; k < K1; k += 256) {
+        int p = -1, l = -1;
+        if (k < NP_ - NP_LIVE_) p = NP_LIVE_ + k;
+        else if (k >= KF_ && k < KQ_BETA0) p = k - KF_;
+        else if (k >= KQ_BETA0 && k < KQ_BETA0 + NB_) l = k - KQ_BETA0;
+        const int e9 = p % 9;
+        const float sub = (p >= 0 && (e9 == 0 || e9 == 4 || e9 == 8)) ? 1.f : 0.f;
         float val[FWD_FB];
 #pragma unroll
         for (int f = 0; f < FWD_FB; f++) {
             const int b = min(b0 + f, B - 1);
-            if (k < NP_) val[f] = ws[(size_t)b * WS_FRAME + WS_R + 9 + k];
-            else if (k < NP_ + NB_) val[f] = betas[b * NB_ + (k - NP_)];
-            else val[f] = (k == NP_ + NB_) ? 1.f : 0.f;
+            if (p >= 0) val[f] = ws[(size_t)b * WS_FRAME + WS_R + 9 + p];
+            else if (l >= 0) val[f] = betas[b * NB_ + l];
+            else val[f] = (k == KQ_TEMPLATE) ? 1.f : 0.f;
         }
 #pragma unroll
         for (int f = 0; f < FWD_FB; f++) sAx[f * AXS + k] = val[f] - sub;
     }
-    if (nnz > 0) {
+    if (MODE == 1) {
+    } else if (nnz > 0) {
         for (int i = tid; i < nnz * 64; i += 256) {
             sW[i] = W_sp[(size_t)(i >> 6) * VP_ + blockIdx.x * 64 + (i & 63)];
             sW[SP_K * 64 + i] = W_sp[(size_t)(SP_K + (i >> 6)) * VP_ + blockIdx.x * 64 + (i & 63)];
         }
     } else
         for (int i = tid; i < J_ * 64; i += 256) sW[i] = W_jv[(i >> 6) * VP_ + blockIdx.x * 64 + (i & 63)];
-    if (tid < FWD_FB * 3) { const int f = tid / 3, b = min(b0 + f, B - 1); sTr[tid] = trans[b * 3 + tid % 3]; }
+    if (MODE != 1 && tid < FWD_FB * 3) { const int f = tid / 3, b = min(b0 + f, B - 1); sTr[tid] = trans[b * 3 + tid % 3]; }
     __syncthreads();
 
     f32x4 acc[3];
-#pragma unroll
-    for (int c = 0; c < 3; c++) acc[c] = (f32x4){0.f, 0.f, 0.f, 0.f};
-    constexpr int NS = KQ_ / 8;
+    f32x4 *pre4 = reinterpret_cast<f32x4 *>(prefix) + ((size_t)blockIdx.y * gridDim.x + blockIdx.x) * 3 * 256 + tid;
+#pragma unroll
+    for (int c = 0; c < 3; c++) acc[c] = MODE == 2 ? pre4[c * 256] : (f32x4){0.f, 0.f, 0.f, 0.f};
+    constexpr int S0 = K0 / 8, NS = K1 / 8;
     float bq[FWD_PF][2][3];
 #define FWD_LOADQ(slot_, s_)                                                                     \
     {                                                                                            \
@@ -214,18 +250,23 @@
             _Pragma("unroll") for (int c = 0; c < 3; c++) bq[slot_][e][c] = qk[(size_t)(e * 3 + c) * VP_]; \
     }
 #pragma unroll
-    for (int s = 0; s < FWD_PF; s++) FWD_LOADQ(s, s)
-#pragma unroll
-    for (int s = 0; s < NS; s++) {
+    for (int s = 0; s < FWD_PF; s++) FWD_LOADQ(s, S0 + s)
+#pragma unroll
+    for (int s = S0; s < NS; s++) {
         const float2 av = *reinterpret_cast<const float2 *>(sAx + j * AXS + 8 * s + 2 * q);
 #pragma unroll
-        for (int c = 0; c < 3; c++) acc[c] = MFMA16(av.x, bq[s % FWD_PF][0][c], acc[c]);
-#pragma unroll
-        for (int c = 0; c < 3; c++) acc[c] = MFMA16(av.y, bq[s % FWD_PF][1][c], acc[c]);
-        if (s + FWD_PF < NS) FWD_LOADQ(s % FWD_PF, s + FWD_PF)
+        for (int c = 0; c < 3; c++) acc[c] = MFMA16(av.x, bq[(s - S0) % FWD_PF][0][c], acc[c]);
+#pragma unroll
+        for (int c = 0; c < 3; c++) acc[c] = MFMA16(av.y, bq[(s - S0) % FWD_PF][1][c], acc[c]);
+        if (s + FWD_PF < NS) FWD_LOADQ((s - S0) % FWD_PF, s + FWD_PF)
         __builtin_amdgcn_sched_barrier(0);
     }
 #undef FWD_LOADQ
+    if (MODE == 1) {
+#pragma unroll
+        for (int c = 0; c < 3; c++) pre4[c * 256] = acc[c];
+        return;
+    }
     __syncthreads();
 #pragma unroll
     for (int r = 0; r < 4; r++)
@@ -372,13 +413,14 @@
 #define BL_NW 1
 #endif
 #define BL_AS 132
-__global__ __launch_bounds__(256) void smplh_bwd_blend_kernel(const float *__restrict__ Q_p, const float *__restrict__ dvp_g, int B,
+__global__ __launch_bounds__(256) void smplh_bwd_blend_kernel(const float *__restrict__ Q_p, const float *__restrict__ dvp_g, int B, int ntiles,
                                                               float *__restrict__ part3, const int *skip)
 {
     VT_SKIP_RETURN(skip);
     __shared__ __attribute__((aligned(16))) float sA[BL_M * BL_AS];
     const int tid = threadIdx.x, wave = tid >> 6, lane = tid & 63, q = lane >> 4, j = lane & 15;
     const int ks = blockIdx.x, m0 = blockIdx.z * BL_M, nt0 = blockIdx.y * (4 * BL_NW) + wave * BL_NW;
+    const bool has_tile = nt0 < ntiles;
     f32x4 acc[6][BL_NW];
 #pragma unroll
     for (int mt = 0; mt < 6; mt++)
@@ -395,13 +437,14 @@
             *reinterpret_cast<float4 *>(sA + row * BL_AS + c4 * 4) = v;
         }
         __syncthreads();
+        if (!has_tile) continue;
 #pragma unroll
         for (int g = 0; g < 8; g++) {
             const size_t kg = (size_t)ks * KG_SLAB + c * 8 + g;
             float bq[BL_NW][4];
 #pragma unroll
             for (int n = 0; n < BL_NW; n++) {
-                const float4 fq = Q4[(kg * (NQ_ / 16) + min(nt0 + n, NQ_ / 16 - 1)) * 64 + lane];
+                const float4 fq = Q4[(kg * (NQ_ / 16) + min(nt0 + n, ntiles - 1)) * 64 + lane];
                 bq[n][0] = fq.x; bq[n][1] = fq.y; bq[n][2] = fq.z; bq[n][3] = fq.w;
             }
 #pragma unroll
@@ -424,7 +467,7 @@
                 float *dst = part3 + ((size_t)ks * B + b) * NQ_;
 #pragma unroll
                 for (int n = 0; n < BL_NW; n++)
-                    if (nt0 + n < NQ_ / 16) dst[(nt0 + n) * 16 + j] = acc[mt][n][r];
+                    if (nt0 + n < ntiles) dst[(nt0 + n) * 16 + j] = acc[mt][n][r];
             }
         }
     }
@@ -433,8 +476,8 @@
 __global__ __launch_bounds__(256) void smplh_bwd_frame_kernel(const float *__restrict__ pose, const float *__restrict__ J_s,
                                                               SmplParents par, const float *__restrict__ ws,
                                                               const float *__restrict__ part, const float *__restrict__ part3,
-                                                              const float *__restrict__ djtr, int B, float *__restrict__ dpose, float *__restrict__ dbetas,
-                                                              float *__restrict__ dtrans, const int *skip)
+                                                              const float *__restrict__ djtr, int B, int n_free, float *__restrict__ dpose,
+                                                              float *__restrict__ dbetas, float *__restrict__ dtrans, const int *skip)
 {
     VT_SKIP_RETURN(skip);
     __shared__ float red[PT_N], red3[NQ_];
@@ -451,7 +494,8 @@
         for (int t = 0; t < NVT_; t++) s += part[((size_t)t * B + b) * PT_N + i];
         red[i] = s;
     }
-    for (int i = tid; i < NQ_; i += 256) {
+    const int ncol = n_free < NP_NUM_ ? NQ_HAND_ : NQ_, jfree = n_free / 3;
+    for (int i = tid; i < ncol; i += 256) {
         float s = 0.f;
 #pragma unroll 9
         for (int t = 0; t < NKS_; t++) s += part3[((size_t)t * B + b) * NQ_ + i];
@@ -503,16 +547,16 @@
     }
     if (tid < 3) { for (int c = 0; c < 3; c++) sdR[3 * tid + c] += sdG[tid * 4 + c]; sdJ[tid] += sdG[tid * 4 + 3]; }
     __syncthreads();
-    if (tid < J_) {
+    if (tid < jfree) {
         const int j = tid;
         float g[9], t[3] = {pose[(b * J_ + j) * 3], pose[(b * J_ + j) * 3 + 1], pose[(b * J_ + j) * 3 + 2]}, d[3];
 #pragma unroll
-        for (int e = 0; e < 9; e++) g[e] = sdR[9 * j + e] + (j >= 1 ? red3[(j - 1) * 9 + e] : 0.f);
+        for (int e = 0; e < 9; e++) g[e] = sdR[9 * j + e] + (j >= 1 ? red3[nq_of_posemap((j - 1) * 9 + e)] : 0.f);
         rodrigues_bwd(t, g, d);
         dpose[(b * J_ + j) * 3] = d[0]; dpose[(b * J_ + j) * 3 + 1] = d[1]; dpose[(b * J_ + j) * 3 + 2] = d[2];
     } else if (tid >= 64 && tid < 64 + NB_) {
         const int l = tid - 64;
-        float s = red3[NP_ + l];
+        float s = red3[NQ_BETA0 + l];
         for (int i = 0; i < J_ * 3; i++) s += J_s[i * NB_ + l] * sdJ[i];
         dbetas[b * NB_ + l] = s;
     } else if (tid >= 128 && tid < 131) {
@@ -551,10 +595,12 @@
         for (int k = 0; k < NP_ + NB_ + 1; k++) {
             const float val = k < NP_ ? posedirs[((size_t)v * 3 + c) * NP_ + k]
                             : (k < NP_ + NB_ ? shapedirs[((size_t)v * 3 + c) * NB_ + (k - NP_)] : v_template[v * 3 + c]);
-            Q_kcv[(size_t)(k * 3 + c) * VP_ + v] = val;
-            {
+            const int kq = k < NP_ ? kq_of_posemap(k) : (k < NP_ + NB_ ? KQ_BETA0 + (k - NP_) : KQ_TEMPLATE);
+            Q_kcv[(size_t)(kq * 3 + c) * VP_ + v] = val;
+            if (k < NP_ + NB_) {
+                const int nq = k < NP_ ? nq_of_posemap(k) : NQ_BETA0 + (k - NP_);
                 const size_t kr = (size_t)v * 3 + c, g = kr >> 4, qq = (kr & 15) >> 2, ss = kr & 3;
-                Q_t[((g * (NQ_ / 16) + (k >> 4)) * 64 + qq * 16 + (k & 15)) * 4 + ss] = val;
+                Q_t[((g * (NQ_ / 16) + (nq >> 4)) * 64 + qq * 16 + (nq & 15)) * 4 + ss] = val;
             }
         }
     }
@@ -609,17 +655,67 @@
 
 #define BWD_FB 6
 
+extern "C" long vt_smplh_prefix_floats(int B) { return (long)((B + FWD_FB - 1) / FWD_FB) * (VP_ / 64) * 3 * 256 * 4; }
+
+#define FWD_LDS_FLOATS(w_) (FWD_R0 + FWD_FB * 64 * 3 + (w_) + FWD_FB * 3)
+static int smplh_forward_launch(int mode, const vt_smplh *h, const float *pose, const float *betas, const float *trans, int B, float *verts, float *jtr,
+                                float *v_posed, float *ws, float *prefix, hipStream_t st)
+{
+    const int *skip = mode == 1 ? nullptr : vt_skip_flag_of(st);
+    hipLaunchKernelGGL(smplh_pose_kernel, dim3(B), dim3(64), 0, st, pose, betas, trans, h->J_t, h->J_s, h->par, ws, jtr, mode == 1 ? J_LIVE_ : 0,
+                       mode == 2 ? J_LIVE_ : J_, mode == 1 ? 0 : 1, skip);
+    VT_LAUNCH_CHECK();
+    const size_t lds_f = sizeof(float) * FWD_LDS_FLOATS(h->nnz > 0 ? 2 * SP_K * 64 : J_ * 64), lds_max = sizeof(float) * FWD_LDS_FLOATS(J_ * 64);
+    const dim3 grid(VP_ / 64, (B + FWD_FB - 1) / FWD_FB);
+    if (mode == 0) {
+        VT_LDS_LIMIT(smplh_verts_kernel<0>, lds_max);
+        hipLaunchKernelGGL(smplh_verts_kernel<0>, grid, dim3(256), lds_f, st, h->Q_kcv, h->W_jv, betas, trans, ws, B, verts, v_posed, h->W_sp, h->nnz, prefix, skip);
+    } else if (mode == 1) {
+        VT_LDS_LIMIT(smplh_verts_kernel<1>, sizeof(float) * FWD_R0);
+        hipLaunchKernelGGL(smplh_verts_kernel<1>, grid, dim3(256), sizeof(float) * FWD_R0, st, h->Q_kcv, h->W_jv, betas, trans, ws, B, verts, v_posed, h->W_sp,
+                           h->nnz, prefix, skip);
+    } else {
+        VT_LDS_LIMIT(smplh_verts_kernel<2>, lds_max);
+        hipLaunchKernelGGL(smplh_verts_kernel<2>, grid, dim3(256), lds_f, st, h->Q_kcv, h->W_jv, betas, trans, ws, B, verts, v_posed, h->W_sp, h->nnz, prefix, skip);
+    }
+    VT_LAUNCH_CHECK();
+    return VT_OK;
+}
+
 extern "C" int vt_smplh_forward(const vt_smplh *h, const float *pose, const float *betas, const float *trans, int B,
                                 float *verts, float *jtr, float *v_posed, float *ws, void *stream)
 {
     VT_REQUIRE(h && pose && betas && trans && verts && v_posed && ws && B > 0, "vt_smplh_forward: null argument or B <= 0");
-    hipStream_t st = vt_stream(stream); const int *skip = vt_skip_flag_of(st);
-    hipLaunchKernelGGL(smplh_pose_kernel, dim3(B), dim3(64), 0, st, pose, betas, trans, h->J_t, h->J_s, h->par, ws, jtr, skip);
+    return smplh_forward_launch(0, h, pose, betas, trans, B, verts, jtr, v_posed, ws, nullptr, vt_stream(stream));
+}
+
+extern "C" int vt_smplh_prefix(const vt_smplh *h, const float *pose, int B, float *ws, float *prefix, void *stream)
+{
+    VT_REQUIRE(h && pose && ws && prefix && B > 0, "vt_smplh_prefix: null argument or B <= 0");
+    return smplh_forward_launch(1, h, pose, nullptr, nullptr, B, nullptr, nullptr, nullptr, ws, prefix, vt_stream(stream));
+}
+
+extern "C" int vt_smplh_forward_prefixed(const vt_smplh *h, const float *pose, const float *betas, const float *trans, int B, const float *prefix,
+                                         float *verts, float *jtr, float *v_posed, float *ws, void *stream)
+{
+    VT_REQUIRE(h && pose && betas && trans && prefix && verts && v_posed && ws && B > 0, "vt_smplh_forward_prefixed: null argument or B <= 0");
+    return smplh_forward_launch(2, h, pose, betas, trans, B, verts, jtr, v_posed, ws, const_cast<float *>(prefix), vt_stream(stream));
+}
+
+static int smplh_backward_launch(const vt_smplh *h, const float *pose, int B, const float *dverts, const float *djtr, const float *v_posed, const float *ws,
+                                 float *scratch, int n_free, float *dpose, float *dbetas, float *dtrans, hipStream_t st)
+{
+    const int *skip = vt_skip_flag_of(st);
+    const size_t lds = sizeof(float) * (256 * 13 + BWD_FB * 624);
+    float *dvp_g = scratch + (size_t)NVT_ * B * PT_N, *part3 = dvp_g + (size_t)B * KTOT_;
+    const int ntiles = n_free < NP_NUM_ ? NT_LIVE_ : NQ_ / 16;
+    VT_LDS_LIMIT(smplh_bwd_tile_kernel<BWD_FB>, lds);
+    hipLaunchKernelGGL(smplh_bwd_tile_kernel<BWD_FB>, dim3(NVT_, (B + BWD_FB - 1) / BWD_FB), dim3(256), lds, st, h->W_v64, ws, v_posed, dverts, B, scratch, dvp_g, skip);
     VT_LAUNCH_CHECK();
-    const size_t lds_f = sizeof(float) * (FWD_R0 + FWD_FB * 64 * 3 + (h->nnz > 0 ? 2 * SP_K * 64 : J_ * 64) + FWD_FB * 3);
-    VT_LDS_LIMIT(smplh_verts_kernel, sizeof(float) * (FWD_R0 + FWD_FB * 64 * 3 + J_ * 64 + FWD_FB * 3));
-    hipLaunchKernelGGL(smplh_verts_kernel, dim3(VP_ / 64, (B + FWD_FB - 1) / FWD_FB), dim3(256), lds_f, st, h->Q_kcv, h->W_jv, betas, trans, ws, B,
-                       verts, v_posed, h->W_sp, h->nnz, skip);
+    hipLaunchKernelGGL(smplh_bwd_blend_kernel, dim3(NKS_, (ntiles + 4 * BL_NW - 1) / (4 * BL_NW), (B + BL_M - 1) / BL_M), dim3(256), 0, st, h->Q_t, dvp_g, B, ntiles,
+                       part3, skip);
+    VT_LAUNCH_CHECK();
+    hipLaunchKernelGGL(smplh_bwd_frame_kernel, dim3(B), dim3(256), 0, st, pose, h->J_s, h->par, ws, scratch, part3, djtr, B, n_free, dpose, dbetas, dtrans, skip);
     VT_LAUNCH_CHECK();
     return VT_OK;
 }
@@ -630,17 +726,17 @@
 {
     (void)betas;
     VT_REQUIRE(h && pose && dverts && v_posed && ws && scratch && dpose && dbetas && dtrans && B > 0, "vt_smplh_backward: null argument or B <= 0");
-    hipStream_t st = vt_stream(stream); const int *skip = vt_skip_flag_of(st);
-    const size_t lds = sizeof(float) * (256 * 13 + BWD_FB * 624);
-    float *dvp_g = scratch + (size_t)NVT_ * B * PT_N, *part3 = dvp_g + (size_t)B * KTOT_;
-    VT_LDS_LIMIT(smplh_bwd_tile_kernel<BWD_FB>, lds);
-    hipLaunchKernelGGL(smplh_bwd_tile_kernel<BWD_FB>, dim3(NVT_, (B + BWD_FB - 1) / BWD_FB), dim3(256), lds, st, h->W_v64, ws, v_posed, dverts, B, scratch, dvp_g, skip);
-    VT_LAUNCH_CHECK();
-    hipLaunchKernelGGL(smplh_bwd_blend_kernel, dim3(NKS_, (NQ_ / 16 + 4 * BL_NW - 1) / (4 * BL_NW), (B + BL_M - 1) / BL_M), dim3(256), 0, st, h->Q_t, dvp_g, B, part3, skip);
-    VT_LAUNCH_CHECK();
-    hipLaunchKernelGGL(smplh_bwd_frame_kernel, dim3(B), dim3(256), 0, st, pose, h->J_s, h->par, ws, scratch, part3, djtr, B, dpose, dbetas, dtrans, skip);
-    VT_LAUNCH_CHECK();
-    return VT_OK;
+    return smplh_backward_launch(h, pose, B, dverts, djtr, v_posed, ws, scratch, NP_NUM_, dpose, dbetas, dtrans, vt_stream(stream));
+}
+
+extern "C" int vt_smplh_backward_free(const vt_smplh *h, const float *pose, int B, const float *dverts, const float *djtr, const float *v_posed,
+                                      const float *ws, float *scratch, int n_free_pose_cols, float *dpose, float *dbetas, float *dtrans, void *stream)
+{
+    VT_REQUIRE(h && pose && dverts && v_posed && ws && scratch && dpose && dbetas && dtrans && B > 0, "vt_smplh_backward_free: null argument or B <= 0");
+    VT_REQUIRE(n_free_pose_cols > 0 && n_free_pose_cols <= 3 * J_LIVE_ && n_free_pose_cols % 3 == 0,
+               "vt_smplh_backward_free: n_free_pose_cols=%d must be a multiple of 3 in (0, %d] (the joints from %d on are the frozen ones of the layout)",
+               n_free_pose_cols, 3 * J_LIVE_, J_LIVE_);
+    return smplh_backward_launch(h, pose, B, dverts, djtr, v_posed, ws, scratch, n_free_pose_cols, dpose, dbetas, dtrans, vt_stream(stream));
 }
 
 extern "C" int vt_rodrigues_forward(const float *aa, int n, float *R, void *stream)
diff --git a/vistracker_amd/fitting.py b/vistracker_amd/fitting.py
--- a/vistracker_amd/fitting.py
+++ b/vistracker_amd/fitting.py
@@ -212,7 +212,7 @@
 
 class _SmplFit(_Fit):
 
-    def __init__(self, pose, betas, trans, names, nsteps, prev_loss, prof=None):
+    def __init__(self, pose, betas, trans, names, nsteps, prev_loss, prof=None, smpl=None):
         dev = pose.device; B = self.B = pose.shape[0]
         super().__init__(dev, names, nsteps, prev_loss, prof)
         self.pose, self.betas, self.trans = pose, betas, trans
@@ -222,6 +222,11 @@
         self.dpose = torch.empty(B, 156, device=dev); self.dbetas = torch.empty(B, 10, device=dev); self.dtrans = torch.empty(B, 3, device=dev)
         self.vb = torch.empty(B, device=dev)
         self.pose_init = pose.clone()
+        self.prefix, self.n_free = None, 156
+        if smpl is not None:
+            self.prefix = torch.empty(_lib().vt_smplh_prefix_floats(B), device=dev); self.n_free = 66
+            _chk(_lib().vt_smplh_prefix(smpl.h, pose.data_ptr(), B, self.ws.data_ptr(), self.prefix.data_ptr(), L.stream_ptr()))
+            self.dpose.zero_()
 
     @property
     def vert_order_ptr(self):
@@ -256,6 +261,7 @@
     fused_steps = os.environ.get("VT_FUSED_STEPS", "1") != "0"
     fused_smpl_query = os.environ.get("VT_FUSED_SMPL_QUERY", "0") != "0"
     device_skip = os.environ.get("VT_DEVICE_SKIP", "1") != "0"
+    frozen_hands = True
 
     def __init__(self, smpl_model, regressors, priors, decoders=None, part_labels=None, obj_verts=None, obj_faces=None, obj_points=None,
                  cam=ops.DEFAULT_CAM, device="cuda:0"):
@@ -305,11 +311,19 @@
                     self.fp32_fallbacks += 1
                 return run()
 
-    def smpl_forward(self, pose, betas, trans, verts, jtr, vposed, ws):
+    def smpl_forward(self, pose, betas, trans, verts, jtr, vposed, ws, prefix=None):
+        if prefix is not None:
+            _chk(_lib().vt_smplh_forward_prefixed(self.smpl.h, pose.data_ptr(), betas.data_ptr(), trans.data_ptr(), pose.shape[0], prefix.data_ptr(),
+                                                  verts.data_ptr(), jtr.data_ptr(), vposed.data_ptr(), ws.data_ptr(), L.stream_ptr()))
+            return
         _chk(_lib().vt_smplh_forward(self.smpl.h, pose.data_ptr(), betas.data_ptr(), trans.data_ptr(), pose.shape[0], verts.data_ptr(),
                                      jtr.data_ptr(), vposed.data_ptr(), ws.data_ptr(), L.stream_ptr()))
 
-    def smpl_backward(self, pose, betas, dverts, vposed, ws, scratch, dpose, dbetas, dtrans):
+    def smpl_backward(self, pose, betas, dverts, vposed, ws, scratch, dpose, dbetas, dtrans, n_free=156):
+        if n_free < 156:
+            _chk(_lib().vt_smplh_backward_free(self.smpl.h, pose.data_ptr(), pose.shape[0], dverts.data_ptr(), None, vposed.data_ptr(), ws.data_ptr(),
+                                               scratch.data_ptr(), n_free, dpose.data_ptr(), dbetas.data_ptr(), dtrans.data_ptr(), L.stream_ptr()))
+            return
         _chk(_lib().vt_smplh_backward(self.smpl.h, pose.data_ptr(), betas.data_ptr(), pose.shape[0], dverts.data_ptr(), None, vposed.data_ptr(),
                                       ws.data_ptr(), scratch.data_ptr(), dpose.data_ptr(), dbetas.data_ptr(), dtrans.data_ptr(), L.stream_ptr()))
 
@@ -358,7 +372,8 @@
         if weights is not None:
             table.update({k: float(v) for k, v in weights.items() if k in table})
         start, end = it_range if it_range is not None else (0, max_iter)
-        f = _SmplFit(pose, betas, trans, ["kpts", "temp", "ptemp", "pose", "pinit", "hand"], (end - start) * 10, 0.0)
+        f = _SmplFit(pose, betas, trans, ["kpts", "temp", "ptemp", "pose", "pinit", "hand"], (end - start) * 10, 0.0,
+                     smpl=self.smpl if self.frozen_hands else None)
         f.kpts = _as_input(kpts, pose.device)
         f.temporal = temporal and f.B >= 3
         self.hand_prior_value(pose, f.terms, "hand", f.vb)
@@ -388,12 +403,13 @@
             maps.build_projection(self.net)
         total = iter_for_betas + iter_for_kpts + iter_for_pose + max_iter
         start, end = it_range if it_range is not None else (0, total)
-        f = _SmplFit(pose, betas, trans, ["df_h", "part", "pose", "pinit", "j2d", "stemp", "hand"], (end - start) * 10, 300.0, prof)
+        f = _SmplFit(pose, betas, trans, ["df_h", "part", "pose", "pinit", "j2d", "stemp", "hand"], (end - start) * 10, 300.0, prof,
+                     smpl=self.smpl if self.frozen_hands else None)
         f.maps, f.net_size = maps, net_size
         f.crop_center, f.body_center, f.body_kpts = _as_input(crop_center, dev), _as_input(body_center, dev), _as_input(body_kpts, dev)
         f.vert_order = self.vert_order
         if self.sort_query_points:
-            self.smpl_forward(pose, betas, trans, f.verts, f.jtr, f.vposed, f.ws)
+            self.smpl_forward(pose, betas, trans, f.verts, f.jtr, f.vposed, f.ws, f.prefix)
             v0 = f.verts[f.B // 2]
             f.vert_order = morton_order_device(torch.stack([v0[:, 0] / v0[:, 2], v0[:, 1] / v0[:, 2]], 1))
         self.hand_prior_value(pose, f.terms, "hand", f.vb)
@@ -429,7 +445,7 @@
         dev = obj_R.device; B = obj_R.shape[0]
         _require_params(obj_R, obj_t)
         if self.use_projection and self.net.precision != "fp32" and not maps.force_fp32:
-            maps.build_projection(self.net)
+            maps.build_projection(self.net, reuse=True)
         total = joint_iter + iter_for_obj + max_iter + iter_for_sil
         start, end = it_range if it_range is not None else (0, total)
         f = _ObjectFit(self, obj_R, obj_t, sil, (end - start) * 10, prof)
@@ -494,13 +510,13 @@
     def _smplt_step(self, f, phase, k, w, armed):
         lib = _lib(); st = L.stream_ptr(); B = f.B; pose = f.pose
         f.terms.zero(0, 5)
-        self.smpl_forward(pose, f.betas, f.trans, f.verts, f.jtr, f.vposed, f.ws)
+        self.smpl_forward(pose, f.betas, f.trans, f.verts, f.jtr, f.vposed, f.ws, f.prefix)
         _chk(lib.vt_landmarks_forward(self.b25.h, f.verts.data_ptr(), B, f.J.data_ptr(), st))
         _chk(lib.vt_kpts_loss(f.J.data_ptr(), f.kpts.data_ptr(), None, B, 25, 0, self.cam.ctypes.data, 0.0, float(w[0]), f.terms.ptr("kpts"), f.dJ.data_ptr(), st))
         _chk(lib.vt_landmarks_backward(self.b25.h, f.dJ.data_ptr(), B, f.dverts.data_ptr(), 0, st))
         if f.temporal:
             _chk(lib.vt_accel_loss(f.verts.data_ptr(), B, 6890 * 3, None, float(w[1]), f.terms.ptr("temp"), f.dverts.data_ptr(), st))
-        self.smpl_backward(pose, f.betas, f.dverts, f.vposed, f.ws, f.scratch, f.dpose, f.dbetas, f.dtrans)
+        self.smpl_backward(pose, f.betas, f.dverts, f.vposed, f.ws, f.scratch, f.dpose, f.dbetas, f.dtrans, f.n_free)
         if f.temporal:
             _chk(lib.vt_accel_loss_strided(pose.data_ptr(), B, 66, 156, self.jw66.data_ptr(), float(w[2]), f.terms.ptr("ptemp"), f.dpose.data_ptr(), st))
         self.body_prior(pose, f.dpose, float(w[3]), f.terms, "pose", f.vb)
@@ -520,7 +536,7 @@
     def _smpl_step(self, f, phase, k, w, armed):
         lib = _lib(); st = L.stream_ptr(); B = f.B; pose = f.pose
         f.terms.zero(0, 6)
-        self.smpl_forward(pose, f.betas, f.trans, f.verts, f.jtr, f.vposed, f.ws)
+        self.smpl_forward(pose, f.betas, f.trans, f.verts, f.jtr, f.vposed, f.ws, f.prefix)
         self._human_query(f, k, w)
         if phase == "kpts":
             _chk(lib.vt_landmarks_forward(self.b25.h, f.verts.data_ptr(), B, f.J.data_ptr(), st))
@@ -529,7 +545,7 @@
             _chk(lib.vt_landmarks_backward(self.b25.h, f.dJ.data_ptr(), B, f.dverts.data_ptr(), 1, st))
         if B >= 4:
             _chk(lib.vt_accel_loss(f.verts.data_ptr(), B, 6890 * 3, None, float(w[5]), f.terms.ptr("stemp"), f.dverts.data_ptr(), st))
-        self.smpl_backward(pose, f.betas, f.dverts, f.vposed, f.ws, f.scratch, f.dpose, f.dbetas, f.dtrans)
+        self.smpl_backward(pose, f.betas, f.dverts, f.vposed, f.ws, f.scratch, f.dpose, f.dbetas, f.dtrans, f.n_free)
         self.body_prior(pose, f.dpose, float(w[2]), f.terms, "pose", f.vb)
         _chk(lib.vt_sqdiff_loss(pose.data_ptr() + 12, 156, f.pose_init.data_ptr() + 12, 156, B, 69, float(B), float(w[3]),
                                 f.terms.ptr("pinit"), f.dpose.data_ptr() + 12, st))
@@ -539,19 +555,19 @@
 
     def _smpl_step_fused(self, f, phase, k, w, armed):
         lib = _lib(); st = L.stream_ptr(); B = f.B
-        self.smpl_forward(f.pose, f.betas, f.trans, f.verts, f.jtr, f.vposed, f.ws)
+        self.smpl_forward(f.pose, f.betas, f.trans, f.verts, f.jtr, f.vposed, f.ws, f.prefix)
         self._human_query(f, k, w)
         if phase == "kpts":
             _chk(lib.vt_kpts_step(self.b25.h, f.verts.data_ptr(), f.body_kpts.data_ptr(), f.crop_center.data_ptr(), B, 1, self.cam.ctypes.data, f.net_size,
                                   float(w[4]), f.terms.ptr("j2d"), f.J.data_ptr(), f.dverts.data_ptr(), 1, st))
         if B >= 4:
             _chk(lib.vt_accel_loss(f.verts.data_ptr(), B, 6890 * 3, None, float(w[5]), f.terms.ptr("stemp"), f.dverts.data_ptr(), st))
-        self.smpl_backward(f.pose, f.betas, f.dverts, f.vposed, f.ws, f.scratch, f.dpose, f.dbetas, f.dtrans)
+        self.smpl_backward(f.pose, f.betas, f.dverts, f.vposed, f.ws, f.scratch, f.dpose, f.dbetas, f.dtrans, f.n_free)
         self._smpl_tail(f, k, w, armed)
 
     def _smpl_step_fused_query(self, f, phase, k, w, armed):
         lib = _lib(); st = L.stream_ptr(); B = f.B
-        self.smpl_forward(f.pose, f.betas, f.trans, f.verts, f.jtr, f.vposed, f.ws)
+        self.smpl_forward(f.pose, f.betas, f.trans, f.verts, f.jtr, f.vposed, f.ws, f.prefix)
         if phase == "kpts":
             _chk(lib.vt_kpts_step(self.b25.h, f.verts.data_ptr(), f.body_kpts.data_ptr(), f.crop_center.data_ptr(), B, 1, self.cam.ctypes.data, f.net_size,
                                   float(w[4]), f.terms.ptr("j2d"), f.J.data_ptr(), f.dverts.data_ptr(), 0, st))
@@ -560,7 +576,7 @@
                                      self.labels.data_ptr(), f.vert_order_ptr, float(w[0]), float(w[1]), int(phase == "kpts"), float(w[5]),
                                      f.terms.ptr("stemp") if B >= 4 else None, f.dverts.data_ptr(), f.terms.ptr("df_h"), st))
         _ev_end(f.lp, "human", ev, B, k)
-        self.smpl_backward(f.pose, f.betas, f.dverts, f.vposed, f.ws, f.scratch, f.dpose, f.dbetas, f.dtrans)
+        self.smpl_backward(f.pose, f.betas, f.dverts, f.vposed, f.ws, f.scratch, f.dpose, f.dbetas, f.dtrans, f.n_free)
         self._smpl_tail(f, k, w, armed)
 
     def _smpl_tail(self, f, k, w, armed):
diff --git a/vistracker_amd/ops.py b/vistracker_amd/ops.py
--- a/vistracker_amd/ops.py
+++ b/vistracker_amd/ops.py
@@ -197,7 +197,7 @@
         for t, c in zip(self.t, MAP_CHANNELS):
             assert t.is_cuda and t.is_contiguous() and t.dtype == torch.float32 and t.shape[-1] == c and t.shape[1] == t.shape[2]
         self.B = self.t[0].shape[0]
-        self.proj = None
+        self.proj = None; self._proj_key = None
         self.c = L.VtMaps()
         for i, t in enumerate(self.t):
             self.c.maps[i] = t.data_ptr(); self.c.res[i] = t.shape[1]
@@ -234,18 +234,24 @@
             fm.c.proj = fm.proj.data_ptr(); fm.c.proj_cols = self.c.proj_cols; fm.c.proj_level = self.c.proj_level
         return fm
 
-    def build_projection(self, net):
+    def build_projection(self, net, reuse=False):
         h = net.h if hasattr(net, "h") else net.handle.h
+        key = (h.value if hasattr(h, "value") else int(h), int(self.c.act_level), tuple(t.data_ptr() for t in self.t),
+               torch.cuda.current_stream(self.t[0].device).cuda_stream)
+        if reuse and self.proj is not None and self.c.proj and self._proj_key == key:
+            return self
+        self._proj_key = None
         n = L.lib().vt_query_projection_floats(C.byref(self.c), self.B)
         self.proj = torch.empty(n, device=self.t[0].device)
         self.c.proj = None; self.c.proj_cols = 0
         L.check(L.lib().vt_query_build_projection(h, C.byref(self.c), self.B, self.proj.data_ptr(), L.stream_ptr()))
         self.c.proj = self.proj.data_ptr(); self.c.proj_cols = n // (self.B * self.t[0].shape[1] * self.t[0].shape[2])
         self.c.proj_level = self.c.act_level
+        self._proj_key = key
         return self
 
     def drop_projection(self):
-        self.proj = None; self.c.proj = None; self.c.proj_cols = 0
+        self.proj = None; self.c.proj = None; self.c.proj_cols = 0; self._proj_key = None
         return self
 
     @staticmethod
```

New measurement: 155.0 (median of 6 runs). 2.3% higher.
